# ArbiterMob/FluidSimulationCuda

Measured on AMD Instinct MI355X. Metric: Mcells/s per Jacobi iter, higher is better.
Workload: dtype f32

## Files before the change

### fluidsimulationcuda_amd/capi.py

```python
import ctypes as C
import os

import numpy as np

from ._build import LIB

OK, E_INVALID, E_NOMEM, E_HIP, E_COMM = 0, 1, 2, 3, 4
U, V, DENS, U_PREV, V_PREV, DENS_PREV, TMP0, TMP1, TMP2, TMP3, TMP4, TMP5 = range(12)
NFIELDS = 12
JACOBI_STREAM, JACOBI_LDS, JACOBI_NAIVE, JACOBI_TB = 0, 1, 2, 3
STORAGE_F32, STORAGE_F16 = 0, 1
PARAM_TB_MAX_SWEEPS, PARAM_TB_ROWS, PARAM_HALO, PARAM_TB_FAST_DIVISION, PARAM_TB_MIN_CELLS, PARAM_TB_EDGE_ROWS_PCT = 0, 1, 2, 3, 4, 5
PARAM_TB_LANE_COLUMNS = 6
PARAM_TB_T16_MIN_CELLS = 7
PARAM_TB_AUTOTUNE = 8
PARAM_FUSE_DIVERGENCE = 9
PARAM_SLAB_OVERLAP = 10
PARAM_EARLY_ADVECT = 11
PARAM_FUSE_ADD_SOURCE = 12
PARAM_XCHG_OVERLAP = 13
PARAM_F16_PRESSURE_SCALE = 14
PARAM_TB_FILL = 15
XCHG_HALO, XCHG_GATHER, XCHG_MAX, XCHG_MAX_BEGIN, XCHG_MAX_END = 0, 1, 2, 3, 4
RCCL_ID_BYTES = 128
FIELD_NAMES = ("u", "v", "dens", "u_prev", "v_prev", "dens_prev", "tmp0", "tmp1", "tmp2", "tmp3", "tmp4", "tmp5")


class FluidError(RuntimeError):
    def __init__(self, code, msg):
        super().__init__("libfluid_amd error %d: %s" % (code, msg))
        self.code = code


class Config(C.Structure):
    _fields_ = [("n", C.c_int), ("rank", C.c_int), ("nranks", C.c_int), ("halo", C.c_int),
                ("jacobi_variant", C.c_int), ("stream", C.c_void_p), ("arena", C.c_void_p),
                ("arena_bytes", C.c_size_t), ("storage", C.c_int)]


TIME_SOURCE, TIME_DIFFUSION, TIME_DIVERGENCE, TIME_PROJECTION, TIME_ADVECTION = range(5)
TIMING_CATEGORIES = ("source", "diffusion", "divergence", "projection", "advection")


class Timing(C.Structure):
    _fields_ = [("jacobi_ms", C.c_double), ("sweeps", C.c_longlong), ("solves", C.c_longlong),
                ("category_ms", C.c_double * 5), ("category_calls", C.c_longlong * 5),
                ("jacobi_launches", C.c_longlong), ("jacobi_field_launches", C.c_longlong),
                ("pressure_ms", C.c_double), ("pressure_sweeps", C.c_longlong)]


class RunPlan(C.Structure):
    _fields_ = [("iters", C.c_int), ("nsteps", C.c_int), ("use_sources", C.c_int), ("sources", C.c_void_p),
                ("every", C.c_int), ("fields", C.POINTER(C.c_int)), ("nfields", C.c_int),
                ("snapshots", C.c_void_p), ("capacity", C.c_size_t)]


EXCHANGE_FN = C.CFUNCTYPE(C.c_int, C.c_void_p, C.c_int, C.POINTER(C.c_int), C.c_int, C.c_int,
                          C.POINTER(C.c_float))

_HOSTF = np.ctypeslib.ndpointer(dtype=np.float32, flags="C_CONTIGUOUS")
_ctx = C.c_void_p
_i, _f = C.c_int, C.c_float
_MF = C.POINTER(C.c_float)

SIGNATURES = {
    "step": [_i, _f, _f, _f, _HOSTF, _HOSTF, _HOSTF],
    "step_src": [_i, _f, _f, _f, _i] + [_HOSTF] * 6,
    "fluid_release_cached": [],
    "fluid_coefficients": [_i, _f, _f, C.POINTER(_f), C.POINTER(_f)],
    "fluid_layout": [_i, C.POINTER(_i), C.POINTER(_i), C.POINTER(C.c_size_t)],
    "fluid_create": [_i, C.POINTER(_ctx)],
    "fluid_create_ex": [C.POINTER(Config), C.POINTER(_ctx)],
    "fluid_create_ensemble": [C.POINTER(Config), _i, C.POINTER(_ctx)],
    "fluid_members": [_ctx, C.POINTER(_i)],
    "fluid_upload_member": [_ctx, _i, _i, _HOSTF],
    "fluid_download_member": [_ctx, _i, _i, _HOSTF],
    "fluid_step_members": [_ctx, _MF, _MF, _MF, _i, _i, _i],
    "fluid_vel_step_members": [_ctx, _MF, _MF, _i],
    "fluid_dens_step_members": [_ctx, _MF, _MF, _i],
    "fluid_op_add_source_members": [_ctx, _i, _i, _MF],
    "fluid_op_jacobi_sweep_members": [_ctx, _i, _i, _i, _i, _MF, _MF],
    "fluid_op_diffuse_members": [_ctx, _i, _i, _i, _MF, _MF, _i],
    "fluid_op_advect_members": [_ctx, _i, _i, _i, _i, _i, _MF],
    "fluid_destroy": [_ctx],
    "fluid_synchronize": [_ctx],
    "fluid_owned_rows": [_ctx, C.POINTER(_i), C.POINTER(_i)],
    "fluid_field_ptr": [_ctx, _i, C.POINTER(C.c_void_p)],
    "fluid_scalar_ptr": [_ctx, C.POINTER(C.c_void_p)],
    "fluid_upload": [_ctx, _i, _HOSTF],
    "fluid_download": [_ctx, _i, _HOSTF],
    "fluid_upload_rows": [_ctx, _i, _HOSTF, _i, _i],
    "fluid_download_rows": [_ctx, _i, _HOSTF, _i, _i],
    "fluid_fill": [_ctx, _i, _f],
    "fluid_step": [_ctx, _f, _f, _f, _i, _i, _i],
    "fluid_vel_step": [_ctx, _f, _f, _i],
    "fluid_dens_step": [_ctx, _f, _f, _i],
    "fluid_op_set_bnd": [_ctx, _i, _i],
    "fluid_op_add_source": [_ctx, _i, _i, _f],
    "fluid_op_jacobi_sweep": [_ctx, _i, _i, _i, _i, _f, _f],
    "fluid_op_diffuse": [_ctx, _i, _i, _i, _f, _f, _i],
    "fluid_op_advect": [_ctx, _i, _i, _i, _i, _i, _f],
    "fluid_op_divergence": [_ctx, _i, _i, _i, _i],
    "fluid_op_subtract_gradient": [_ctx, _i, _i, _i],
    "fluid_residual": [_ctx, _i, _i, _f, _f, C.POINTER(_f)],
    "fluid_absmax_velocity": [_ctx, _i, _i, C.POINTER(_f)],
    "fluid_residual_members": [_ctx, _i, _i, _MF, _MF, _MF],
    "fluid_absmax_velocity_members": [_ctx, _i, _i, _MF],
    "fluid_member_moments": [_ctx, _i, C.POINTER(C.c_double), C.POINTER(C.c_double)],
    "fluid_ensemble_stats": [_ctx, _i, _MF, _MF],
    "fluid_ensemble_stats_ptr": [_ctx, C.POINTER(C.c_void_p), C.POINTER(C.c_void_p)],
    "fluid_member_gram": [_ctx, _i, _i, C.POINTER(C.c_double)],
    "fluid_pack_members": [_ctx, _i, _i, _i, C.c_void_p, C.c_size_t],
    "fluid_unpack_members": [_ctx, _i, _i, _i, C.c_void_p, C.c_size_t],
    "fluid_download_members": [_ctx, _i, _MF],
    "fluid_upload_members": [_ctx, _i, _MF],
    "fluid_run": [_ctx, _f, _f, _f, C.POINTER(RunPlan), C.POINTER(_i)],
    "fluid_run_members": [_ctx, _MF, _MF, _MF, C.POINTER(RunPlan), C.POINTER(_i)],
    "fluid_coarse_size": [_i, _i, C.POINTER(_i)],
    "fluid_pack_members_coarse": [_ctx, _i, _i, _i, _i, C.c_void_p, C.c_size_t],
    "fluid_download_members_coarse": [_ctx, _i, _i, _MF],
    "fluid_run_coarse": [_ctx, _f, _f, _f, C.POINTER(RunPlan), _i, C.POINTER(_i)],
    "fluid_run_members_coarse": [_ctx, _MF, _MF, _MF, C.POINTER(RunPlan), _i, C.POINTER(_i)],
    "fluid_transform_members": [_ctx, C.POINTER(_i), _i, _MF],
    "fluid_select_members": [_ctx, C.POINTER(_i), _i, C.POINTER(_i)],
    "fluid_set_jacobi_variant": [_ctx, _i],
    "fluid_division_mode": [_ctx, _f, _f, C.POINTER(_i)],
    "fluid_autotune_pending": [_ctx, C.POINTER(_i)],
    "fluid_plan_sweeps": [_i, _i, _i, _i, _i, _i, _i, C.POINTER(_i), _i, C.POINTER(_i)],
    "fluid_set_param": [_ctx, _i, _i],
    "fluid_timing_enable": [_ctx, _i],
    "fluid_timing_read": [_ctx, C.POINTER(Timing), _i],
    "fluid_op_diffuse_tol": [_ctx, _i, _i, _i, _f, _f, _f, _i, _i, C.POINTER(_i), C.POINTER(_f)],
    "fluid_set_exchange": [_ctx, EXCHANGE_FN, C.c_void_p],
    "fluid_exchange_now": [_ctx, _i, C.POINTER(_i), _i, _i],
    "fluid_exchange_stream": [_ctx, C.POINTER(C.c_void_p)],
    "fluid_split_launches": [_ctx, C.POINTER(C.c_longlong)],
    "fluid_rccl_available": [],
    "fluid_rccl_unique_id": [C.c_void_p, C.c_size_t],
    "fluid_exchange_rccl_attach": [_ctx, C.c_void_p, C.c_size_t],
    "fluid_exchange_rccl_attach_comm": [_ctx, C.c_void_p],
    "fluid_exchange_rccl_detach": [_ctx],
    "fluid_exchange_rccl_calls": [_ctx, C.POINTER(C.c_longlong), C.POINTER(C.c_longlong), C.POINTER(C.c_longlong)],
}
OTHER_SYMBOLS = {"fluid_last_error": (C.c_char_p, []), "fluid_arena_bytes": (C.c_size_t, [_i]),
                 "fluid_arena_bytes_ex": (C.c_size_t, [_i, _i]),
                 "fluid_arena_bytes_ensemble": (C.c_size_t, [_i, _i, _i])}
MAX_MEMBERS = 21845
COARSE_FACTORS = (1, 2, 4, 8, 16, 32, 64)
TRANSFORM_MAX_MEMBERS = 64

_lib = None


def lib():
    global _lib
    if _lib is None:
        if not os.path.exists(LIB):
            raise ImportError("%s not found: run `python -c 'import __graft_entry__ as g; g.build()'` "
                              "(hipcc --offload-arch=gfx950). There is no CPU fallback." % LIB)
        try:
            import torch
        except ImportError:
            pass
        L = C.CDLL(LIB)
        for name, args in SIGNATURES.items():
            fn = getattr(L, name)
            fn.restype, fn.argtypes = C.c_int, args
        for name, (res, args) in OTHER_SYMBOLS.items():
            fn = getattr(L, name)
            fn.restype, fn.argtypes = res, args
        _lib = L
    return _lib


def check(rc):
    if rc != OK:
        raise FluidError(rc, lib().fluid_last_error().decode(errors="replace"))
```

### fluidsimulationcuda_amd/csrc/fluid_ctx.h

```cpp
#pragma once
#include <hip/hip_runtime.h>

#include <string>
#include <utility>
#include <vector>

#include "../../include/fluid_amd.h"
#include "fluid_kernels.h"

namespace fluid_detail {
int fail(int code, const char* fmt, ...);
int materialize_zero(fluid_ctx* c, int f);
int refuse_ensemble(const fluid_ctx* c, const char* what);
struct RcclExchange;
void rccl_release(RcclExchange* x);
}

#define HIP_TRY(expr)                                                                                      \
    do {                                                                                                   \
        hipError_t e_ = (expr);                                                                            \
        if (e_ != hipSuccess)                                                                              \
            return fluid_detail::fail(e_ == hipErrorOutOfMemory ? FLUID_E_NOMEM : FLUID_E_HIP, "%s: %s",   \
                                      #expr, hipGetErrorString(e_));                                       \
    } while (0)

#define TRY(expr)                        \
    do {                                 \
        int rc_ = (expr);                \
        if (rc_ != FLUID_OK) return rc_; \
    } while (0)

class MemberVal {
    float s_;
    std::vector<float> v_;
    explicit MemberVal(std::vector<float>&& v) : s_(v[0]), v_(std::move(v)) {}

public:
    MemberVal(float v = 0.0f) : s_(v) {}
    MemberVal(const float* per_member, int members) : s_(per_member[0]), v_(per_member, per_member + members) {}
    bool uniform() const { return v_.empty(); }
    float at(int m) const { return v_.empty() ? s_ : v_[(size_t)m]; }
    const std::vector<float>& values() const { return v_; }
    bool operator==(const MemberVal& o) const { return s_ == o.s_ && v_ == o.v_; }
    template <class F>
    MemberVal map(const MemberVal& b, F f) const
    {
        if (uniform() && b.uniform()) return MemberVal(f(s_, b.s_));
        std::vector<float> r(uniform() ? b.v_.size() : v_.size());
        for (size_t m = 0; m < r.size(); ++m) r[m] = f(at((int)m), b.at((int)m));
        return MemberVal(std::move(r));
    }
    template <class F>
    MemberVal map(F f) const { return map(MemberVal(), [&](float x, float) { return f(x); }); }
};

struct FieldState {
    void* ptr = nullptr;
    int reach = 0;
    bool zero = false;
    bool pend = false;
    MemberVal pend_inc;
    int src_of = 0;
    MemberVal src_dt;
    float fscale = 1.0f;
};

struct ConstRing {
    char *dev = nullptr, *host = nullptr;
    size_t bytes = 0, head = 0;
    struct Blob { size_t off, len; unsigned long long hash; hipEvent_t copied; };
    std::vector<Blob> live;
    std::vector<hipEvent_t> free_events;
};

struct EnsembleReduce {
    unsigned int* d_max = nullptr;
    double2* d_moments = nullptr;
    double2* d_partials = nullptr;
    char* host = nullptr;
    float *d_mean = nullptr, *d_var = nullptr;
    bool have_stats = false;
    double *d_gram_partials = nullptr, *d_gram = nullptr, *gram_host = nullptr;
};

struct MemberStage {
    float* dev = nullptr;
    int members = 0;
};

struct TransformTables {
    static constexpr int kSlots = 8;
    char *dev = nullptr, *host = nullptr;
    size_t slot = 0;
    int next = 0;
    hipEvent_t copied[kSlots] = {};
    bool in_use[kSlots] = {};
};

struct fluid_ctx {
    int n = 0, w = 0, pitch = 0;
    size_t field_floats = 0;
    int members = 1;
    char* arena = nullptr;
    bool own_arena = false;
    int st = fluid::STORAGE_F32;
    size_t esz = 4;
    hipStream_t stream = nullptr;
    bool own_stream = false;
    hipStream_t stream2 = nullptr;
    hipEvent_t ev_fork = nullptr, ev_join = nullptr;
    bool slab_overlap = true;
    hipStream_t xstream = nullptr;
    hipEvent_t ev_xbegin = nullptr, ev_xdone = nullptr;
    bool xchg_overlap = true;
    unsigned xowed = 0;
    long long split_launches = 0;
    bool early_advect = true;
    float vmax_prev[2] = {-1.0f, -1.0f};
    FieldState field[FLUID_NFIELDS];
    size_t field_bytes = 0;
    unsigned int* d_scalar = nullptr;
    float* d_partials = nullptr;
    ConstRing consts;
    EnsembleReduce red;
    MemberStage stage;
    TransformTables xform;
    unsigned int* tiles = nullptr;
    unsigned int* h_scalar = nullptr;
    hipEvent_t scalar_ready = nullptr;
    int variant = fluid::JACOBI_TB;
    int tb_max_t = 16, tb_rows = 0, num_cu = 256;
    long long tb_min_cells = 0;
    long long tb_t16_min_cells = -1;
    bool fuse_divergence = true;
    bool tb_fill = true;
    bool autotune = true;
    struct Trial { unsigned long long key; int cand; hipEvent_t a, b; };
    std::vector<Trial> trials;
    std::vector<hipEvent_t> free_events;
    bool defer_zero_source = true;
    bool in_halo_exchange = false;
    int tb_nv = 2;
    int tb_edge_pct = 40;
    int fast_div = 2;
    int rank = 0, nranks = 1, own0 = 1, own1 = 1, min_slab = 0, halo = 1;
    bool fuse_add_source = true;
    float pscale = 1.0f;
    fluid_exchange_fn xchg = nullptr;
    void* xchg_user = nullptr;
    fluid_detail::RcclExchange* rccl = nullptr;
    bool timing = false;
    struct Ev { hipEvent_t a, b; int cat; bool pressure; };
    std::vector<Ev> ev_pool;
    size_t ev_used = 0;
    double cat_ms[FLUID_TIMING_CATEGORIES] = {};
    long long cat_calls[FLUID_TIMING_CATEGORIES] = {};
    long long sweeps = 0, pending_sweeps = 0, launches = 0, field_launches = 0;
    double pressure_ms = 0.0;
    long long pressure_sweeps = 0, pending_pressure_sweeps = 0;
    bool in_pressure_solve = false;

    bool valid_field(int id) const { return id >= 0 && id < FLUID_NFIELDS; }
    void* ptr(int id) const { return field[id].ptr; }
    fluid::Members mb() const { return {members, field_floats}; }
    size_t all_bytes() const { return field_bytes * (size_t)members; }
    void* row(int id, int r) const { return static_cast<char*>(ptr(id)) + (size_t)r * pitch * esz; }
    int lo_all() const { return own0 - (rank == 0 ? 1 : 0); }
    int hi_all() const { return own1 + (rank == nranks - 1 ? 1 : 0); }
};
```

### fluidsimulationcuda_amd/csrc/fluid_kernels.h

```cpp
#pragma once
#include <hip/hip_runtime.h>

namespace fluid {

constexpr int XOFF = 63;

enum JacobiVariant { JACOBI_STREAM = 0, JACOBI_LDS = 1, JACOBI_NAIVE = 2, JACOBI_TB = 3, JACOBI_VARIANTS = 4 };

enum Storage { STORAGE_F32 = 0, STORAGE_F16 = 1 };
typedef _Float16 half_t;
inline size_t storage_bytes(int st) { return st == STORAGE_F16 ? 2 : 4; }

inline int pitch_for(int n) { return ((XOFF + 1 + 4 * ((n + 3) / 4) + 1) + 63) / 64 * 64; }

struct Members {
    int count = 1;
    size_t stride = 0;
};

struct TbMemberK {
    double yd;
    float alpha, beta, hi, lo;
    float x0_inc, div_scale;
    unsigned tile_thr, pad;
};

struct TbBatch {
    const void* x[3];
    const void* x0[3];
    void* out[3];
    float alpha[3], beta[3];
    double yd[3];
    float hi[3], lo[3];
    const unsigned* tiles[3];
    unsigned tile_thr[3];
    int tile_pitch;
    void* div[3];
    float div_scale;
    int b[3];
    int x_zero[3];
    float x0_inc[3];
    int count;
    int members;
    size_t mstride;
    size_t tile_mstride;
    const TbMemberK* mk;
};

void launch_set_bnd(hipStream_t s, int st, void* f, int pitch, int n, int b, Members mb = {});
void launch_add_source(hipStream_t s, int st, void* x, const void* src, int pitch, int row_lo, int row_hi, float dt, Members mb = {},
                       const float* mdt = nullptr);
void launch_jacobi(hipStream_t s, int st, int variant, const void* x, const void* x0, void* out, int pitch, int n,
                   int row_lo, int row_hi, float alpha, float beta, int b, Members mb = {}, const float2* mab = nullptr);
enum TbForm { TB_PLAIN = 0, TB_DIVSRC = 1, TB_ADDSRC = 2 };
struct TbShape { int T, divmode, nv, form; };
inline constexpr TbShape kTbShapes[] = {
    {2, 0, 2, TB_PLAIN},   {2, 2, 2, TB_PLAIN},   {2, 3, 2, TB_PLAIN},   {2, 4, 2, TB_PLAIN},   {2, 5, 2, TB_PLAIN},
    {2, 0, 4, TB_PLAIN},   {2, 2, 4, TB_PLAIN},   {2, 3, 4, TB_PLAIN},   {2, 4, 4, TB_PLAIN},   {2, 5, 4, TB_PLAIN},
    {4, 0, 2, TB_PLAIN},   {4, 2, 2, TB_PLAIN},   {4, 3, 2, TB_PLAIN},   {4, 4, 2, TB_PLAIN},   {4, 5, 2, TB_PLAIN},
    {4, 0, 4, TB_PLAIN},   {4, 2, 4, TB_PLAIN},   {4, 3, 4, TB_PLAIN},   {4, 4, 4, TB_PLAIN},   {4, 5, 4, TB_PLAIN},
    {8, 0, 2, TB_PLAIN},   {8, 2, 2, TB_PLAIN},   {8, 3, 2, TB_PLAIN},   {8, 4, 2, TB_PLAIN},   {8, 5, 2, TB_PLAIN},
    {8, 0, 4, TB_PLAIN},   {8, 2, 4, TB_PLAIN},   {8, 3, 4, TB_PLAIN},   {8, 4, 4, TB_PLAIN},   {8, 5, 4, TB_PLAIN},
    {12, 0, 2, TB_PLAIN},  {12, 2, 2, TB_PLAIN},  {12, 3, 2, TB_PLAIN},  {12, 4, 2, TB_PLAIN},  {12, 5, 2, TB_PLAIN},
    {16, 0, 2, TB_PLAIN},  {16, 2, 2, TB_PLAIN},  {16, 3, 2, TB_PLAIN},  {16, 4, 2, TB_PLAIN},  {16, 5, 2, TB_PLAIN},
    {8, 4, 2, TB_DIVSRC},  {12, 4, 2, TB_DIVSRC}, {16, 4, 2, TB_DIVSRC}, {8, 0, 2, TB_ADDSRC},  {8, 2, 2, TB_ADDSRC},  {8, 5, 2, TB_ADDSRC},
    {12, 0, 2, TB_ADDSRC}, {12, 2, 2, TB_ADDSRC}, {12, 5, 2, TB_ADDSRC}, {16, 0, 2, TB_ADDSRC}, {16, 2, 2, TB_ADDSRC}, {16, 5, 2, TB_ADDSRC},
};
constexpr int kTbShapeCount = sizeof(kTbShapes) / sizeof(kTbShapes[0]);
constexpr int jacobi_tb_index(int T, int divmode, int nv, int form)
{
    for (int i = 0; i < kTbShapeCount; ++i) {
        const TbShape& s = kTbShapes[i];
        if ((T < 0 || s.T == T) && (divmode < 0 || s.divmode == divmode) && s.nv == nv && s.form == form) return i;
    }
    return -1;
}
constexpr bool jacobi_tb_exists(int T, int divmode, int nv, int form) { return jacobi_tb_index(T, divmode, nv, form) >= 0; }
constexpr bool tb_shapes_unique(int i = 0)
{
    return i == kTbShapeCount || (jacobi_tb_index(kTbShapes[i].T, kTbShapes[i].divmode, kTbShapes[i].nv, kTbShapes[i].form) == i && tb_shapes_unique(i + 1));
}
static_assert(kTbShapeCount == 52 && tb_shapes_unique(), "52 distinct shapes: adding or removing one is a change of this table");
inline constexpr int kTbDepths[] = {16, 12, 8, 4, 2};
constexpr bool is_tb_depth(int T) { for (int d : kTbDepths) if (d == T) return true; return false; }
bool launch_jacobi_tb(hipStream_t s, int st, int T, int divmode, int nv, int form, const TbBatch& batch, int pitch, int n, int row_lo,
                      int row_hi, int rb, int rb_edge, int hole_lo = 0, int hole_hi = 0, bool fill = true);
constexpr int kTileRows = 32, kTileCols = 64;
inline int tile_rows(int n) { return (n + kTileRows - 1) / kTileRows; }
inline int tile_pitch(int n) { return (n + kTileCols - 1) / kTileCols; }
struct TileBatch {
    const void* field[3];
    unsigned* tiles[3];
    int count;
    size_t mstride, tile_mstride;
};
void launch_tile_min_abs(hipStream_t s, int st, const TileBatch& tb, int count, int pitch, int n, int row_lo, int row_hi, int tile_pitch,
                         Members mb = {}, size_t tile_mstride = 0);
void launch_validate_div(hipStream_t s, int divmode, float beta, float kbeta, double yd, float hi, float lo, unsigned long long* bad);
void launch_advect(hipStream_t s, int st, void* d, const void* d0, const void* u, const void* v, int pitch, int n,
                   int row_lo, int row_hi, float dt0, int b, Members mb = {}, const float* mdt0 = nullptr);
void launch_advect2(hipStream_t s, int st, void* da, const void* d0a, int ba, void* db, const void* d0b, int bb, const void* u,
                    const void* v, int pitch, int n, int row_lo, int row_hi, float dt0, Members mb = {}, const float* mdt0 = nullptr);
void launch_divergence(hipStream_t s, int st, const void* u, const void* v, void* p, void* div, int pitch, int n,
                       int row_lo, int row_hi, float h, int write_p, float pscale = 1.0f, Members mb = {});
void launch_scale(hipStream_t s, int st, void* x, int pitch, int row_lo, int row_hi, float factor, Members mb = {});
constexpr int kMaxPartials = 8192;
void launch_subtract_gradient(hipStream_t s, int st, void* u, void* v, const void* p, int pitch, int n, int row_lo,
                              int row_hi, float h, float* partials = nullptr, unsigned int* max_out = nullptr, float pinv = 1.0f,
                              Members mb = {});
void launch_gradient_advect(hipStream_t s, int st, void* u, void* v, const void* p, void* d, const void* d0, int pitch, int n,
                            int row_lo, int row_hi, float h, float dt0, int b, float pinv = 1.0f, Members mb = {},
                            const float* mdt0 = nullptr);
void launch_absmax2(hipStream_t s, int st, const void* u, const void* v, int pitch, int n, int row_lo, int row_hi,
                    unsigned int* result, Members mb = {}, int rstride = 0);
void launch_residual(hipStream_t s, int st, const void* x, const void* x0, int pitch, int n, int row_lo, int row_hi,
                     float alpha, float beta, unsigned int* result, Members mb = {}, int rstride = 0, const float2* mab = nullptr);
constexpr int kMomentBlocks = 4096;
int moment_blocks(int n, int members);
void launch_member_moments(hipStream_t s, int st, const void* x, int pitch, int n, Members mb, double2* partials, double2* out);
void launch_ensemble_stats(hipStream_t s, int st, const void* x, int pitch, int n, Members mb, float* mean, float* var);
void launch_pack_members(hipStream_t s, int st, const void* x, int pitch, int n, Members mb, float inv, float* dense, size_t dstride);
void launch_unpack_members(hipStream_t s, int st, void* x, int pitch, int n, Members mb, const float* dense, size_t dstride);
void launch_pack_members_coarse(hipStream_t s, int st, const void* x, int pitch, int n, Members mb, float inv, int factor, float* coarse,
                                size_t cstride);
constexpr int kTransformMaxMembers = 64;
inline int transform_padded(int members)
{
    int mp = 1;
    while (mp < members) mp <<= 1;
    return mp;
}
void launch_transform_members(hipStream_t s, int st, void* x, int pitch, int n, Members mb, float inv, const double* table,
                              const unsigned long long* bits, unsigned long long empty, bool dense);
inline int gram_padded(int members) { return members > 8 ? transform_padded(members) : 8; }
int gram_blocks(int n, int members);
void launch_member_gram(hipStream_t s, int st, const void* x, int pitch, int n, Members mb, float inv, bool centre, double* partials,
                        double* out);

}
```

### fluidsimulationcuda_amd/csrc/fluid_kernels.hip

```cpp
#include <hip/hip_runtime.h>
#include <stdint.h>

#include <algorithm>
#include <array>
#include <cstdlib>
#include <utility>

#include "fluid_kernels.h"

namespace fluid {

__device__ __forceinline__ float flip_if(bool c, float v) { return c ? -v : v; }

__device__ __forceinline__ float keep_f32(float v) { asm("" : "+v"(v)); return v; }
__device__ __forceinline__ float ld1(const float* p) { return *p; }
__device__ __forceinline__ float ld1(const half_t* p) { return keep_f32((float)*p); }
__device__ __forceinline__ void st1(float* p, float v) { *p = v; }
__device__ __forceinline__ void st1(half_t* p, float v) { *p = (half_t)keep_f32(v); }
template <typename S>
__device__ __forceinline__ float as_stored(float v)
{
    if constexpr (sizeof(S) == 2) return keep_f32((float)(S)keep_f32(v));
    else return v;
}
// ... 222 lines not shown
    if (mab) {
        const float2 ab = mab[blockIdx.z];
        alpha = ab.x;
        beta = ab.y;
    }
    x += blockIdx.z * ms; x0 += blockIdx.z * ms; out += blockIdx.z * ms;
    const int lane = threadIdx.x & 63;
    const int vec = blockIdx.x * 256 + threadIdx.x;
    const int nvec = (n + 3) >> 2;
    const int i0 = row_lo + blockIdx.y * RB;
    const int i1 = min(i0 + RB, row_hi);
    const bool active = vec < nvec;
    const int v = active ? vec : nvec - 1;
    const int j = 1 + 4 * v;
    const size_t P = (size_t)pitch;
    const S* xc = x + XOFF + j;
    const S* rc = x0 + XOFF + j;
    S* oc = out + XOFF + j;
    const bool edge_lo = (lane == 0), edge_hi = (lane == 63) | (vec >= nvec - 1);
    const bool nx = (b == 1), ny = (b == 2);

    float4 up = ld4(xc + (size_t)(i0 - 1) * P);
    float4 me = ld4(xc + (size_t)i0 * P);
    for (int i = i0; i < i1; ++i) {
        const float4 dn = ld4(xc + (size_t)(i + 1) * P);
        const float4 r = ld4(rc + (size_t)i * P);
        float le = 0.f, re = 0.f;
        if (edge_lo) le = ld1(xc + (size_t)i * P - 1);
        if (edge_hi) re = ld1(xc + (size_t)i * P + 4);
        float L = from_lane_below(me.w, le);
        float R = from_lane_above(me.x, re);
        if (edge_lo) L = le;
        if (edge_hi) R = re;
        float4 o;
        float nb;
        nb = L + me.y;     nb = nb + up.x; nb = nb + dn.x; o.x = (r.x + alpha * nb) / beta;
        nb = me.x + me.z;  nb = nb + up.y; nb = nb + dn.y; o.y = (r.y + alpha * nb) / beta;
        nb = me.y + me.w;  nb = nb + up.z; nb = nb + dn.z; o.z = (r.z + alpha * nb) / beta;
        nb = me.z + R;     nb = nb + up.w; nb = nb + dn.w; o.w = (r.w + alpha * nb) / beta;
        if (active) {
            S* orow = oc + (size_t)i * P;
            const int last = n - j;
            if (last >= 3) {
                st4(orow, o);
            } else {
                st1(orow, o.x);
                if (last >= 1) st1(orow + 1, o.y);
                if (last >= 2) st1(orow + 2, o.z);
            }
            const float vn = last == 0 ? o.x : last == 1 ? o.y : last == 2 ? o.z : o.w;
            if (j == 1) st1(orow - 1, flip_if(nx, o.x));
            if (last <= 3) st1(orow + last + 1, flip_if(nx, vn));
            if (i == 1 || i == n) {
                float4 g4;
                g4.x = flip_if(ny, o.x); g4.y = flip_if(ny, o.y);
                g4.z = flip_if(ny, o.z); g4.w = flip_if(ny, o.w);
                const float cl = 0.5f * (g4.x + flip_if(nx, o.x));
                const float cr = 0.5f * (flip_if(ny, vn) + flip_if(nx, vn));
#pragma unroll
                for (int side = 0; side < 2; ++side) {
                    if (side == 0 ? i != 1 : i != n) continue;
                    S* g = oc + (side == 0 ? (size_t)0 : (size_t)(n + 1) * P);
                    if (last >= 3) {
                        st4(g, g4);
                    } else {
                        st1(g, g4.x);
                        if (last >= 1) st1(g + 1, g4.y);
                        if (last >= 2) st1(g + 2, g4.z);
                    }
                    if (j == 1) st1(g - 1, cl);
                    if (last <= 3) st1(g + last + 1, cr);
                }
            }
        }
        up = me;
        me = dn;
    }
}



template <int NV>
struct Vec {
    float c[NV];
};
typedef float v2f __attribute__((ext_vector_type(2)));
typedef half_t half2_t __attribute__((ext_vector_type(2)));

template <int NV>
__device__ __forceinline__ Vec<NV> buf_ldv(const float*, __amdgpu_buffer_rsrc_t r, unsigned off)
{
    Vec<NV> v;
    if constexpr (NV == 4) {
        const uint4_t u = __builtin_amdgcn_raw_buffer_load_b128(r, off, 0, 0);
        v.c[0] = __uint_as_float(u.x); v.c[1] = __uint_as_float(u.y); v.c[2] = __uint_as_float(u.z); v.c[3] = __uint_as_float(u.w);
    } else {
        const uint2_t u = __builtin_amdgcn_raw_buffer_load_b64(r, off, 0, 0);
        v.c[0] = __uint_as_float(u.x); v.c[1] = __uint_as_float(u.y);
    }
    return v;
}
template <int NV>
__device__ __forceinline__ Vec<NV> buf_ldv(const half_t*, __amdgpu_buffer_rsrc_t r, unsigned off)
{
    Vec<NV> v;
    if constexpr (NV == 4) {
        const uint2_t u = __builtin_amdgcn_raw_buffer_load_b64(r, off, 0, 0);
        half4_t h;
        __builtin_memcpy(&h, &u, 8);
        v.c[0] = keep_f32((float)h.x); v.c[1] = keep_f32((float)h.y); v.c[2] = keep_f32((float)h.z); v.c[3] = keep_f32((float)h.w);
    } else {
        const unsigned u = __builtin_amdgcn_raw_buffer_load_b32(r, off, 0, 0);
        half2_t h;
        __builtin_memcpy(&h, &u, 4);
        v.c[0] = keep_f32((float)h.x); v.c[1] = keep_f32((float)h.y);
    }
    return v;
}
template <int NV>
__device__ __forceinline__ void buf_stv(float*, __amdgpu_buffer_rsrc_t r, unsigned off, const Vec<NV>& v)
{
    if constexpr (NV == 4) {
        uint4_t u;
        u.x = __float_as_uint(v.c[0]); u.y = __float_as_uint(v.c[1]); u.z = __float_as_uint(v.c[2]); u.w = __float_as_uint(v.c[3]);
        __builtin_amdgcn_raw_buffer_store_b128(u, r, off, 0, 0);
    } else {
        uint2_t u;
        u.x = __float_as_uint(v.c[0]); u.y = __float_as_uint(v.c[1]);
        __builtin_amdgcn_raw_buffer_store_b64(u, r, off, 0, 0);
    }
}
template <int NV>
__device__ __forceinline__ void buf_stv(half_t*, __amdgpu_buffer_rsrc_t r, unsigned off, const Vec<NV>& v)
{
    if constexpr (NV == 4) {
        half4_t h;
        h.x = (half_t)keep_f32(v.c[0]); h.y = (half_t)keep_f32(v.c[1]); h.z = (half_t)keep_f32(v.c[2]); h.w = (half_t)keep_f32(v.c[3]);
        uint2_t u;
        __builtin_memcpy(&u, &h, 8);
        __builtin_amdgcn_raw_buffer_store_b64(u, r, off, 0, 0);
    } else {
        half2_t h;
        h.x = (half_t)keep_f32(v.c[0]); h.y = (half_t)keep_f32(v.c[1]);
        unsigned u;
        __builtin_memcpy(&u, &h, 4);
        __builtin_amdgcn_raw_buffer_store_b32(u, r, off, 0, 0);
    }
}

struct DivK {
    float beta;
    double yd;
    float hi, lo;
};
constexpr float kDiv5NegScale = -0x1p24f;

template <typename S, int NV>
struct TbArgs {
    const S* xc;
    const S* rc;
    S* oc;
    __amdgpu_buffer_rsrc_t bx, br, bo;
    unsigned ld_off;
    unsigned st_off;
    unsigned row_bytes;
    unsigned m_lg;
    unsigned m_r[NV];
    int n, q_lo, q_hi, cg;
    float alpha;
    DivK k;
    S* dc;
    __amdgpu_buffer_rsrc_t bd;
    float div_scale;
    int s_lo, s_hi;
    unsigned sx, sy;
    float x0_inc;
    bool st_rg_lane, is_lg;
    bool fill;
};

__device__ __forceinline__ float fxor(float v, unsigned m) { return __uint_as_float(__float_as_uint(v) ^ m); }
template <int NV>
__device__ __forceinline__ Vec<NV> fxorv(const Vec<NV>& v, unsigned m)
{
    Vec<NV> o;
#pragma unroll
    for (int c = 0; c < NV; ++c) o.c[c] = fxor(v.c[c], m);
    return o;
}

template <int DIVMODE>
__device__ __forceinline__ float tb_div(float num, const DivK& k)
{
    if (DIVMODE == 0) return num / k.beta;
    if (DIVMODE == 4) return num * k.beta;
    if (DIVMODE == 3) return __builtin_fmaf(num, k.hi, num * k.lo);
    if (DIVMODE == 5) {
        const float q0 = num * k.beta;
        const float e = __builtin_fmaf(q0, k.hi, num * kDiv5NegScale);
        return __builtin_fmaf(e, k.lo, q0);
    }
    return (float)((double)num * k.yd);
}
template <int DIVMODE>
__device__ __forceinline__ v2f tb_div2(v2f num, const DivK& k)
{
    if constexpr (DIVMODE == 4) return num * k.beta;
    else if constexpr (DIVMODE == 3) {
        const v2f p = num * k.lo;
        return __builtin_elementwise_fma(num, (v2f){k.hi, k.hi}, p);
    } else if constexpr (DIVMODE == 5) {
        const v2f ds = num * kDiv5NegScale;
        const v2f q0 = num * k.beta;
        const v2f e = __builtin_elementwise_fma(q0, (v2f){k.hi, k.hi}, ds);
        return __builtin_elementwise_fma(e, (v2f){k.lo, k.lo}, q0);
    } else return (v2f){tb_div<DIVMODE>(num.x, k), tb_div<DIVMODE>(num.y, k)};
}

template <int DIVMODE, int NV>
__device__ __forceinline__ Vec<NV> tb_stencil(const Vec<NV>& up, const Vec<NV>& me, const Vec<NV>& dn, const Vec<NV>& r,
                                              float alpha, const DivK& k)
{
    float h[NV];
    h[0] = lane_below0(me.c[NV - 1]) + me.c[1];
#pragma unroll
    for (int c = 1; c < NV - 1; ++c) h[c] = me.c[c - 1] + me.c[c + 1];
    h[NV - 1] = me.c[NV - 2] + lane_above0(me.c[0]);
    Vec<NV> G;
#pragma unroll
    for (int p = 0; p < NV; p += 2) {
        v2f s = {h[p], h[p + 1]};
        s = s + (v2f){up.c[p], up.c[p + 1]};
        s = s + (v2f){dn.c[p], dn.c[p + 1]};
        if constexpr (DIVMODE != 4) s = s * alpha;
        s = (v2f){r.c[p], r.c[p + 1]} + s;
        s = tb_div2<DIVMODE>(s, k);
        G.c[p] = s.x;
        G.c[p + 1] = s.y;
    }
    return G;
}

template <int DIVMODE>
__global__ __launch_bounds__(256) void k_validate_div(float beta, DivK k, unsigned long long* __restrict__ bad)
{
    unsigned long long n = 0;
    const unsigned long long stride = (unsigned long long)gridDim.x * 256;
    auto differs = [](float got, float ref) { return (ref != ref) ? !(got != got) : (__float_as_uint(got) != __float_as_uint(ref)); };
    DivK k2 = k;
    for (unsigned long long i = (unsigned long long)blockIdx.x * 256 + threadIdx.x; i < (1ull << 32); i += stride) {
        const float a = __uint_as_float((unsigned)i);
        const float ref = a / beta;
        if constexpr (DIVMODE == 3) {
            const bool in_range = a == 0.0f || !(__builtin_fabsf(a) < beta * 0x1p-98f);
            n += differs(tb_div<2>(a, k2), ref) || (in_range && differs(tb_div<3>(a, k), ref));
        } else if constexpr (DIVMODE == 5) {
            const float got = tb_div<5>(a, k);
            const bool finite = __builtin_fabsf(got) < __builtin_inff();
            const bool must_be_exact = __builtin_fabsf(a) < 0x1p100f;
            n += differs(got, ref) && (finite || must_be_exact);
        } else {
            n += differs(tb_div<DIVMODE>(a, k), ref);
        }
    }
    if (n) atomicAdd(bad, n);
}

__device__ __forceinline__ float bitsel(unsigned mask, float a, float b)
{
    return __uint_as_float((__float_as_uint(a) & mask) | (__float_as_uint(b) & ~mask));
}

template <typename S, int NV>
__device__ __forceinline__ void tb_fix_columns(Vec<NV>& G, const TbArgs<S, NV>& a, float& v1, float& vn, bool need_corners)
{
    float o[NV];
#pragma unroll
    for (int c = 0; c < NV; ++c) o[c] = G.c[c];
    const float from_right = lane_above0(o[0]);
    const float from_left = lane_below0(o[NV - 1]);
    G.c[0] = bitsel(a.m_r[0], fxor(from_left, a.sx), o[0]);
#pragma unroll
    for (int c = 1; c < NV - 1; ++c) G.c[c] = bitsel(a.m_r[c], fxor(o[c - 1], a.sx), o[c]);
    G.c[NV - 1] = bitsel(a.m_lg, fxor(from_right, a.sx), bitsel(a.m_r[NV - 1], fxor(o[NV - 2], a.sx), o[NV - 1]));
    if (need_corners) {
        v1 = from_right;
        unsigned bits = __float_as_uint(from_left) & a.m_r[0];
#pragma unroll
        for (int c = 1; c < NV; ++c) bits |= __float_as_uint(o[c - 1]) & a.m_r[c];
        vn = __uint_as_float(bits);
    }
}

template <bool EDGE, bool WALL, typename S, int NV>
__device__ __forceinline__ void tb_store_to(S* oc, __amdgpu_buffer_rsrc_t bo, const Vec<NV>& G, int q, bool mine, const TbArgs<S, NV>& a,
                                            float v1, float vn)
{
    auto on = [](bool c, unsigned off) { return c ? off : kBufOff; };
    buf_stv<NV>(oc, bo, on(mine, a.st_off) + (unsigned)q * a.row_bytes, G);
    if (WALL) {
        Vec<NV> g = fxorv<NV>(G, a.sy);
        if (EDGE) {
            const float cl = 0.5f * (fxor(v1, a.sy) + fxor(v1, a.sx));
            const float cr = 0.5f * (fxor(vn, a.sy) + fxor(vn, a.sx));
            if (a.is_lg) g.c[NV - 1] = cl;
#pragma unroll
            for (int c = 0; c < NV; ++c)
                if (a.st_rg_lane && a.cg == c) g.c[c] = cr;
        }
        buf_stv<NV>(oc, bo, on(mine & (q == 1), a.st_off), g);
        buf_stv<NV>(oc, bo, on(mine & (q == a.n), a.st_off) + (unsigned)(a.n + 1) * a.row_bytes, g);
    }
}
template <bool EDGE, bool WALL, typename S, int NV>
__device__ __forceinline__ void tb_store(const Vec<NV>& G, int q, bool mine, const TbArgs<S, NV>& a, float v1, float vn)
{
    tb_store_to<EDGE, WALL, S, NV>(a.oc, a.bo, G, q, mine, a, v1, vn);
}

template <int NV>
__device__ __forceinline__ Vec<NV> tb_divergence(const Vec<NV>& u, const Vec<NV>& v_up, const Vec<NV>& v_dn, float scale)
{
    float g[NV];
#pragma unroll
    for (int c = 0; c < NV; ++c) {
        const float ur = c < NV - 1 ? u.c[c + 1] : lane_above0(u.c[0]);
        const float ul = c > 0 ? u.c[c - 1] : lane_below0(u.c[NV - 1]);
        g[c] = ur - ul;
    }
    Vec<NV> d;
#pragma unroll
    for (int p = 0; p < NV; p += 2) {
        v2f s = {g[p], g[p + 1]};
        s = s + (v2f){v_dn.c[p], v_dn.c[p + 1]};
        s = s - (v2f){v_up.c[p], v_up.c[p + 1]};
        s = s * scale;
        d.c[p] = s.x;
        d.c[p + 1] = s.y;
    }
    return d;
}

template <int NV>
__device__ __forceinline__ Vec<NV> take(const Vec<NV>& v)
{
    Vec<NV> o;
#pragma unroll
    for (int p = 0; p < NV; p += 2) {
        v2f in = {v.c[p], v.c[p + 1]}, out;
        asm("v_mov_b64 %0, %1" : "=v"(out) : "v"(in));
        o.c[p] = out.x;
        o.c[p + 1] = out.y;
    }
    return o;
}

template <int K, int N, int NV>
__device__ __forceinline__ void tb_qshift(Vec<NV> (&Q)[N])
{
    if constexpr (K >= 1) {
        Q[K] = Q[K - 1];
        tb_qshift<K - 1, N, NV>(Q);
    }
}

template <int DIVMODE, int NV>
__device__ __forceinline__ void tb_sticky(const Vec<NV>& G, v2f& nf)
{
    if constexpr (DIVMODE == 5) {
#pragma unroll
        for (int p = 0; p < NV; p += 2) nf = __builtin_elementwise_fma((v2f){G.c[p], G.c[p + 1]}, (v2f){0.f, 0.f}, nf);
    }
}

template <int T, int DIVMODE, bool EDGE, bool WALL, bool GEN, int PH, typename S, int NV, bool DIVSRC = false, bool ADDSRC = false,
          bool PART = false>
__device__ __forceinline__ void tb_step(int t, Vec<NV> (&W)[T][3], Vec<NV> (&Q)[T + 1], Vec<NV> (&PX)[3], Vec<NV> (&PQ)[3],
                                        const TbArgs<S, NV>& a, Vec<NV> (&UR)[3], Vec<NV> (&VR)[3], v2f& nf, int smax = T)
{
    static_assert(!(PART && GEN), "the general body runs every stage");
    constexpr int UP = PH % 3, ME = (PH + 1) % 3, FR = (PH + 2) % 3;
    __builtin_amdgcn_sched_barrier(0);
    if constexpr (DIVSRC) {
        UR[FR] = take<NV>(PX[PH]);
        VR[FR] = take<NV>(PQ[PH]);
    } else {
        W[0][FR] = take<NV>(PX[PH]);
        Q[0] = take<NV>(PQ[PH]);
        if constexpr (ADDSRC) {
#pragma unroll
            for (int p = 0; p < NV; p += 2) {
                const v2f ds = (v2f){W[0][FR].c[p], W[0][FR].c[p + 1]} * a.div_scale;
                const v2f q = (v2f){Q[0].c[p], Q[0].c[p + 1]} + ds;
                Q[0].c[p] = as_stored<S>(q.x);
                Q[0].c[p + 1] = as_stored<S>(q.y);
            }
            buf_stv<NV>(a.dc, a.bd, (((t >= a.s_lo) & (t < a.s_hi)) ? a.st_off : kBufOff) + (unsigned)t * a.row_bytes, Q[0]);
        } else {
#pragma unroll
            for (int p = 0; p < NV; p += 2) {
                const v2f q = (v2f){Q[0].c[p], Q[0].c[p + 1]} + a.x0_inc;
                Q[0].c[p] = q.x;
                Q[0].c[p + 1] = q.y;
            }
        }
    }
    {
        const unsigned off = a.ld_off + (unsigned)(t + 3) * a.row_bytes;
        PX[PH] = buf_ldv<NV>(a.xc, a.bx, off);
        PQ[PH] = buf_ldv<NV>(a.rc, a.br, off);
    }
    __builtin_amdgcn_sched_barrier(0);
    if constexpr (DIVSRC) {
        const int q = t - 1;
        Vec<NV> D = tb_divergence<NV>(UR[ME], VR[UP], VR[FR], a.div_scale);
#pragma unroll
        for (int c = 0; c < NV; ++c) D.c[c] = as_stored<S>(D.c[c]);
        Q[1] = D;
        float v1 = 0.f, vn = 0.f;
        if (EDGE) tb_fix_columns<S, NV>(D, a, v1, vn, WALL);
        tb_store_to<EDGE, (WALL || GEN), S, NV>(a.dc, a.bd, D, q, (q >= 1) & (q <= a.n) & (q >= a.q_lo) & (q < a.q_hi), a, v1, vn);
    }
    if constexpr (!GEN) {
#pragma unroll
        for (int s = 1; s <= T; ++s) {
            const bool run = !PART || s <= smax;
            const int q = t - s;
            Vec<NV> G;
            float v1 = 0.f, vn = 0.f;
            if (run) {
                G = tb_stencil<DIVMODE, NV>(W[s - 1][UP], W[s - 1][ME], W[s - 1][FR], Q[s], a.alpha, a.k);
                if (EDGE) tb_fix_columns<S, NV>(G, a, v1, vn, WALL && s == T);
                if (s == T) tb_sticky<DIVMODE, NV>(G, nf);
            } else {
#pragma unroll
                for (int c = 0; c < NV; ++c) G.c[c] = __builtin_nondeterministic_value(W[s - 1][FR].c[c]);
            }
            if (s < T) W[s][FR] = G;
            else tb_store<EDGE, WALL, S, NV>(G, q, run & (q >= a.q_lo) & (q < a.q_hi), a, v1, vn);
        }
    } else {
#pragma unroll
        for (int s = 1; s <= T; ++s) {
            const int q = t - s;
            const bool interior = (q >= 1 && q <= a.n);
            Vec<NV> G = tb_stencil<DIVMODE, NV>(W[s - 1][UP], W[s - 1][ME], W[s - 1][FR], Q[s], a.alpha, a.k);
            float v1 = 0.f, vn = 0.f;
            if (EDGE) tb_fix_columns<S, NV>(G, a, v1, vn, s == T);
            if (s < T) {
                const Vec<NV> me = W[s][ME];
                const Vec<NV> flipped_me = fxorv<NV>(me, a.sy);
                const Vec<NV> flipped_g = fxorv<NV>(G, a.sy);
                const bool bot_ghost = (q == a.n + 1), top_ghost = (q == 1);
#pragma unroll
                for (int c = 0; c < NV; ++c) {
                    W[s][FR].c[c] = bot_ghost ? flipped_me.c[c] : G.c[c];
                    W[s][ME].c[c] = top_ghost ? flipped_g.c[c] : me.c[c];
                }
            } else {
                tb_sticky<DIVMODE, NV>(G, nf);
                tb_store<EDGE, true, S, NV>(G, q, interior & (q >= a.q_lo) & (q < a.q_hi), a, v1, vn);
            }
        }
    }
    tb_qshift<T, T + 1, NV>(Q);
}

template <int T, int DIVMODE, bool EDGE, bool WALL, typename S, int NV, bool DIVSRC = false, bool ADDSRC = false>
__device__ __forceinline__ bool tb_march(int t0, int t1, const TbArgs<S, NV>& a)
{
    Vec<NV> W[T][3], Q[T + 1], PX[3], PQ[3], UR[3], VR[3];
    v2f nf = {0.f, 0.f};
    Vec<NV> zero;
#pragma unroll
    for (int c = 0; c < NV; ++c) zero.c[c] = 0.f;
#pragma unroll
    for (int s = 0; s < T; ++s) { W[s][0] = zero; W[s][1] = zero; W[s][2] = zero; }
#pragma unroll
    for (int s = 0; s <= T; ++s) Q[s] = zero;
#pragma unroll
    for (int d = 0; d < 3; ++d) { UR[d] = zero; VR[d] = zero; }
#pragma unroll
    for (int d = 0; d < 3; ++d) {
        const unsigned off = a.ld_off + (unsigned)(t0 + d) * a.row_bytes;
        PX[d] = buf_ldv<NV>(a.xc, a.bx, off);
        PQ[d] = buf_ldv<NV>(a.rc, a.br, off);
        buf_stv<NV>(a.oc, a.bo, kBufOff, zero);
        if constexpr (DIVSRC || ADDSRC) buf_stv<NV>(a.dc, a.bd, kBufOff, zero);
        __builtin_amdgcn_sched_barrier(0);
    }
    int t = t0;
    if constexpr (WALL) {
        for (; t <= t1 && t < T + 1; t += 3) {
            tb_step<T, DIVMODE, EDGE, WALL, true, 0, S, NV, DIVSRC, ADDSRC>(t, W, Q, PX, PQ, a, UR, VR, nf);
            tb_step<T, DIVMODE, EDGE, WALL, true, 1, S, NV, DIVSRC, ADDSRC>(t + 1, W, Q, PX, PQ, a, UR, VR, nf);
            tb_step<T, DIVMODE, EDGE, WALL, true, 2, S, NV, DIVSRC, ADDSRC>(t + 2, W, Q, PX, PQ, a, UR, VR, nf);
        }
    }
    const int fill_end = (a.fill && t0 == a.q_lo - T) ? t0 + 3 * ((2 * T + 2) / 3) : t0;
    const int full_end = a.fill ? t1 - 2 : t1;
    auto stages = [&](int u) { return u > t1 ? 0 : u < fill_end ? (u - t0) >> 1 : T; };
    for (; t <= t1 && t < fill_end && (!WALL || t + 1 <= a.n); t += 3) {
        tb_step<T, DIVMODE, EDGE, WALL, false, 0, S, NV, DIVSRC, ADDSRC, true>(t, W, Q, PX, PQ, a, UR, VR, nf, stages(t));
        tb_step<T, DIVMODE, EDGE, WALL, false, 1, S, NV, DIVSRC, ADDSRC, true>(t + 1, W, Q, PX, PQ, a, UR, VR, nf, stages(t + 1));
        tb_step<T, DIVMODE, EDGE, WALL, false, 2, S, NV, DIVSRC, ADDSRC, true>(t + 2, W, Q, PX, PQ, a, UR, VR, nf, stages(t + 2));
    }
    for (; t <= full_end && (!WALL || t + 1 <= a.n); t += 3) {
        tb_step<T, DIVMODE, EDGE, WALL, false, 0, S, NV, DIVSRC, ADDSRC>(t, W, Q, PX, PQ, a, UR, VR, nf);
        tb_step<T, DIVMODE, EDGE, WALL, false, 1, S, NV, DIVSRC, ADDSRC>(t + 1, W, Q, PX, PQ, a, UR, VR, nf);
        tb_step<T, DIVMODE, EDGE, WALL, false, 2, S, NV, DIVSRC, ADDSRC>(t + 2, W, Q, PX, PQ, a, UR, VR, nf);
    }
    for (; t <= t1 && (!WALL || t + 1 <= a.n); t += 3) {
        tb_step<T, DIVMODE, EDGE, WALL, false, 0, S, NV, DIVSRC, ADDSRC, true>(t, W, Q, PX, PQ, a, UR, VR, nf, stages(t));
        tb_step<T, DIVMODE, EDGE, WALL, false, 1, S, NV, DIVSRC, ADDSRC, true>(t + 1, W, Q, PX, PQ, a, UR, VR, nf, stages(t + 1));
        tb_step<T, DIVMODE, EDGE, WALL, false, 2, S, NV, DIVSRC, ADDSRC, true>(t + 2, W, Q, PX, PQ, a, UR, VR, nf, stages(t + 2));
    }
    if constexpr (WALL) {
        for (; t <= t1; t += 3) {
            tb_step<T, DIVMODE, EDGE, WALL, true, 0, S, NV, DIVSRC, ADDSRC>(t, W, Q, PX, PQ, a, UR, VR, nf);
            tb_step<T, DIVMODE, EDGE, WALL, true, 1, S, NV, DIVSRC, ADDSRC>(t + 1, W, Q, PX, PQ, a, UR, VR, nf);
            tb_step<T, DIVMODE, EDGE, WALL, true, 2, S, NV, DIVSRC, ADDSRC>(t + 2, W, Q, PX, PQ, a, UR, VR, nf);
        }
    }
    if constexpr (DIVMODE == 5) return __builtin_amdgcn_ballot_w64((nf.x != nf.x) | (nf.y != nf.y)) != 0ull;
    else return false;
}

template <int T, int DIVMODE, typename S, int NV, bool DIVSRC = false, bool ADDSRC = false>
__device__ __forceinline__ bool tb_march_any(bool edge, bool wall, int t0, int t1, const TbArgs<S, NV>& a)
{
    if (edge) {
        if (wall) return tb_march<T, DIVMODE, true, true, S, NV, DIVSRC, ADDSRC>(t0, t1, a);
        return tb_march<T, DIVMODE, true, false, S, NV, DIVSRC, ADDSRC>(t0, t1, a);
    }
    if (wall) return tb_march<T, DIVMODE, false, true, S, NV, DIVSRC, ADDSRC>(t0, t1, a);
    return tb_march<T, DIVMODE, false, false, S, NV, DIVSRC, ADDSRC>(t0, t1, a);
}

struct TbGrid {
    int inner_wins, inner_blocks, edge_wins, edge_blocks, first_right;
    int hole_lo, hole_hi;
};

constexpr int tb_waves_per_simd(int T, int NV) { return NV == 2 ? (T <= 8 ? 4 : T <= 12 ? 3 : 2) : (T <= 4 ? 3 : 2); }

template <int T, int DIVMODE, int NV, typename S, bool DIVSRC = false, bool ADDSRC = false>
__global__ __launch_bounds__(256, tb_waves_per_simd(T, NV)) void k_jacobi_tb(TbBatch batch, int pitch, int n, int row_lo,
                                                                             int row_hi, int rb, int rb_edge, TbGrid g, int fill)
{
    static_assert(!DIVSRC || DIVMODE == 4, "the divergence-sourced launch is the first launch of a pressure solve");
    static_assert(!(DIVSRC && ADDSRC) && (!ADDSRC || DIVMODE != 3), "one second store per launch; mode 3's tiles are taken from the summed field");
    const unsigned per_xcd = gridDim.x >> 3;
    unsigned vid = (blockIdx.x & 7u) * per_xcd + (blockIdx.x >> 3);
    if (vid >= (unsigned)(g.inner_blocks + g.edge_blocks)) return;
    int win, strip_group;
    if (vid < (unsigned)g.inner_blocks) {
        win = 1 + (int)(vid % (unsigned)g.inner_wins);
        strip_group = (int)(vid / (unsigned)g.inner_wins);
    } else {
        vid -= (unsigned)g.inner_blocks;
        const int e = (int)(vid % (unsigned)g.edge_wins);
        strip_group = (int)(vid / (unsigned)g.edge_wins);
        win = e == 0 ? 0 : g.first_right + e - 1;
    }
    const unsigned member = batch.count == 3 ? blockIdx.z / 3u : batch.count == 2 ? blockIdx.z >> 1 : blockIdx.z;
    const unsigned sv = blockIdx.z - member * (unsigned)batch.count;
    const size_t mofs = (size_t)member * batch.mstride;
    const S* __restrict__ x = static_cast<const S*>(batch.x[sv]) + mofs;
    const S* __restrict__ x0 = static_cast<const S*>(batch.x0[sv]) + mofs;
    S* __restrict__ out = static_cast<S*>(batch.out[sv]) + mofs;
    float alpha = batch.alpha[sv], beta = batch.beta[sv];
    double yd = batch.yd[sv];
    float k_hi = batch.hi[sv], k_lo = batch.lo[sv], x0_inc = batch.x0_inc[sv], div_scale = batch.div_scale;
    unsigned tile_thr = batch.tile_thr[sv];
    if (batch.mk != nullptr) {
        typedef const TbMemberK __attribute__((address_space(4))) * MemberKPtr;
        const MemberKPtr mk = (MemberKPtr)(uintptr_t)batch.mk + ((size_t)sv * (unsigned)batch.members + member);
        alpha = mk->alpha;
        beta = mk->beta;
        yd = mk->yd;
        k_hi = mk->hi;
        k_lo = mk->lo;
        x0_inc = mk->x0_inc;
        if (ADDSRC) div_scale = mk->div_scale;
        if (DIVMODE == 3) tile_thr = mk->tile_thr;
    }
    const int b = batch.b[sv];
    constexpr int HL = (T + NV - 1) / NV;
    constexpr int VS = 64 - 2 * HL;
    constexpr int C0 = (XOFF + 1) / NV;
    static_assert((XOFF + 1) % NV == 0 && HL <= C0, "window overlap must fit the row's left pad");
    const int lane = threadIdx.x & 63;
    const int strip = strip_group * 4 + __builtin_amdgcn_readfirstlane(threadIdx.x >> 6);
    const int kg = n / NV;
    const bool left_edge = (win == 0);
    const bool right_edge = (kg >= win * VS - HL) && (kg < win * VS - HL + 64);
    const bool edge = left_edge || right_edge;
    const int rbw = edge ? rb_edge : rb;
    TbArgs<S, NV> a;
    a.k.yd = yd;
    a.k.lo = k_lo;
    a.k.hi = k_hi;
    a.x0_inc = x0_inc;
    int seg_hi = row_hi;
    a.q_lo = row_lo + strip * rbw;
    if (g.hole_lo < g.hole_hi) {
        const int top = (g.hole_lo - row_lo + rbw - 1) / rbw;
        if (strip < top) seg_hi = g.hole_lo;
        else a.q_lo = g.hole_hi + (strip - top) * rbw;
    }
    if (a.q_lo >= seg_hi) return;
    a.q_hi = min(a.q_lo + rbw, seg_hi);
    a.s_lo = a.q_lo == 1 ? 0 : a.q_lo;
    a.s_hi = a.q_hi == n + 1 ? n + 2 : a.q_hi;
    const int k = win * VS - HL + lane;
    const int nvec = (n + NV - 1) / NV;
    const bool ld_ok = k <= pitch / NV - C0 - 1;
    const ptrdiff_t cofs = (ptrdiff_t)(XOFF + 1) + NV * (ptrdiff_t)(ld_ok ? k : 0);
    a.xc = x + cofs;
    a.rc = x0 + cofs;
    a.oc = out + cofs;
    {
        const unsigned field_bytes = (unsigned)((size_t)(n + 2) * (size_t)pitch * sizeof(S));
        a.bx = __builtin_amdgcn_make_buffer_rsrc(const_cast<S*>(x), 0, (batch.x_zero[sv] && !DIVSRC) ? 0u : field_bytes, 0x00020000);
        a.br = __builtin_amdgcn_make_buffer_rsrc(const_cast<S*>(x0), 0, field_bytes, 0x00020000);
        a.bo = __builtin_amdgcn_make_buffer_rsrc(out, 0, field_bytes, 0x00020000);
        S* dv = (DIVSRC || ADDSRC) ? static_cast<S*>(batch.div[sv]) + mofs : out;
        a.dc = dv + cofs;
        a.bd = __builtin_amdgcn_make_buffer_rsrc(dv, 0, field_bytes, 0x00020000);
        a.div_scale = div_scale;
        a.row_bytes = (unsigned)((size_t)pitch * sizeof(S));
        const unsigned col = (unsigned)((XOFF + 1 + NV * (ptrdiff_t)k) * (ptrdiff_t)sizeof(S));
        a.ld_off = ld_ok ? col : kBufOff;
    }
    a.n = n;
    a.cg = n % NV;
    a.is_lg = (k == -1);
    const bool is_rg = (k == kg);
    const bool own = (lane >= HL) && (lane < 64 - HL);
    const bool st_int = own && k >= 0 && k < nvec;
    a.st_rg_lane = is_rg && (own || k == nvec);
    a.m_lg = a.is_lg ? 0xFFFFFFFFu : 0u;
#pragma unroll
    for (int c = 0; c < NV; ++c) a.m_r[c] = (is_rg && a.cg == c) ? 0xFFFFFFFFu : 0u;
    a.st_off = (ld_ok && (st_int || a.is_lg || a.st_rg_lane)) ? a.ld_off : kBufOff;
    a.sx = (b == 1) ? 0x80000000u : 0u;
    a.sy = (b == 2) ? 0x80000000u : 0u;
    a.alpha = alpha;
    a.k.beta = beta;
    a.fill = fill != 0;
    const int t0 = max(0, a.q_lo - T), t1 = a.q_hi - 1 + T;
    const bool wall = (a.q_lo < T) || (a.q_hi - 1 + T > n + 1);
    constexpr int DM = DIVMODE == 3 ? 2 : DIVMODE;
    bool two_term = false;
    if constexpr (DIVMODE == 3) {
        const unsigned* __restrict__ tiles = batch.tiles[sv] ? batch.tiles[sv] + (size_t)member * batch.tile_mstride : nullptr;
        const unsigned thr = tile_thr;
        const int tr0 = (max(1, a.q_lo - T + 1) - 1) / kTileRows, tr1 = (min(n, a.q_hi + T - 2) - 1) / kTileRows;
        const int c0 = max(1, 1 + NV * (win * VS - HL)), c1 = min(n, NV * (win * VS - HL + 64));
        const int tc0 = (c0 - 1) / kTileCols, tc1 = (c1 - 1) / kTileCols, ntc = tc1 - tc0 + 1;
        const int count = (tr1 - tr0 + 1) * ntc;
        bool low = false;
        if (tiles != nullptr)
            for (int i = lane; i < count; i += 64)
                low |= tiles[(size_t)(tr0 + i / ntc) * batch.tile_pitch + (tc0 + i % ntc)] < thr;
        two_term = tiles != nullptr && __builtin_amdgcn_ballot_w64(low) == 0ull;
    }
    if (two_term) {
        tb_march_any<T, DIVMODE, S, NV>(edge, wall, t0, t1, a);
    } else {
        const bool again = tb_march_any<T, DM, S, NV, DIVSRC, ADDSRC>(edge, wall, t0, t1, a);
        if constexpr (DIVMODE == 5) {
            if (again) tb_march_any<T, 2, S, NV, false, ADDSRC>(edge, wall, t0, t1, a);
        }
    }
}

template <typename S>
__global__ __launch_bounds__(256) void k_tile_min_abs(TileBatch tb, int pitch, int n, int row_lo, int row_hi, int tile_row0, int tile_pitch)
{
    const unsigned member = blockIdx.z / (unsigned)tb.count, sv = blockIdx.z - member * (unsigned)tb.count;
    const S* __restrict__ f = static_cast<const S*>(tb.field[sv]) + (size_t)member * tb.mstride;
    unsigned* __restrict__ out = tb.tiles[sv] + (size_t)member * tb.tile_mstride;
    const int lane = threadIdx.x & 63, wave = threadIdx.x >> 6;
    const int tr = tile_row0 + blockIdx.y;
    const int j = 1 + 4 * (lane + 64 * (blockIdx.x * 4 + wave));
    const int i0 = max(row_lo, 1 + tr * kTileRows), i1 = min(row_hi, 1 + (tr + 1) * kTileRows);
    const size_t P = (size_t)pitch;
    float m = __builtin_inff();
    if (j <= n)
        for (int i = i0; i < i1; ++i) {
            const float4 v = ld4(f + (size_t)i * P + XOFF + j);
            m = fminf(m, fabsf(v.x));
            if (j + 1 <= n) m = fminf(m, fabsf(v.y));
            if (j + 2 <= n) m = fminf(m, fabsf(v.z));
            if (j + 3 <= n) m = fminf(m, fabsf(v.w));
        }
#pragma unroll
    for (int off = 8; off > 0; off >>= 1) m = fminf(m, __shfl_xor(m, off, 16));
    const bool whole = row_lo <= 1 + tr * kTileRows && row_hi >= min(n + 1, 1 + (tr + 1) * kTileRows);
    if ((lane & 15) == 0 && j <= n) out[(size_t)tr * tile_pitch + (j - 1) / kTileCols] = whole ? __float_as_uint(m) : 0u;
}

template <typename S, typename IDX>
__device__ __forceinline__ const S* at(const S* base, IDX byte_off) { return reinterpret_cast<const S*>(reinterpret_cast<const char*>(base) + byte_off); }
template <typename S, typename IDX>
__device__ __forceinline__ S* at(S* base, IDX byte_off) { return reinterpret_cast<S*>(reinterpret_cast<char*>(base) + byte_off); }

template <typename IDX>
struct AdvectTap {
    IDX o;
    float s0, s1, t0, t1;
};

template <typename IDX>
__device__ __forceinline__ AdvectTap<IDX> advect_trace(int j, int i, float uu, float vv, float dt0, int n, IDX P, IDX E)
{
    float px = (float)j - dt0 * uu;
    float py = (float)i - dt0 * vv;
    const float hi = (float)n + 0.5f;
    px = __builtin_fminf(__builtin_fmaxf(px, 0.5f), hi);
    py = __builtin_fminf(__builtin_fmaxf(py, 0.5f), hi);
    const int j0 = (int)px, i0 = (int)py;
    AdvectTap<IDX> t;
    t.s1 = px - (float)j0;
    t.s0 = 1.0f - t.s1;
    t.t1 = py - (float)i0;
    t.t0 = 1.0f - t.t1;
    t.o = (IDX)i0 * P + (IDX)(XOFF + j0) * E;
    return t;
}

struct __attribute__((packed, aligned(4))) FloatPair { float a, b; };
__device__ __forceinline__ void ld_pair(const float* p, float& a, float& b)
{
    const FloatPair v = *reinterpret_cast<const FloatPair*>(p);
    a = v.a;
    b = v.b;
}
__device__ __forceinline__ void ld_pair(const half_t* p, float& a, float& b)
{
    a = ld1(p);
    b = ld1(p + 1);
}

template <typename S, typename IDX>
__device__ __forceinline__ float advect_sample(const S* __restrict__ d0, IDX P, const AdvectTap<IDX>& t)
{
    float q00, q10, q01, q11;
    ld_pair(at(d0, t.o), q00, q10);
    ld_pair(at(d0, t.o + P), q01, q11);
    const float a = t.t0 * q00 + t.t1 * q01;
    const float e = t.t0 * q10 + t.t1 * q11;
    return t.s0 * a + t.s1 * e;
}

constexpr int kAdvectRounds = 4;
__device__ __forceinline__ int advect_col0() { return 1 + (int)blockIdx.x * 1024 + (int)(threadIdx.x >> 6) * 256 + (int)(threadIdx.x & 63); }
__device__ __forceinline__ bool advect_wall_block(int i, int n) { return i == 1 || i == n || blockIdx.x == 0 || blockIdx.x == gridDim.x - 1; }

template <typename S>
__device__ __forceinline__ void wave_cells_in(const S* __restrict__ p, int cells, float* __restrict__ tile, float (&out)[4])
{
    const int lane = threadIdx.x & 63;
    const int vec = min(lane, (cells - 1) >> 2);
    *reinterpret_cast<float4*>(tile + 4 * lane) = ld4(p + 4 * vec);
    __builtin_amdgcn_wave_barrier();
#pragma unroll
    for (int k = 0; k < 4; ++k) out[k] = tile[lane + 64 * k];
    __builtin_amdgcn_wave_barrier();
}
template <typename S>
__device__ __forceinline__ void wave_cells_out(S* __restrict__ p, int cells, float* __restrict__ tile, const float (&val)[4])
{
    const int lane = threadIdx.x & 63;
#pragma unroll
    for (int k = 0; k < 4; ++k) tile[lane + 64 * k] = val[k];
    __builtin_amdgcn_wave_barrier();
    const float4 y = *reinterpret_cast<const float4*>(tile + 4 * lane);
    __builtin_amdgcn_wave_barrier();
    const int left = cells - 4 * lane;
    if (left >= 4) {
        st4(p + 4 * lane, y);
    } else if (left > 0) {
        st1(p + 4 * lane, y.x);
        if (left > 1) st1(p + 4 * lane + 1, y.y);
        if (left > 2) st1(p + 4 * lane + 2, y.z);
    }
}

template <typename S, typename IDX>
__global__ __launch_bounds__(256) void k_advect(S* __restrict__ d, const S* __restrict__ d0, const S* __restrict__ u,
                                                const S* __restrict__ v, int pitch, int n, int row_lo, int row_hi,
                                                float dt0, int b, size_t ms, const float* __restrict__ mdt0)
{
    __shared__ __attribute__((aligned(16))) float tiles[4][2][256];
    if (mdt0) dt0 = mdt0[blockIdx.z];
    d += blockIdx.z * ms; d0 += blockIdx.z * ms; u += blockIdx.z * ms; v += blockIdx.z * ms;
    const int j0 = advect_col0();
    const int i = row_lo + blockIdx.y;
    if (i >= row_hi) return;
    const IDX E = (IDX)sizeof(S), P = (IDX)pitch * E;
    const IDX r = (IDX)i * P + (IDX)XOFF * E;
    const bool wall = advect_wall_block(i, n);
    const int wave = threadIdx.x >> 6;
    const int c0 = j0 - (int)(threadIdx.x & 63);
    const int cells = min(256, n + 1 - c0);
    if (cells <= 0) return;
    float uu[kAdvectRounds], vv[kAdvectRounds], val[kAdvectRounds];
    wave_cells_in(at(u, r + (IDX)c0 * E), cells, tiles[wave][0], uu);
    wave_cells_in(at(v, r + (IDX)c0 * E), cells, tiles[wave][1], vv);
#pragma unroll
    for (int k = 0; k < kAdvectRounds; ++k) val[k] = advect_sample(d0, P, advect_trace<IDX>(min(j0 + 64 * k, n), i, uu[k], vv[k], dt0, n, P, E));
    wave_cells_out(at(d, r + (IDX)c0 * E), cells, tiles[wave][0], val);
    if (wall) {
#pragma unroll
        for (int k = 0; k < kAdvectRounds; ++k) {
            const int j = j0 + 64 * k;
            if (j <= n) emit_ghosts(d, (size_t)pitch, n, b, j, i, val[k]);
        }
    }
}

template <typename S, typename IDX>
// ... 646 lines not shown
    const int bi = (int)(t / (unsigned)groups), g = (int)(t % (unsigned)groups);
    x += blockIdx.y * ms;
    coarse += blockIdx.y * cstride;
    const bool own = (threadIdx.x & 63u) == 0 || g == 0;
    I at = (I)(bi << LR) * (I)pitch + (I)(XOFF + 1 + VW * g);
    double s[OUTS];
    coarse_rows<S, I, LR, ROWS, true>(x, at, pitch, inv, own, s);
#pragma unroll 1
    for (int i = ROWS; i < R; i += ROWS) {
        at += (I)ROWS * (I)pitch;
        coarse_rows<S, I, LR, ROWS, false>(x, at, pitch, inv, own, s);
    }
    const size_t out = (size_t)bi * (size_t)side;
    if constexpr (R >= VW) {
        if ((g & (LANES - 1)) == 0) coarse[out + (size_t)(g / LANES)] = (float)(s[0] * SCALE);
    } else {
#pragma unroll
        for (int k = 0; k < OUTS; ++k)
            if (g * OUTS + k < side) coarse[out + (size_t)(g * OUTS + k)] = (float)(s[k] * SCALE);
    }
}

constexpr int kTransformAhead = 4;

template <int MP, bool DENSE>
__device__ __forceinline__ void transform_term(double (&acc)[MP], double xd, const double* __restrict__ w, unsigned long long bits)
{
    if constexpr (DENSE) {
#pragma unroll
        for (int g = 0; g < MP; g += 32) {
#pragma unroll
            for (int m = g; m < g + 32 && m < MP; ++m) acc[m] = __builtin_fma(xd, w[m], acc[m]);
            __builtin_amdgcn_sched_barrier(0);
        }
    } else {
        if (bits == 0) return;
#pragma unroll
        for (int g = 0; g < MP; g += 8) {
            if (MP > 8 && ((bits >> g) & 0xffull) == 0) continue;
#pragma unroll
            for (int m = g; m < g + 8 && m < MP; ++m)
                if ((bits >> m) & 1ull) acc[m] = __builtin_fma(xd, w[m], acc[m]);
        }
    }
}

template <typename S, int MP, bool DENSE>
__global__ __launch_bounds__(256) void k_transform_members(S* __restrict__ x, int pitch, int n, size_t ms, int members, float inv,
                                                           const double* __restrict__ table, const unsigned long long* __restrict__ bits,
                                                           unsigned long long empty)
{
    const unsigned col = blockIdx.x * 256u + threadIdx.x;
    if (col > (unsigned)(n + 1)) return;
    x += (size_t)blockIdx.y * (size_t)pitch + (size_t)XOFF;
    double acc[MP];
#pragma unroll
    for (int m = 0; m < MP; ++m) acc[m] = -0.0;
    int k = 0;
    for (; k + kTransformAhead <= members; k += kTransformAhead) {
        float f[kTransformAhead];
#pragma unroll
        for (int r = 0; r < kTransformAhead; ++r) f[r] = ld1(x + (size_t)(k + r) * ms + col);
#pragma unroll
        for (int r = 0; r < kTransformAhead; ++r) {
            if constexpr (sizeof(S) != 4) f[r] = f[r] * inv;
            transform_term<MP, DENSE>(acc, (double)f[r], table + (size_t)(k + r) * MP, DENSE ? 0ull : bits[k + r]);
        }
    }
    for (; k < members; ++k) {
        float f = ld1(x + (size_t)k * ms + col);
        if constexpr (sizeof(S) != 4) f = f * inv;
        transform_term<MP, DENSE>(acc, (double)f, table + (size_t)k * MP, DENSE ? 0ull : bits[k]);
    }
#pragma unroll
    for (int m = 0; m < MP; ++m)
        if (m < members) st1(x + (size_t)m * ms + col, (empty >> m) & 1ull ? 0.0f : (float)acc[m]);
}

static inline unsigned cdiv(unsigned a, unsigned b) { return (a + b - 1) / b; }

static inline bool narrow_index(int st, int pitch, int n) { return (size_t)(n + 2) * (size_t)pitch * storage_bytes(st) < (1ull << 32); }

#define FLUID_BY_STORAGE(st, ...)             \
    do {                                      \
        if ((st) == STORAGE_F16) {            \
            using S = half_t;                 \
            __VA_ARGS__;                      \
        } else {                              \
            using S = float;                  \
            __VA_ARGS__;                      \
        }                                     \
    } while (0)
#define FLUID_BY_STORAGE_INDEX(st, pitch, n, ...)                                                  \
    do {                                                                                           \
        if (narrow_index(st, pitch, n)) { using I = unsigned; FLUID_BY_STORAGE(st, __VA_ARGS__); } \
        else { using I = size_t; FLUID_BY_STORAGE(st, __VA_ARGS__); }                              \
    } while (0)

static inline unsigned stride_blocks(int pitch, int row_lo, int row_hi)
{
    return (unsigned)std::clamp<size_t>(((size_t)(row_hi - row_lo) * (pitch >> 2) + 255) / 256, 1, 8192);
}

void launch_set_bnd(hipStream_t s, int st, void* f, int pitch, int n, int b, Members mb)
{
    FLUID_BY_STORAGE(st, hipLaunchKernelGGL(k_set_bnd<S>, dim3(cdiv(n, 256), mb.count), dim3(256), 0, s, (S*)f, pitch, n, b, mb.stride));
}

void launch_add_source(hipStream_t s, int st, void* x, const void* src, int pitch, int row_lo, int row_hi, float dt, Members mb,
                       const float* mdt)
{
    const dim3 grid(stride_blocks(pitch, row_lo, row_hi), mb.count);
    if (!src) {
        FLUID_BY_STORAGE(st, hipLaunchKernelGGL(k_add_zero_source<S>, grid, dim3(256), 0, s, (S*)x, pitch, row_lo, row_hi, dt, mb.stride, mdt));
        return;
    }
    FLUID_BY_STORAGE(st, hipLaunchKernelGGL(k_add_source<S>, grid, dim3(256), 0, s, (S*)x, (const S*)src, pitch, row_lo, row_hi, dt, mb.stride,
                                            mdt));
}

void launch_scale(hipStream_t s, int st, void* x, int pitch, int row_lo, int row_hi, float factor, Members mb)
{
    FLUID_BY_STORAGE(st, hipLaunchKernelGGL(k_scale<S>, dim3(stride_blocks(pitch, row_lo, row_hi), mb.count), dim3(256), 0, s, (S*)x, pitch,
                                            row_lo, row_hi, factor, mb.stride));
}

void launch_jacobi(hipStream_t s, int st, int variant, const void* x, const void* x0, void* out, int pitch, int n,
                   int row_lo, int row_hi, float alpha, float beta, int b, Members mb, const float2* mab)
{
    const int rows = row_hi - row_lo;
    if (rows <= 0) return;
    switch (variant) {
    case JACOBI_NAIVE:
        FLUID_BY_STORAGE(st, hipLaunchKernelGGL(k_jacobi_naive<S>, dim3(cdiv(n, 64), cdiv(rows, 4), mb.count), dim3(256), 0, s,
                                                (const S*)x, (const S*)x0, (S*)out, pitch, n, row_lo, row_hi, alpha,
                                                beta, b, mb.stride, mab));
        break;
    case JACOBI_LDS:
        FLUID_BY_STORAGE(st, hipLaunchKernelGGL(k_jacobi_lds<S>, dim3(cdiv(n, LT_X), cdiv(rows, LT_Y), mb.count), dim3(256), 0, s,
                                                (const S*)x, (const S*)x0, (S*)out, pitch, n, row_lo, row_hi, alpha,
                                                beta, b, mb.stride, mab));
        break;
    default: {
        constexpr int RB = 8;
        const unsigned nvec = (n + 3) / 4;
        FLUID_BY_STORAGE(st, hipLaunchKernelGGL((k_jacobi_stream<RB, S>), dim3(cdiv(nvec, 256), cdiv(rows, RB), mb.count), dim3(256),
                                                0, s, (const S*)x, (const S*)x0, (S*)out, pitch, n, row_lo, row_hi,
                                                alpha, beta, b, mb.stride, mab));
    }
    }
}

using TbKernel = void (*)(TbBatch, int, int, int, int, int, int, TbGrid, int);
template <typename S, size_t... I>
static std::array<TbKernel, kTbShapeCount> tb_kernels(std::index_sequence<I...>)
{
    return {&k_jacobi_tb<kTbShapes[I].T, kTbShapes[I].divmode, kTbShapes[I].nv, S, kTbShapes[I].form == TB_DIVSRC,
                         kTbShapes[I].form == TB_ADDSRC>...};
}

bool launch_jacobi_tb(hipStream_t s, int st, int T, int divmode, int nv, int form, const TbBatch& batch, int pitch, int n, int row_lo,
                      int row_hi, int rb, int rb_edge, int hole_lo, int hole_hi, bool fill)
{
    static const auto f32 = tb_kernels<float>(std::make_index_sequence<kTbShapeCount>());
    static const auto f16 = tb_kernels<half_t>(std::make_index_sequence<kTbShapeCount>());
    const int shape = jacobi_tb_index(T, divmode, nv, form);
    if (shape < 0) return false;
    const int rows = row_hi - row_lo;
    if (rows <= 0 || batch.count <= 0 || batch.members <= 0) return true;
    if (hole_lo < row_lo) hole_lo = row_lo;
    if (hole_hi > row_hi) hole_hi = row_hi;
    const bool hole = hole_lo < hole_hi;
    if (hole && hole_lo == row_lo && hole_hi == row_hi) return true;
    const int HL = (T + nv - 1) / nv, VS = 64 - 2 * HL;
    const unsigned nvec = (n + nv - 1) / nv;
    rb_edge = rb_edge < 1 ? rb : (rb_edge > rb ? rb : rb_edge);
    const int nwin = (int)cdiv(nvec, VS), kg = n / nv;
    int first_right = nwin - 1;
    while (first_right > 1 && kg < (first_right - 1) * VS - HL + 64) --first_right;
    if (first_right < 1) first_right = 1;
    TbGrid g;
    g.first_right = first_right;
    g.inner_wins = first_right - 1;
    g.edge_wins = 1 + (nwin - first_right);
    auto strips = [&](int r) { return hole ? cdiv(hole_lo - row_lo, r) + cdiv(row_hi - hole_hi, r) : cdiv(rows, r); };
    g.hole_lo = hole ? hole_lo : 0;
    g.hole_hi = hole ? hole_hi : 0;
    g.inner_blocks = g.inner_wins * (int)cdiv(strips(rb), 4);
    g.edge_blocks = g.edge_wins * (int)cdiv(strips(rb_edge), 4);
    const dim3 grid(8 * cdiv(g.inner_blocks + g.edge_blocks, 8), 1, batch.count * batch.members), block(256);
    const TbKernel k = (st == STORAGE_F16 ? f16 : f32)[shape];
    hipLaunchKernelGGL(k, grid, block, 0, s, batch, pitch, n, row_lo, row_hi, rb, rb_edge, g, fill ? 1 : 0);
    return true;
}

void launch_tile_min_abs(hipStream_t s, int st, const TileBatch& tiles, int count, int pitch, int n, int row_lo, int row_hi, int tile_pitch,
                         Members mb, size_t tile_mstride)
{
    if (row_lo < 1) row_lo = 1;
    if (row_hi > n + 1) row_hi = n + 1;
    if (row_hi <= row_lo || count <= 0) return;
    const int tr0 = (row_lo - 1) / kTileRows, tr1 = (row_hi - 2) / kTileRows;
    const dim3 grid(cdiv(cdiv(n, 4), 256), tr1 - tr0 + 1, count * mb.count);
    TileBatch tb = tiles;
    tb.count = count;
    tb.mstride = mb.stride;
    tb.tile_mstride = tile_mstride;
    FLUID_BY_STORAGE(st, hipLaunchKernelGGL(k_tile_min_abs<S>, grid, dim3(256), 0, s, tb, pitch, n, row_lo, row_hi, tr0, tile_pitch));
}

void launch_validate_div(hipStream_t s, int divmode, float beta, float kbeta, double yd, float hi, float lo, unsigned long long* bad)
{
    DivK k;
    k.beta = kbeta;
    k.yd = yd;
    k.hi = hi;
    k.lo = lo;
    const auto f = divmode == 4 ? k_validate_div<4> : divmode == 5 ? k_validate_div<5> : divmode == 3 ? k_validate_div<3> : k_validate_div<2>;
    hipLaunchKernelGGL(f, dim3(8192), dim3(256), 0, s, beta, k, bad);
}

void launch_advect(hipStream_t s, int st, void* d, const void* d0, const void* u, const void* v, int pitch, int n,
                   int row_lo, int row_hi, float dt0, int b, Members mb, const float* mdt0)
{
    if (row_hi <= row_lo) return;
    const dim3 grid(cdiv(n, 1024), row_hi - row_lo, mb.count);
    FLUID_BY_STORAGE_INDEX(st, pitch, n, hipLaunchKernelGGL((k_advect<S, I>), grid, dim3(256), 0, s, (S*)d, (const S*)d0, (const S*)u,
                                                            (const S*)v, pitch, n, row_lo, row_hi, dt0, b, mb.stride, mdt0));
}

void launch_advect2(hipStream_t s, int st, void* da, const void* d0a, int ba, void* db, const void* d0b, int bb, const void* u,
                    const void* v, int pitch, int n, int row_lo, int row_hi, float dt0, Members mb, const float* mdt0)
{
    if (row_hi <= row_lo) return;
    const dim3 grid(cdiv(n, 1024), row_hi - row_lo, mb.count);
    FLUID_BY_STORAGE_INDEX(st, pitch, n, hipLaunchKernelGGL((k_advect2<S, I>), grid, dim3(256), 0, s, (S*)da, (const S*)d0a, ba, (S*)db,
                                                            (const S*)d0b, bb, (const S*)u, (const S*)v, pitch, n, row_lo, row_hi, dt0, mb.stride,
                                                            mdt0));
}

void launch_divergence(hipStream_t s, int st, const void* u, const void* v, void* p, void* div, int pitch, int n,
                       int row_lo, int row_hi, float h, int write_p, float pscale, Members mb)
{
    if (row_hi <= row_lo) return;
    FLUID_BY_STORAGE(st, hipLaunchKernelGGL(k_divergence<S>, dim3(cdiv(n, 256), row_hi - row_lo, mb.count), dim3(256), 0, s,
                                            (const S*)u, (const S*)v, (S*)p, (S*)div, pitch, n, row_lo, row_hi, h,
                                            write_p, pscale, mb.stride));
}

void launch_subtract_gradient(hipStream_t s, int st, void* u, void* v, const void* p, int pitch, int n, int row_lo,
                              int row_hi, float h, float* partials, unsigned int* max_out, float pinv, Members mb)
{
    if (row_hi <= row_lo) return;
    if (max_out && mb.count == 1) {
        const unsigned per_col = cdiv(n, 256), rows = (unsigned)(row_hi - row_lo);
        const unsigned gy = std::max(1u, std::min(rows, (unsigned)kMaxPartials / per_col));
        FLUID_BY_STORAGE(st, hipLaunchKernelGGL(k_subtract_gradient_max<S>, dim3(per_col, gy), dim3(256), 0, s, (S*)u, (S*)v,
                                                (const S*)p, pitch, n, row_lo, row_hi, h, partials, pinv));
        hipLaunchKernelGGL(k_max_partials, dim3(1), dim3(256), 0, s, partials, (int)(per_col * gy), max_out);
        return;
    }
    FLUID_BY_STORAGE(st, hipLaunchKernelGGL(k_subtract_gradient<S>, dim3(cdiv(n, 256), row_hi - row_lo, mb.count), dim3(256), 0, s,
                                            (S*)u, (S*)v, (const S*)p, pitch, n, row_lo, row_hi, h, pinv, mb.stride));
}

void launch_gradient_advect(hipStream_t s, int st, void* u, void* v, const void* p, void* d, const void* d0, int pitch, int n,
                            int row_lo, int row_hi, float h, float dt0, int b, float pinv, Members mb, const float* mdt0)
{
    if (row_hi <= row_lo) return;
    const dim3 grid(cdiv(n, 1024), row_hi - row_lo, mb.count);
    FLUID_BY_STORAGE_INDEX(st, pitch, n, hipLaunchKernelGGL((k_gradient_advect<S, I>), grid, dim3(256), 0, s, (S*)u, (S*)v, (const S*)p,
                                                            (S*)d, (const S*)d0, pitch, n, row_lo, row_hi, h, dt0, b, pinv, mb.stride,
                                                            mdt0));
}

void launch_absmax2(hipStream_t s, int st, const void* u, const void* v, int pitch, int n, int row_lo, int row_hi,
                    unsigned int* result, Members mb, int rstride)
{
    if (row_hi <= row_lo) return;
    const unsigned blocks = (unsigned)(row_hi - row_lo) < 1024u ? (unsigned)(row_hi - row_lo) : 1024u;
    FLUID_BY_STORAGE(st, hipLaunchKernelGGL(k_absmax2<S>, dim3(blocks, mb.count), dim3(256), 0, s, (const S*)u, (const S*)v, pitch,
                                            n, row_lo, row_hi, result, mb.stride, rstride));
}

void launch_residual(hipStream_t s, int st, const void* x, const void* x0, int pitch, int n, int row_lo, int row_hi,
                     float alpha, float beta, unsigned int* result, Members mb, int rstride, const float2* mab)
{
    if (row_hi <= row_lo) return;
    const unsigned blocks = (unsigned)(row_hi - row_lo) < 1024u ? (unsigned)(row_hi - row_lo) : 1024u;
    FLUID_BY_STORAGE(st, hipLaunchKernelGGL(k_residual<S>, dim3(blocks, mb.count), dim3(256), 0, s, (const S*)x, (const S*)x0, pitch,
                                            n, row_lo, row_hi, alpha, beta, result, mb.stride, rstride, mab));
}

int moment_blocks(int n, int members)
{
    return std::max(1, std::min(n, kMomentBlocks / std::max(1, members)));
}

void launch_member_moments(hipStream_t s, int st, const void* x, int pitch, int n, Members mb, double2* partials, double2* out)
{
    const int blocks = moment_blocks(n, mb.count);
    FLUID_BY_STORAGE(st, hipLaunchKernelGGL(k_member_moments<S>, dim3(blocks, mb.count), dim3(256), 0, s, (const S*)x, pitch, n, mb.stride,
                                            partials));
    hipLaunchKernelGGL(k_fold_moments, dim3(mb.count), dim3(64), 0, s, partials, blocks, out);
}

static inline unsigned gram_chunks(int n, int mp)
{
    const int ch = kGramChunkValues / mp;
    return (unsigned)n * (unsigned)((n + ch - 1) / ch);
}

int gram_blocks(int n, int members)
{
    const int mp = gram_padded(members);
    return (int)std::min<unsigned>(gram_chunks(n, mp), mp == 64 ? 512u : 1024u);
}

void launch_member_gram(hipStream_t s, int st, const void* x, int pitch, int n, Members mb, float inv, bool centre, double* partials,
                        double* out)
// ... 104 lines not shown
```

### fluidsimulationcuda_amd/csrc/fluid_solver.hip

```cpp
#include <hip/hip_runtime.h>

#include <algorithm>
#include <cmath>
#include <cstdarg>
#include <cstdio>
#include <cstring>
#include <functional>
#include <mutex>
#include <new>
#include <string>
#include <unordered_map>
#include <vector>

#include "fluid_ctx.h"

namespace fluid_detail {

thread_local std::string g_err;

int fail(int code, const char* fmt, ...)
{
    char buf[512];
    va_list ap;
    va_start(ap, fmt);
// ... 104 lines not shown
        r.live.erase(r.live.begin() + (ptrdiff_t)k);
    }
    std::memcpy(r.host + lo, data, len);
    HIP_TRY(hipMemcpyAsync(r.dev + lo, r.host + lo, len, hipMemcpyHostToDevice, c->stream));
    hipEvent_t ev = r.free_events.back();
    r.free_events.pop_back();
    HIP_TRY(hipEventRecord(ev, c->stream));
    r.live.push_back({lo, len, hash, ev});
    r.head = hi;
    *dev = r.dev + lo;
    return FLUID_OK;
}

int member_pairs(fluid_ctx* c, const MemberVal& alpha, const MemberVal& beta, const float2** dev)
{
    *dev = nullptr;
    if (alpha.uniform() && beta.uniform()) return FLUID_OK;
    std::vector<float2> ab(c->members);
    for (int m = 0; m < c->members; ++m) ab[m] = make_float2(alpha.at(m), beta.at(m));
    const void* p = nullptr;
    TRY(member_consts(c, ab.data(), ab.size() * sizeof ab[0], &p));
    *dev = static_cast<const float2*>(p);
    return FLUID_OK;
}

int member_floats(fluid_ctx* c, const MemberVal& v, const float** dev)
{
    *dev = nullptr;
    if (v.uniform()) return FLUID_OK;
    const void* p = nullptr;
    TRY(member_consts(c, v.values().data(), v.values().size() * sizeof(float), &p));
    *dev = static_cast<const float*>(p);
    return FLUID_OK;
}

unsigned stream_bit(const fluid_ctx* c) { return c->stream2 && c->stream == c->stream2 ? 2u : 1u; }

int xchg_join(fluid_ctx* c)
{
    if (!(c->xowed & stream_bit(c))) return FLUID_OK;
    HIP_TRY(hipStreamWaitEvent(c->stream, c->ev_xdone, 0));
    c->xowed &= ~stream_bit(c);
    return FLUID_OK;
}

int call_exchange(fluid_ctx* c, int kind, const int* ids, int count, int depth, float* scalar, bool async = false)
{
    TRY(xchg_join(c));
    if (!async || !c->xstream || !c->xchg_overlap) return c->xchg(c->xchg_user, kind, ids, count, depth, scalar);
    HIP_TRY(hipEventRecord(c->ev_xbegin, c->stream));
    HIP_TRY(hipStreamWaitEvent(c->xstream, c->ev_xbegin, 0));
    hipStream_t compute = c->stream;
    c->stream = c->xstream;
    const int rc = c->xchg(c->xchg_user, kind, ids, count, depth, scalar);
    c->stream = compute;
    if (rc != 0) return rc;
    HIP_TRY(hipEventRecord(c->ev_xdone, c->xstream));
    c->xowed = 3u;
    return 0;
}

int exchange(fluid_ctx* c, int kind, std::initializer_list<int> fields, int depth, float* scalar = nullptr)
{
    if (c->nranks == 1 && !c->rccl) return FLUID_OK;
    if (!c->xchg) return fail(FLUID_E_COMM, "multi-GPU context without an exchange callback");
    std::vector<int> ids(fields);
    std::sort(ids.begin(), ids.end());
    ids.erase(std::unique(ids.begin(), ids.end()), ids.end());
    const int rc = call_exchange(c, kind, ids.data(), (int)ids.size(), depth, scalar);
    if (rc != 0) return fail(FLUID_E_COMM, "exchange callback failed (kind %d, rc %d)", kind, rc);
    return FLUID_OK;
}

int reduce_to_host(fluid_ctx* c, float* out)
{
    HIP_TRY(hipMemcpyAsync(c->h_scalar, c->d_scalar, sizeof(unsigned), hipMemcpyDeviceToHost, c->stream));
    HIP_TRY(hipStreamSynchronize(c->stream));
    float v;
    std::memcpy(&v, c->h_scalar, sizeof v);
    *out = v;
    return FLUID_OK;
}

int timing_begin(fluid_ctx* c, int cat, hipEvent_t* stop_out)
{
    *stop_out = nullptr;
    if (!c->timing) return FLUID_OK;
    if (c->ev_used == c->ev_pool.size()) {
        fluid_ctx::Ev e{};
        HIP_TRY(hipEventCreate(&e.a));
        HIP_TRY(hipEventCreate(&e.b));
        c->ev_pool.push_back(e);
    }
    auto& p = c->ev_pool[c->ev_used++];
    p.cat = cat;
    p.pressure = cat == FLUID_TIME_DIFFUSION && c->in_pressure_solve;
    HIP_TRY(hipEventRecord(p.a, c->stream));
    *stop_out = p.b;
    return FLUID_OK;
}

int timing_end(fluid_ctx* c, hipEvent_t stop, int sweeps)
{
    if (!stop) return FLUID_OK;
    HIP_TRY(hipEventRecord(stop, c->stream));
    c->pending_sweeps += sweeps;
    if (c->in_pressure_solve) c->pending_pressure_sweeps += sweeps;
    return FLUID_OK;
}

int timing_collect(fluid_ctx* c)
{
    if (c->ev_used == 0) return FLUID_OK;
    HIP_TRY(hipStreamSynchronize(c->stream));
    if (c->stream2) HIP_TRY(hipStreamSynchronize(c->stream2));
    for (size_t k = 0; k < c->ev_used; ++k) {
        float ms = 0.f;
        HIP_TRY(hipEventElapsedTime(&ms, c->ev_pool[k].a, c->ev_pool[k].b));
        c->cat_ms[c->ev_pool[k].cat] += ms;
        c->cat_calls[c->ev_pool[k].cat] += 1;
        if (c->ev_pool[k].pressure) c->pressure_ms += ms;
    }
    c->sweeps += c->pending_sweeps;
    c->pending_sweeps = 0;
    c->pressure_sweeps += c->pending_pressure_sweeps;
    c->pending_pressure_sweeps = 0;
    c->ev_used = 0;
    return FLUID_OK;
}

#define TIMED(c, cat, stmt)                      \
    do {                                         \
        hipEvent_t stop_;                        \
        TRY(timing_begin((c), (cat), &stop_));   \
        stmt;                                    \
        TRY(timing_end((c), stop_, 0));          \
    } while (0)

struct DivProofs {
    std::mutex mu;
    std::unordered_map<unsigned long long, int> proven;
};
DivProofs& div_proofs()
{
    static DivProofs p;
    return p;
}

struct DivPlan {
    int mode = 0;
    float arg = 0.f;
    float hi = 0.f, lo = 0.f;
    unsigned tile_thr = 0;
    double yd = 0.0;
};

float round_down_to_float(double v)
{
    float f = (float)v;
    if ((double)f > v) f = std::nextafterf(f, -INFINITY);
    return f;
}

DivPlan division_mode(fluid_ctx* c, float beta, float alpha, int force = 0)
{
    DivPlan plan;
    plan.arg = beta;
    plan.yd = 1.0 / (double)beta;
    if (c->fast_div == 0 || !(beta > 0.f) || !std::isfinite(beta)) return plan;
    int e2 = 0;
    const float rbeta = 1.0f / beta;
    const bool pow2 = std::frexp(beta, &e2) == 0.5f && std::isnormal(rbeta) && rbeta * beta == 1.0f;
    const float hi = round_down_to_float(plan.yd), lo = (float)(plan.yd - (double)hi);
    const bool two_term = c->fast_div == 1 && c->tiles && beta >= 1.0f && beta <= 0x1p24f && std::isnormal(hi) && std::isnormal(lo) && lo > 0.f;
    const bool residual = c->fast_div == 2 && beta >= 0x1p-60f && beta <= 0x1p60f;
    const float r5_hi = beta * 0x1p24f, r5_lo = -(rbeta * 0x1p-24f);
    int want = force ? force : (pow2 && alpha == 1.0f) ? 4 : two_term ? 3 : residual ? 5 : 2;
    unsigned bits;
    std::memcpy(&bits, &beta, sizeof bits);
    int dev = 0;
    (void)hipGetDevice(&dev);
    DivProofs& proofs = div_proofs();
    std::lock_guard<std::mutex> lock(proofs.mu);
    int mode = 0;
    while (want != 0) {
        const unsigned long long key = ((unsigned long long)(dev & 0xFF) << 40) | ((unsigned long long)want << 32) | bits;
        auto it = proofs.proven.find(key);
        if (it != proofs.proven.end()) {
            mode = it->second;
        } else {
            unsigned long long* bad = reinterpret_cast<unsigned long long*>(c->d_scalar) + 1;
            unsigned long long* hbad = reinterpret_cast<unsigned long long*>(c->h_scalar) + 1;
            if (hipMemsetAsync(bad, 0, sizeof *bad, c->stream) != hipSuccess) return plan;
            fluid::launch_validate_div(c->stream, want, beta, (want == 4 || want == 5) ? rbeta : beta, plan.yd, want == 5 ? r5_hi : hi,
                                       want == 5 ? r5_lo : lo, bad);
            if (hipMemcpyAsync(hbad, bad, sizeof *bad, hipMemcpyDeviceToHost, c->stream) != hipSuccess ||
                hipStreamSynchronize(c->stream) != hipSuccess)
                return plan;
            mode = *hbad == 0 ? want : 0;
            proofs.proven.emplace(key, mode);
        }
        if (mode != 0) break;
        want = want == 2 ? 0 : 2;
    }
    plan.mode = mode;
    if (mode == 4 || mode == 5) plan.arg = rbeta;
    if (mode == 5) {
        plan.hi = r5_hi;
        plan.lo = r5_lo;
    }
    if (mode == 3) {
        plan.hi = hi;
        plan.lo = lo;
        const float thr = beta * 0x1p-72f;
        std::memcpy(&plan.tile_thr, &thr, sizeof thr);
    }
    return plan;
}

constexpr int kEverywhere = 1 << 28;

int exchange_cap(const fluid_ctx* c) { return c->min_slab - 1; }

void wrote(fluid_ctx* c, int f, int reach)
{
    c->field[f].reach = c->nranks > 1 ? reach : kEverywhere;
    c->field[f].zero = false;
    c->field[f].pend = false;
    c->field[f].src_of = 0;
    c->field[f].fscale = 1.0f;
}

void trade(fluid_ctx* c, int a, int b) { std::swap(c->field[a], c->field[b]); }

int need_list(fluid_ctx* c, const std::vector<int>& fields, int reach, bool async = false)
{
    if (c->nranks == 1 || reach <= 0) return FLUID_OK;
    if (reach > exchange_cap(c)) return fail(FLUID_E_COMM, "halo of %d rows exceeds the slab height", reach);
    std::vector<int> ids;
    for (int f : fields)
        if (c->field[f].reach < reach) ids.push_back(f);
    if (ids.empty()) return FLUID_OK;
    if (!c->xchg) return fail(FLUID_E_COMM, "multi-GPU context without an exchange callback");
    std::sort(ids.begin(), ids.end());
    ids.erase(std::unique(ids.begin(), ids.end()), ids.end());
    c->in_halo_exchange = true;
    const int rc = call_exchange(c, FLUID_XCHG_HALO, ids.data(), (int)ids.size(), reach, nullptr, async);
    c->in_halo_exchange = false;
    if (rc != 0) return fail(FLUID_E_COMM, "halo exchange failed (rc %d)", rc);
    for (int f : ids) c->field[f].reach = reach;
    return FLUID_OK;
}

int need(fluid_ctx* c, std::initializer_list<int> fields, int reach, bool async = false)
{
    return need_list(c, std::vector<int>(fields), reach, async);
}

void rows(const fluid_ctx* c, int reach, int* lo, int* hi)
{
    *lo = std::max(1, c->own0 - reach);
    *hi = std::min(c->n + 1, c->own1 + reach);
}

void rows_with_walls(const fluid_ctx* c, int reach, int* lo, int* hi)
{
    rows(c, reach, lo, hi);
    if (*lo == 1) *lo = 0;
    if (*hi == c->n + 1) *hi = c->n + 2;
}

int settle_source(fluid_ctx* c, int f);

int unscale(fluid_ctx* c, int f)
{
    if (c->field[f].fscale == 1.0f) return FLUID_OK;
    const float inv = 1.0f / c->field[f].fscale;
    c->field[f].fscale = 1.0f;
    if (c->field[f].zero) return FLUID_OK;
    fluid::launch_scale(c->stream, c->st, c->ptr(f), c->pitch, 0, c->n + 2, inv, c->mb());
    return FLUID_OK;
}

int add_source_now(fluid_ctx* c, int x, const void* src, int lo, int hi, const MemberVal& amount)
{
    const float* per_member = nullptr;
    TRY(member_floats(c, amount, &per_member));
    TIMED(c, FLUID_TIME_SOURCE,
          fluid::launch_add_source(c->stream, c->st, c->ptr(x), src, c->pitch, lo, hi, amount.at(0), c->mb(), per_member));
    return FLUID_OK;
}

int settle(fluid_ctx* c, int f, bool keep_scale = false)
{
    if (!keep_scale) TRY(unscale(c, f));
    if (c->field[f].src_of) return settle_source(c, f);
    if (!c->field[f].pend) return FLUID_OK;
    const int reach = c->nranks > 1 ? std::min(c->field[f].reach, exchange_cap(c)) : 0;
    int lo, hi;
    rows_with_walls(c, reach, &lo, &hi);
    TRY(add_source_now(c, f, nullptr, lo, hi, c->field[f].pend_inc));
    c->field[f].pend = false;
    return FLUID_OK;
}

int settle_source(fluid_ctx* c, int f)
{
    if (!c->field[f].src_of) return FLUID_OK;
    const int s = c->field[f].src_of - 1;
    const int reach = c->nranks > 1 ? std::min({c->field[f].reach, c->field[s].reach, exchange_cap(c)}) : 0;
    int lo, hi;
    rows_with_walls(c, reach, &lo, &hi);
    TRY(add_source_now(c, f, c->ptr(s), lo, hi, c->field[f].src_dt));
    wrote(c, f, reach);
    return FLUID_OK;
}

int materialize(fluid_ctx* c, int f, bool keep_scale = false)
{
    TRY(materialize_zero(c, f));
    return settle(c, f, keep_scale);
}

int materialize(fluid_ctx* c, std::initializer_list<int> fs)
{
    for (int f : fs) TRY(materialize(c, f));
    return FLUID_OK;
}

void mark_zero(fluid_ctx* c, int f) { wrote(c, f, kEverywhere); c->field[f].zero = true; }

int op_add_source(fluid_ctx* c, int x, int s, const MemberVal& dt, bool defer = false)
{
    const int reach = c->nranks > 1 ? std::min({c->field[x].reach, c->field[s].reach, exchange_cap(c)}) : 0;
    int lo, hi;
    rows_with_walls(c, reach, &lo, &hi);
    TRY(materialize(c, x));
    if (c->field[s].zero) {
        volatile float z = 0.0f;
        const MemberVal inc = dt.map([&](float d) { return d * z; });
        if (c->variant == fluid::JACOBI_TB && c->defer_zero_source) {
            c->field[x].pend = true;
            c->field[x].pend_inc = inc;
            return FLUID_OK;
        }
        TRY(add_source_now(c, x, nullptr, lo, hi, inc));
    } else {
        TRY(settle(c, s));
        if (defer && c->fuse_add_source && c->variant == fluid::JACOBI_TB && fluid::jacobi_tb_exists(-1, -1, c->tb_nv, fluid::TB_ADDSRC)) {
            c->field[x].src_of = 1 + s;
            c->field[x].src_dt = dt;
            return FLUID_OK;
        }
        TRY(add_source_now(c, x, c->ptr(s), lo, hi, dt));
    }
    wrote(c, x, reach);
    return FLUID_OK;
}

struct RbTuner {
    struct Entry {
        std::vector<int> cand;
        std::vector<float> best_ms;
        std::vector<int> samples, issued;
        int fixed = 0;
        std::string what;
// ... 53 lines not shown
            }
        }
        c->free_events.push_back(tr.a);
        c->free_events.push_back(tr.b);
    }
    c->trials.resize(keep);
}

int tune_pick(fluid_ctx* c, unsigned long long key, int heuristic, int T, long long rows_n, int* trial, int solves = 0, int form = 0, int divmode = 0)
{
    *trial = -1;
    tune_harvest(c);
    RbTuner& t = rb_tuner();
    std::lock_guard<std::mutex> lock(t.mu);
    RbTuner::Entry& e = t.table[key];
    if (e.fixed) return e.fixed;
    if (e.cand.empty()) {
        char what[96];
        snprintf(what, sizeof what, "N=%d T=%d solves=%d members=%d form=%d divmode=%d rows=%lld", c->n, T, solves, c->members, form, divmode, rows_n);
        e.what = what;
        e.cand.push_back(heuristic);
        for (int r : {48, 56, 64, 80, 96, 112, 128, 160, 192}) {
            if (r < T || r >= rows_n + 2 * T) continue;
            if (std::find(e.cand.begin(), e.cand.end(), r) == e.cand.end()) e.cand.push_back(r);
        }
        if (rows_n > 2200)
            for (int r : {32, 40})
                if (r >= T && std::find(e.cand.begin(), e.cand.end(), r) == e.cand.end()) e.cand.push_back(r);
        if (rows_n <= 2200)
            for (int r : {2, 4, 8, 12, 24, 32, 40})
                if (r < rows_n && std::find(e.cand.begin(), e.cand.end(), r) == e.cand.end()) e.cand.push_back(r);
        if (e.cand.size() == 1) {
            e.fixed = heuristic;
            return heuristic;
        }
        e.best_ms.assign(e.cand.size(), 0.f);
        e.samples.assign(e.cand.size(), 0);
        e.issued.assign(e.cand.size(), 0);
    }
    const int pick = (int)(std::min_element(e.issued.begin(), e.issued.end()) - e.issued.begin());
    if (e.issued[pick] >= kTuneSamples + 2) return e.cand[0];
    e.issued[pick] += 1;
    *trial = pick;
    return e.cand[pick];
}

int tune_begin(fluid_ctx* c, unsigned long long key, int trial)
{
    fluid_ctx::Trial tr{};
    tr.key = key;
    tr.cand = trial;
    for (hipEvent_t* ev : {&tr.a, &tr.b}) {
        if (!c->free_events.empty()) {
            *ev = c->free_events.back();
            c->free_events.pop_back();
        } else {
            HIP_TRY(hipEventCreate(ev));
        }
    }
    HIP_TRY(hipEventRecord(tr.a, c->stream));
    c->trials.push_back(tr);
    return FLUID_OK;
}

int tune_end(fluid_ctx* c)
{
    HIP_TRY(hipEventRecord(c->trials.back().b, c->stream));
    return FLUID_OK;
}

struct SweepShape {
    bool canonical, small;
    long long slab_cells;
};

SweepShape sweep_shape(const fluid_ctx* c, int count)
{
    const bool canonical = c->st == fluid::STORAGE_F16;
    const long long slab_cells = (long long)(c->nranks > 1 ? c->min_slab : c->n) * c->n;
    return {canonical, (canonical ? (long long)c->n * c->n : slab_cells * count) < c->tb_min_cells, slab_cells};
}

int pick_sweeps(const fluid_ctx* c, int remaining, int room, const SweepShape& shape, bool all_mode4)
{
    const long long slab_cells = shape.slab_cells;
    if (c->variant != fluid::JACOBI_TB || shape.small || c->field_bytes >= 0x7F000000ull) return 1;
    room = std::min(room, remaining);
    const int greedy = (room >= 8 && c->tb_max_t >= 8) ? 8 : (room >= 4 && c->tb_max_t >= 4) ? 4 : room >= 2 ? 2 : 1;
    if (shape.canonical || !fluid::jacobi_tb_exists(12, -1, c->tb_nv, fluid::TB_PLAIN) || c->tb_max_t < 12 || room < 12 || (remaining & 1)) return greedy;
    const bool forced = c->tb_t16_min_cells >= 0;
    const bool big = forced ? slab_cells >= c->tb_t16_min_cells : slab_cells >= (8ll << 20);
    if (!big) return greedy;
    const long long slab_rows = slab_cells / std::max(c->n, 1);
    const bool pays16 = forced || ((all_mode4 || (unsigned long long)slab_cells * c->esz > (96ull << 20)) && slab_rows >= 3000);
    const int* depth = fluid::kTbDepths;
    constexpr int nd = (int)std::size(fluid::kTbDepths);
    static const double per_sweep[] = {1.00, 1.04, 1.30, 2.6, 5.0};
    static_assert(std::size(per_sweep) == nd, "one cost per depth");
    const double per_launch = 0.5;
    bool allowed[nd];
    for (int k = 0; k < nd; ++k)
        allowed[k] = depth[k] <= c->tb_max_t && (depth[k] != 16 || pays16) && fluid::jacobi_tb_exists(depth[k], -1, c->tb_nv, fluid::TB_PLAIN);
    std::vector<double> cost(remaining + 1, 1e300);
    cost[0] = 0.0;
    for (int r = 2; r <= remaining; r += 2)
        for (int k = 0; k < nd; ++k) {
            if (!allowed[k] || depth[k] > r) continue;
            const double v = cost[r - depth[k]] + depth[k] * per_sweep[k] + per_launch;
            if (v < cost[r] - 1e-9) cost[r] = v;
        }
    int best = 0;
    for (int r = remaining; r > 0;) {
        int pickd = 0;
        for (int k = 0; k < nd && !pickd; ++k)
            if (allowed[k] && depth[k] <= r && std::fabs(cost[r - depth[k]] + depth[k] * per_sweep[k] + per_launch - cost[r]) < 1e-9)
                pickd = depth[k];
        if (!pickd) break;
        if (pickd <= room) best = std::max(best, pickd);
        r -= pickd;
    }
    return best ? best : greedy;
}

struct Coeffs {
    MemberVal alpha, beta;
};

struct Solve {
    int b, x, x0;
    const Coeffs* k;
};

struct DivSource {
    int u, v;
    float scale;
};

struct Batch {
    const Solve* sv;
    int count, iters, final_reach;
    const DivSource* ds;
    int scratch_base;
    const int* scratch;
    const int* sum;
    int cur[3], nxt[3];
    std::vector<DivPlan> plan[3];
    bool same_mode, all_mode4, add_src;
    float out_scale[3];
    SweepShape shape;
};

size_t tile_words(const fluid_ctx* c) { return (size_t)fluid::tile_rows(c->n) * fluid::tile_pitch(c->n); }
unsigned* solve_tiles(const fluid_ctx* c, int slot) { return c->tiles + (size_t)slot * c->members * tile_words(c); }

void plan_members(fluid_ctx* c, const Coeffs& k, std::vector<DivPlan>& out)
{
    const int M = c->members;
    const MemberVal &alpha = k.alpha, &beta = k.beta;
    out.resize(M);
    bool same = true;
    for (int m = 0; m < M; ++m) {
        out[m] = (m > 0 && beta.at(m) == beta.at(m - 1) && alpha.at(m) == alpha.at(m - 1)) ? out[m - 1] : division_mode(c, beta.at(m), alpha.at(m));
        same = same && out[m].mode == out[0].mode;
    }
    if (same) return;
    bool all2 = true;
    for (int m = 0; m < M; ++m) {
        out[m] = division_mode(c, beta.at(m), alpha.at(m), 2);
        all2 = all2 && out[m].mode == 2;
    }
    if (all2) return;
    for (int m = 0; m < M; ++m) {
        out[m] = DivPlan{};
        out[m].arg = beta.at(m);
        out[m].yd = 1.0 / (double)beta.at(m);
    }
}

int batch_prepare(fluid_ctx* c, Batch& B)
{
    static const int kScratch[3] = {FLUID_TMP0, FLUID_TMP1, FLUID_TMP2};
    static const int kSum[3] = {FLUID_TMP3, FLUID_TMP4, FLUID_TMP5};
    const Solve* sv = B.sv;
    if (B.scratch_base < 0 || B.scratch_base + B.count > 3) return fail(FLUID_E_INVALID, "a batch holds 1 to 3 solves");
    B.scratch = kScratch + B.scratch_base;
    B.sum = kSum + B.scratch_base;
    TRY(check_iters(B.iters));
    if (B.count < 1 || B.count > 3) return fail(FLUID_E_INVALID, "a batch holds 1 to 3 solves");
    for (int k = 0; k < B.count; ++k) {
        if (sv[k].x == sv[k].x0 || sv[k].x >= FLUID_TMP0 || sv[k].x0 >= FLUID_TMP0)
            return fail(FLUID_E_INVALID, "diffuse: x and x0 must be distinct non-scratch fields");
        for (int j = 0; j < k; ++j)
            if (sv[j].x == sv[k].x || sv[j].x == sv[k].x0 || sv[j].x0 == sv[k].x)
                return fail(FLUID_E_INVALID, "diffuse: the solves of a batch must not share fields");
    }
    for (int k = 0; k < B.count; ++k) {
        const FieldState &x = c->field[sv[k].x], &x0 = c->field[sv[k].x0];
        if ((x.zero ? x0.fscale : x.fscale) != x0.fscale || x0.src_of) {
            if (x.fscale != 1.0f || x0.fscale != 1.0f) TRY(xchg_join(c));
            TRY(unscale(c, sv[k].x));
            TRY(unscale(c, sv[k].x0));
        }
        B.out_scale[k] = x0.fscale;
    }
    if (B.iters == 0) {
        TRY(xchg_join(c));
        for (int k = 0; k < B.count; ++k) TRY(settle_source(c, sv[k].x0));
        return FLUID_OK;
    }
    for (int k = 0; k < B.count; ++k) TRY(materialize_zero(c, sv[k].x0));
    for (int k = 0; k < B.count; ++k)
        if (c->field[sv[k].x].pend) {
            TRY(xchg_join(c));
            TRY(settle(c, sv[k].x, true));
        }
    return FLUID_OK;
}

int batch_plan(fluid_ctx* c, Batch& B)
{
    const Solve* sv = B.sv;
    B.same_mode = B.all_mode4 = true;
    for (int k = 0; k < B.count; ++k) {
        B.cur[k] = sv[k].x;
        B.nxt[k] = B.scratch[k];
        const Coeffs& co = *sv[k].k;
        if (k > 0 && sv[k].k == sv[k - 1].k) {
            B.plan[k] = B.plan[k - 1];
        } else if (c->variant != fluid::JACOBI_TB) {
            B.plan[k].assign(1, DivPlan{});
            B.plan[k][0].arg = co.beta.at(0);
        } else if (co.alpha.uniform() && co.beta.uniform()) {
            B.plan[k].assign(1, division_mode(c, co.beta.at(0), co.alpha.at(0)));
        } else {
            plan_members(c, co, B.plan[k]);
        }
        B.same_mode = B.same_mode && B.plan[k][0].mode == B.plan[0][0].mode;
        B.all_mode4 = B.all_mode4 && B.plan[k][0].mode == 4;
    }
    B.shape = sweep_shape(c, B.count);
    const FieldState& x00 = c->field[sv[0].x0];
    bool add_src = x00.src_of != 0 && B.ds == nullptr && B.same_mode;
    for (int k = 0; k < B.count; ++k) {
        const FieldState &x = c->field[sv[k].x], &x0 = c->field[sv[k].x0];
        add_src = add_src && x0.src_of == 1 + sv[k].x && x0.src_dt == x00.src_dt && !x.zero && !x.pend && !x.src_of;
    }
    B.add_src = add_src && fluid::jacobi_tb_exists(pick_sweeps(c, B.iters, B.iters, B.shape, B.all_mode4), B.plan[0][0].mode, c->tb_nv, fluid::TB_ADDSRC);
    if (!B.add_src)
        for (int k = 0; k < B.count; ++k)
            if (c->field[sv[k].x0].src_of) {
                TRY(xchg_join(c));
                TRY(settle_source(c, sv[k].x0));
            }
    fluid::TileBatch tb{};
    int m = 0, valid = kEverywhere;
    for (int k = 0; k < B.count; ++k)
        if (B.plan[k][0].mode == 3) {
            tb.field[m] = c->ptr(sv[k].x0);
            tb.tiles[m] = solve_tiles(c, B.scratch_base + k);
            valid = std::min(valid, c->nranks > 1 ? c->field[sv[k].x0].reach : kEverywhere);
            ++m;
        }
    if (m == 0) return FLUID_OK;
    TRY(xchg_join(c));
    if (c->nranks > 1)
        HIP_TRY(hipMemsetAsync(solve_tiles(c, B.scratch_base), 0, (size_t)B.count * c->members * tile_words(c) * sizeof(unsigned), c->stream));
    int lo, hi;
    rows(c, std::min(valid, c->n), &lo, &hi);
    fluid::launch_tile_min_abs(c->stream, c->st, tb, m, c->pitch, c->n, lo, hi, fluid::tile_pitch(c->n), c->mb(), tile_words(c));
    return FLUID_OK;
}

int batch_reach(const fluid_ctx* c, const Batch& B)
{
    int r = kEverywhere;
    for (int k = 0; k < B.count; ++k) r = std::min(r, std::min(c->field[B.cur[k]].reach, c->field[B.sv[k].x0].reach + 1));
    return r;
}

fluid::TbMemberK solve_constants(const Batch& B, int j, int m, const MemberVal& x0_inc, const MemberVal& div_scale)
{
    const DivPlan& p = B.plan[j][B.plan[j].size() > 1 ? (size_t)m : 0];
    return {p.yd, B.sv[j].k->alpha.at(m), p.arg, p.hi, p.lo, x0_inc.at(m), div_scale.at(m), p.tile_thr, 0};
}

int fill_batch(fluid_ctx* c, const Batch& B, int first, int last, bool divsrc, bool addsrc, fluid::TbBatch* out)
{
    static const MemberVal nothing_pending(-0.0f);
    const MemberVal own_scale(divsrc ? B.ds->scale : 0.0f);
    const MemberVal& div_scale = addsrc ? c->field[B.sv[first].x0].src_dt : own_scale;
    const MemberVal* x0_inc[3];
    fluid::TbBatch bt{};
    bool per_member = !div_scale.uniform();
    for (int j = first; j < last; ++j) {
        const int q = j - first;
        const FieldState& x0 = c->field[B.sv[j].x0];
        x0_inc[q] = x0.pend && !addsrc && !divsrc ? &x0.pend_inc : &nothing_pending;
        per_member = per_member || B.plan[j].size() > 1 || !x0_inc[q]->uniform();
        const fluid::TbMemberK k0 = solve_constants(B, j, 0, *x0_inc[q], div_scale);
        bt.x[q] = c->ptr(B.cur[j]);
        bt.x0[q] = x0.ptr;
        bt.out[q] = c->ptr(B.nxt[j]);
        bt.alpha[q] = k0.alpha;
        bt.beta[q] = k0.beta;
        bt.yd[q] = k0.yd;
        bt.hi[q] = k0.hi;
        bt.lo[q] = k0.lo;
        bt.tiles[q] = B.plan[j][0].mode == 3 ? solve_tiles(c, B.scratch_base + j) : nullptr;
        bt.tile_thr[q] = k0.tile_thr;
        bt.b[q] = B.sv[j].b;
        bt.x_zero[q] = c->field[B.cur[j]].zero ? 1 : 0;
        bt.x0_inc[q] = k0.x0_inc;
        if (addsrc) bt.div[q] = c->ptr(B.sum[j]);
    }
    bt.count = last - first;
    bt.members = c->members;
    bt.mstride = c->field_floats;
    bt.tile_mstride = tile_words(c);
    bt.tile_pitch = fluid::tile_pitch(c->n);
    bt.div_scale = div_scale.at(0);
    if (divsrc) {
        bt.x[0] = c->ptr(B.ds->u);
        bt.x0[0] = c->ptr(B.ds->v);
        bt.div[0] = c->ptr(B.sv[0].x0);
    }
    if (per_member && c->members > 1) {
        const int M = c->members;
        std::vector<fluid::TbMemberK> rec((size_t)bt.count * M);
        for (int j = first; j < last; ++j)
            for (int m = 0; m < M; ++m) rec[(size_t)(j - first) * M + m] = solve_constants(B, j, m, *x0_inc[j - first], div_scale);
        const void* dev = nullptr;
        TRY(member_consts(c, rec.data(), rec.size() * sizeof rec[0], &dev));
        bt.mk = static_cast<const fluid::TbMemberK*>(dev);
    }
    *out = bt;
    return FLUID_OK;
}

int edge_rows(const fluid_ctx* c, int T, int rb) { return std::max(2 * T, rb * (c->tb_edge_pct > 0 ? c->tb_edge_pct : 100) / 100); }

int strip_rows(const fluid_ctx* c, int T, int m, long long rows_n)
{
    const int nv = c->tb_nv;
    const int HL = (T + nv - 1) / nv, VS = 64 - 2 * HL;
    const long long windows = ((c->n + nv - 1) / nv + VS - 1) / VS;
    const long long inner = windows > 2 ? windows - 2 : 0, outer = windows - inner;
    const int resident = nv == 2 ? (T >= 16 ? 2 : 4) : (T >= 8 ? 2 : 3);
    const long long room = (long long)c->num_cu * resident * 92 / 100;
    const int cap = T >= 16 ? 192 : (T >= 8 ? 80 : 96) * (m > 1 ? 2 : 1);
    int rb = c->tb_fill ? T : 2 * T;
    auto fits = [&](int r) {
        const long long si = (rows_n + r - 1) / r, se = (rows_n + edge_rows(c, T, r) - 1) / edge_rows(c, T, r);
        return (inner * ((si + 3) / 4) + outer * ((se + 3) / 4)) * m <= room;
    };
    for (; rb < cap; rb += 2)
        if (fits(rb)) break;
    if (rows_n <= 1100) {
        const int low = std::max(2, std::min(rb, (int)(rows_n / 64) & ~1));
        if (c->members == 1 || fits(low)) rb = low;
        else rb = (int)std::min<long long>(rb, std::max<long long>(low, (rows_n + 1) & ~1ll));
    }
    return rb;
}

int launch_fused(fluid_ctx* c, const fluid::TbBatch& bt, int T, int divmode, bool divsrc, bool addsrc, int lo, int hi)
{
    const bool owed = c->nranks > 1 && (c->xowed & stream_bit(c));
    const int in_lo = owed && c->rank > 0 ? std::max(lo, c->own0 + T) : lo;
    const int in_hi = owed && c->rank < c->nranks - 1 ? std::min(hi, c->own1 - T) : hi;
    const bool split = owed && in_hi - in_lo >= 2 * T && (in_lo > lo || in_hi < hi);
    const int form = divsrc ? fluid::TB_DIVSRC : addsrc ? fluid::TB_ADDSRC : fluid::TB_PLAIN;
    for (int part = split ? 0 : 1; part < 2; ++part) {
        const int plo = part ? lo : in_lo, phi = part ? hi : in_hi;
        const int hole_lo = part && split ? in_lo : 0, hole_hi = part && split ? in_hi : 0;
        if (part) TRY(xchg_join(c));
        const long long rows_n = (phi - plo) - std::max(0, hole_hi - hole_lo);
        int rb = c->tb_rows > 0 ? c->tb_rows : strip_rows(c, T, bt.count * c->members, rows_n);
        int trial = -1;
        unsigned long long key = 0;
        if (c->tb_rows <= 0 && c->autotune) {
            key = tune_key(c, T, bt.count + (divsrc ? 8 : 0) + (addsrc ? 16 : 0) + (hole_hi > hole_lo ? 32 : 0), divmode, rows_n);
            rb = tune_pick(c, key, rb, T, rows_n, &trial, bt.count, form, divmode);
        }
        if (trial >= 0) TRY(tune_begin(c, key, trial));
        if (!fluid::launch_jacobi_tb(c->stream, c->st, T, divmode, c->tb_nv, form, bt, c->pitch, c->n, plo, phi, rb,
                                     std::min(rb, edge_rows(c, T, rb)), hole_lo, hole_hi, c->tb_fill))
            return fail(FLUID_E_INVALID, "no fused Jacobi kernel: %d sweeps, division mode %d, %d-column lanes, form %d", T, divmode, c->tb_nv, form);
        if (trial >= 0) TRY(tune_end(c));
    }
    if (split) c->split_launches += 1;
    return FLUID_OK;
}

void commit_launch(fluid_ctx* c, Batch& B, bool first, int r)
{
    if (B.ds && first && c->nranks > 1)
        c->field[B.sv[0].x0].reach = std::max(0, std::min(c->field[B.sv[0].x0].reach, r));
    if (B.add_src && first) {
        for (int j = 0; j < B.count; ++j) {
            trade(c, B.sv[j].x0, B.sum[j]);
            wrote(c, B.sum[j], 0);
            wrote(c, B.sv[j].x0, std::max(0, r));
        }
        B.add_src = false;
    }
    for (int j = 0; j < B.count; ++j) {
        c->field[B.cur[j]].zero = false;
        wrote(c, B.nxt[j], r);
        std::swap(B.cur[j], B.nxt[j]);
    }
}

int batch_sweep(fluid_ctx* c, Batch& B)
{
    const Solve* sv = B.sv;
    const bool multi = c->nranks > 1, canonical = B.shape.canonical;
    int r = multi ? batch_reach(c, B) : kEverywhere;
    for (int k = 0; k < B.iters;) {
        const int remaining = B.iters - k;
        const int wantT = canonical ? pick_sweeps(c, remaining, remaining, B.shape, B.all_mode4) : 1;
        if (r < wantT) {
            const int depth = std::max(wantT, std::min(c->halo, remaining + B.final_reach));
            std::vector<int> ids;
            for (int j = 0; j < B.count; ++j) {
                ids.push_back(B.cur[j]);
                if (c->field[sv[j].x0].reach < depth - 1) ids.push_back(sv[j].x0);
            }
            TRY(xchg_join(c));
            TRY(need_list(c, ids, depth, true));
            r = batch_reach(c, B);
        }
        const int T = canonical ? wantT : pick_sweeps(c, remaining, std::min(r, remaining), B.shape, B.all_mode4);
        if (B.add_src && k == 0 && !fluid::jacobi_tb_exists(T, B.plan[0][0].mode, c->tb_nv, fluid::TB_ADDSRC)) {
            B.add_src = false;
            TRY(xchg_join(c));
            for (int j = 0; j < B.count; ++j) TRY(settle_source(c, sv[j].x0));
        }
        int lo, hi;
        rows(c, multi ? std::min(r - T, exchange_cap(c)) : 0, &lo, &hi);
        if (T == 1) {
            const int v = c->variant == fluid::JACOBI_TB ? (B.shape.small ? fluid::JACOBI_NAIVE : fluid::JACOBI_STREAM) : c->variant;
            TRY(xchg_join(c));
            for (int j = 0; j < B.count; ++j) TRY(materialize(c, B.cur[j], true));
            for (int j = 0; j < B.count; ++j) TRY(settle(c, sv[j].x0, true));
            for (int j = 0; j < B.count; ++j) {
                const float2* mab = nullptr;
                TRY(member_pairs(c, sv[j].k->alpha, sv[j].k->beta, &mab));
                fluid::launch_jacobi(c->stream, c->st, v, c->ptr(B.cur[j]), c->ptr(sv[j].x0), c->ptr(B.nxt[j]), c->pitch, c->n, lo, hi,
                                     sv[j].k->alpha.at(0), sv[j].k->beta.at(0), sv[j].b, c->mb(), mab);
            }
            if (c->timing) {
                c->launches += B.count;
                c->field_launches += (long long)B.count * c->members;
            }
        } else {
            for (int first = 0, last; first < B.count; first = last) {
                last = B.same_mode ? B.count : first + 1;
                const bool divsrc = B.ds != nullptr && k == 0, addsrc = B.add_src && k == 0;
                fluid::TbBatch bt;
                TRY(fill_batch(c, B, first, last, divsrc, addsrc, &bt));
                TRY(launch_fused(c, bt, T, B.plan[first][0].mode, divsrc, addsrc, lo, hi));
                if (c->timing) {
                    c->launches += 1;
                    c->field_launches += (long long)(last - first) * c->members;
                }
            }
        }
        r = multi ? std::min(r - T, exchange_cap(c)) : kEverywhere;
        commit_launch(c, B, k == 0, r);
        k += T;
    }
    return FLUID_OK;
}

int op_diffuse_batch(fluid_ctx* c, const Solve* sv, int count, int iters, int final_reach = 0, const DivSource* ds = nullptr,
                     int scratch_base = 0)
{
    Batch B{sv, count, iters, final_reach, ds, scratch_base};
    TRY(batch_prepare(c, B));
    if (iters == 0) return FLUID_OK;
    hipEvent_t stop;
    TRY(timing_begin(c, FLUID_TIME_DIFFUSION, &stop));
    TRY(batch_plan(c, B));
    TRY(batch_sweep(c, B));
    HIP_TRY(hipGetLastError());
    for (int j = 0; j < count; ++j) {
        if (B.cur[j] != sv[j].x) trade(c, sv[j].x, B.scratch[j]);
        wrote(c, B.scratch[j], 0);
        c->field[sv[j].x].fscale = B.out_scale[j];
    }
    return timing_end(c, stop, iters * count * c->members);
}

int op_diffuse(fluid_ctx* c, int b, int x, int x0, const Coeffs& k, int iters, int final_reach = 0, const DivSource* ds = nullptr)
{
    const Solve one{b, x, x0, &k};
    return op_diffuse_batch(c, &one, 1, iters, final_reach, ds);
}

int vmax_begin(fluid_ctx* c, int u, int v, bool have_max = false)
{
    if (c->nranks == 1) return FLUID_OK;
    if (!have_max) {
        TRY(materialize(c, {u, v}));
        HIP_TRY(hipMemsetAsync(c->d_scalar, 0, sizeof(unsigned), c->stream));
        fluid::launch_absmax2(c->stream, c->st, c->ptr(u), c->ptr(v), c->pitch, c->n, c->own0, c->own1, c->d_scalar, c->mb());
    }
    TRY(exchange(c, FLUID_XCHG_MAX_BEGIN, {}, 0));
    HIP_TRY(hipMemcpyAsync(c->h_scalar, c->d_scalar, sizeof(unsigned), hipMemcpyDeviceToHost, c->stream));
    HIP_TRY(hipEventRecord(c->scalar_ready, c->stream));
    return FLUID_OK;
}

int advect_rows(fluid_ctx* c, std::initializer_list<int> sources, float dt0, int have, float* vmax, bool* fetched)
{
    HIP_TRY(hipEventSynchronize(c->scalar_ready));
    std::memcpy(vmax, c->h_scalar, sizeof *vmax);
    TRY(exchange(c, FLUID_XCHG_MAX_END, {}, 0, vmax));
    const double reach = std::ceil((double)std::fabs(dt0) * (double)*vmax) + 2.0;
    *fetched = !(have > 0 && reach <= (double)have);
    if (!*fetched) return FLUID_OK;
    if (reach <= (double)exchange_cap(c)) return need(c, sources, (int)reach);
    TRY(exchange(c, FLUID_XCHG_GATHER, sources, 0));
    for (int f : sources) c->field[f].reach = kEverywhere;
    return FLUID_OK;
}

int advect_bounded(fluid_ctx* c, int slot, std::initializer_list<int> sources, float dt0, const std::function<int()>& run)
{
    if (c->nranks == 1) return run();
    int guess = 0;
    const float prev = c->vmax_prev[slot];
    if (c->early_advect && prev >= 0.0f) {
        const double g = std::ceil((double)std::fabs(dt0) * (double)prev * 1.25) + 2.0;
        if (g <= (double)exchange_cap(c)) {
            guess = (int)g;
            TRY(need(c, sources, guess));
            TRY(run());
        }
    }
    float vmax = 0.f;
    bool fetched = false;
    TRY(advect_rows(c, sources, dt0, guess, &vmax, &fetched));
    c->vmax_prev[slot] = std::isfinite(vmax) ? vmax : -1.0f;
    return fetched ? run() : FLUID_OK;
}

int member_dt0(fluid_ctx* c, const MemberVal& dt, const float** dev)
{
    return member_floats(c, dt.map([&](float d) { return d * (float)c->n; }), dev);
}

int op_advect(fluid_ctx* c, int b, int d, int d0, int u, int v, const MemberVal& dt)
{
    if (d == d0 || d == u || d == v) return fail(FLUID_E_INVALID, "advect: output must not alias an input");
    const float dt0 = dt.at(0) * (float)c->n;
    TRY(materialize(c, {d0, u, v}));
    const float* mdt0 = nullptr;
    TRY(member_dt0(c, dt, &mdt0));
    TIMED(c, FLUID_TIME_ADVECTION,
          fluid::launch_advect(c->stream, c->st, c->ptr(d), c->ptr(d0), c->ptr(u), c->ptr(v), c->pitch, c->n, c->own0, c->own1, dt0, b, c->mb(),
                               mdt0));
    wrote(c, d, 0);
    return FLUID_OK;
}

int op_advect2(fluid_ctx* c, int ba, int da, int d0a, int bb, int db, int d0b, int u, int v, const MemberVal& dt)
{
    for (int d : {da, db})
        if (d == d0a || d == d0b || d == u || d == v) return fail(FLUID_E_INVALID, "advect: output must not alias an input");
    if (da == db) return fail(FLUID_E_INVALID, "advect: outputs must be distinct");
    const float dt0 = dt.at(0) * (float)c->n;
    TRY(materialize(c, {d0a, d0b, u, v}));
    const float* mdt0 = nullptr;
    TRY(member_dt0(c, dt, &mdt0));
    TIMED(c, FLUID_TIME_ADVECTION,
          fluid::launch_advect2(c->stream, c->st, c->ptr(da), c->ptr(d0a), ba, c->ptr(db), c->ptr(d0b), bb, c->ptr(u), c->ptr(v), c->pitch,
                                c->n, c->own0, c->own1, dt0, c->mb(), mdt0));
    wrote(c, da, 0);
    wrote(c, db, 0);
    return FLUID_OK;
}

int op_divergence(fluid_ctx* c, int u, int v, int p, int div, int want = 0, float pscale = 1.0f)
{
    if (p == u || p == v || div == u || div == v || p == div)
        return fail(FLUID_E_INVALID, "divergence: outputs must not alias inputs");
    const float h = 1.0f / (float)c->n;
    int reach = 0;
    TRY(materialize(c, {u, v}));
    if (c->nranks > 1) {
        reach = std::max(0, std::min(want, exchange_cap(c) - 1));
        TRY(need(c, {u, v}, reach + 1));
    }
    int lo, hi;
    rows(c, reach, &lo, &hi);
    TIMED(c, FLUID_TIME_DIVERGENCE,
          fluid::launch_divergence(c->stream, c->st, c->ptr(u), c->ptr(v), c->ptr(p), c->ptr(div), c->pitch, c->n, lo, hi, h,
                                   0, pscale, c->mb()));
    wrote(c, div, reach);
    c->field[div].fscale = pscale;
    mark_zero(c, p);
    return FLUID_OK;
}

int op_subtract_gradient(fluid_ctx* c, int u, int v, int p, bool with_max = false)
{
    if (p == u || p == v || u == v) return fail(FLUID_E_INVALID, "subtract_gradient: fields must be distinct");
    const float h = 1.0f / (float)c->n;
    TRY(materialize(c, {u, v}));
    TRY(materialize(c, p, true));
    TRY(need(c, {p}, 1));
    with_max = with_max && c->nranks > 1 && c->d_partials;
    TIMED(c, FLUID_TIME_PROJECTION,
// ... 214 lines not shown
    }
    std::vector<fluid::half_t> stage(rows * w);
    const size_t hp = w * sizeof(fluid::half_t);
    if (to_device) {
        const float* src = chost + (size_t)row_lo * w;
        for (size_t k = 0; k < rows * w; ++k) stage[k] = (fluid::half_t)src[k];
        HIP_TRY(hipMemcpy2DAsync(dev, dp, stage.data(), hp, hp, rows, hipMemcpyHostToDevice, c->stream));
        HIP_TRY(hipStreamSynchronize(c->stream));
    } else {
        HIP_TRY(hipMemcpy2DAsync(stage.data(), hp, dev, dp, hp, rows, hipMemcpyDeviceToHost, c->stream));
        HIP_TRY(hipStreamSynchronize(c->stream));
        float* dst = host + (size_t)row_lo * w;
        for (size_t k = 0; k < rows * w; ++k) dst[k] = (float)stage[k] * host_scale;
    }
    return FLUID_OK;
}

struct CachedCtx {
    fluid_ctx* c = nullptr;
    ~CachedCtx();
};
thread_local CachedCtx g_cached_holder;
#define g_cached (g_cached_holder.c)

}

extern "C" {

const char* fluid_last_error(void) { return g_err.c_str(); }

int fluid_coefficients(int N, float dt, float coef, float* alpha, float* beta)
{
    if (N < 1 || !alpha || !beta) return fail(FLUID_E_INVALID, "fluid_coefficients: bad argument");
    coefficients(N, dt, coef, alpha, beta);
    return FLUID_OK;
}

int fluid_layout(int N, int* pitch, int* xoff, size_t* field_floats)
{
    if (N < 1 || N > kMaxN) return fail(FLUID_E_INVALID, "N must be in [1, %d] (got %d)", kMaxN, N);
    const int p = fluid::pitch_for(N);
    if (pitch) *pitch = p;
    if (xoff) *xoff = XOFF;
    if (field_floats) *field_floats = (size_t)(N + 2) * p;
    return FLUID_OK;
}

size_t fluid_arena_bytes_ensemble(int N, int storage, int members)
{
    size_t ff = 0;
    if (fluid_layout(N, nullptr, nullptr, &ff) != FLUID_OK) return 0;
    if (storage != FLUID_STORAGE_F32 && storage != FLUID_STORAGE_F16) return 0;
    if (members < 1 || members > kMaxMembers) return 0;
    return ff * FLUID_NFIELDS * fluid::storage_bytes(storage) * (size_t)members + kControlBytes;
}

size_t fluid_arena_bytes_ex(int N, int storage) { return fluid_arena_bytes_ensemble(N, storage, 1); }

size_t fluid_arena_bytes(int N) { return fluid_arena_bytes_ex(N, FLUID_STORAGE_F32); }

int fluid_create_ex(const fluid_config* cfg, fluid_ctx** out) { return fluid_create_ensemble(cfg, 1, out); }

int fluid_create_ensemble(const fluid_config* cfg, int members, fluid_ctx** out)
{
    if (!cfg || !out) return fail(FLUID_E_INVALID, "fluid_create_ex / fluid_create_ensemble: null argument");
    *out = nullptr;
    if (members < 1 || members > kMaxMembers) return fail(FLUID_E_INVALID, "members must be in [1, %d] (got %d)", kMaxMembers, members);
    if (members > 1 && cfg->nranks > 1) return fail(FLUID_E_INVALID, "an ensemble runs on one GPU: nranks must be 1 (got %d)", cfg->nranks);
    const int n = cfg->n;
    if (n < 1 || n > kMaxN) return fail(FLUID_E_INVALID, "N must be in [1, %d] (got %d)", kMaxN, n);
    const int P = cfg->nranks < 1 ? 1 : cfg->nranks;
    if (cfg->rank < 0 || cfg->rank >= P) return fail(FLUID_E_INVALID, "rank %d outside [0,%d)", cfg->rank, P);
    if (cfg->jacobi_variant < 0 || cfg->jacobi_variant >= fluid::JACOBI_VARIANTS)
        return fail(FLUID_E_INVALID, "unknown Jacobi variant %d", cfg->jacobi_variant);
    if (cfg->storage != FLUID_STORAGE_F32 && cfg->storage != FLUID_STORAGE_F16)
        return fail(FLUID_E_INVALID, "unknown storage type %d", cfg->storage);
    if (P > 1 && n / P < 2) return fail(FLUID_E_INVALID, "N=%d is too small for %d row slabs (need >= 2 rows each)", n, P);
    fluid_ctx* c = new (std::nothrow) fluid_ctx;
    if (!c) return fail(FLUID_E_NOMEM, "out of host memory");
    c->n = n;
    c->w = n + 2;
    c->pitch = fluid::pitch_for(n);
    c->field_floats = (size_t)c->w * c->pitch;
    c->members = members;
    c->st = cfg->storage;
    c->esz = fluid::storage_bytes(c->st);
    c->field_bytes = c->field_floats * c->esz;
    c->variant = cfg->jacobi_variant;
    if (c->st == fluid::STORAGE_F16 && n >= 16) {
        int e = 0;
        (void)std::frexp((float)n, &e);
        c->pscale = std::ldexp(1.0f, e - 3);
    }
    c->rank = cfg->rank;
    c->nranks = P;
    const int base = n / P, rem = n % P;
    c->own0 = 1 + cfg->rank * base + std::min(cfg->rank, rem);
    c->own1 = c->own0 + base + (cfg->rank < rem ? 1 : 0);
    c->min_slab = base;
    const int want = cfg->halo > 0 ? cfg->halo : std::max(4, std::min(42, base / 8));
    c->halo = P > 1 ? std::max(1, std::min(want, base - 1)) : 1;
    if (P > 1 && cfg->storage == FLUID_STORAGE_F16) {
        if (base - 1 < 8) {
            delete c;
            return fail(FLUID_E_INVALID, "fp16 storage needs row slabs of at least 9 rows (N=%d over %d slabs gives %d)", n, P, base);
        }
        c->halo = std::max(c->halo, 8);
    }
    const size_t bytes = c->all_bytes() * FLUID_NFIELDS + kControlBytes;
    int rc = FLUID_OK;
    auto bail = [&](int code) { fluid_destroy(c); return code; };
    if (cfg->arena) {
        if (cfg->arena_bytes < bytes) return bail(fail(FLUID_E_INVALID, "arena too small: %zu < %zu", cfg->arena_bytes, bytes));
        if (((uintptr_t)cfg->arena & 255u) != 0) return bail(fail(FLUID_E_INVALID, "arena must be 256-byte aligned"));
        c->arena = (char*)cfg->arena;
    } else {
        hipError_t e = hipMalloc((void**)&c->arena, bytes);
        if (e != hipSuccess) return bail(fail(e == hipErrorOutOfMemory ? FLUID_E_NOMEM : FLUID_E_HIP, "hipMalloc(%zu): %s", bytes, hipGetErrorString(e)));
        c->own_arena = true;
    }
    if (cfg->stream) {
        c->stream = (hipStream_t)cfg->stream;
    } else {
        hipError_t e = hipStreamCreateWithFlags(&c->stream, hipStreamNonBlocking);
        if (e != hipSuccess) return bail(fail(FLUID_E_HIP, "hipStreamCreate: %s", hipGetErrorString(e)));
        c->own_stream = true;
    }
    for (int k = 0; k < FLUID_NFIELDS; ++k) c->field[k].ptr = c->arena + (size_t)k * c->all_bytes();
    auto hip_ok = [&](hipError_t e, const char* what) {
        if (e == hipSuccess) return true;
        rc = fail(e == hipErrorOutOfMemory ? FLUID_E_NOMEM : FLUID_E_HIP, "%s: %s", what, hipGetErrorString(e));
        return false;
    };
    {
        int dev = 0, cus = 0;
        if (hipGetDevice(&dev) == hipSuccess &&
            hipDeviceGetAttribute(&cus, hipDeviceAttributeMultiprocessorCount, dev) == hipSuccess && cus > 0)
            c->num_cu = cus;
    }
    if (P > 1) {
        if (!hip_ok(hipStreamCreateWithFlags(&c->stream2, hipStreamNonBlocking), "hipStreamCreate(second stream)")) return bail(rc);
        if (!hip_ok(hipEventCreateWithFlags(&c->ev_fork, hipEventDisableTiming), "hipEventCreate")) return bail(rc);
        if (!hip_ok(hipEventCreateWithFlags(&c->ev_join, hipEventDisableTiming), "hipEventCreate")) return bail(rc);
        if (!hip_ok(hipStreamCreateWithFlags(&c->xstream, hipStreamNonBlocking), "hipStreamCreate(exchange stream)")) return bail(rc);
        if (!hip_ok(hipEventCreateWithFlags(&c->ev_xbegin, hipEventDisableTiming), "hipEventCreate")) return bail(rc);
        if (!hip_ok(hipEventCreateWithFlags(&c->ev_xdone, hipEventDisableTiming), "hipEventCreate")) return bail(rc);
    }
    if (!hip_ok(hipMemsetAsync(c->arena, 0, bytes, c->stream), "hipMemsetAsync(arena)")) return bail(rc);
    c->d_scalar = reinterpret_cast<unsigned int*>(c->arena + c->all_bytes() * FLUID_NFIELDS);
    {
        const size_t words = 3 * (size_t)members * tile_words(c);
        if (!hip_ok(hipMalloc((void**)&c->tiles, words * sizeof(unsigned)), "hipMalloc(tiles)")) return bail(rc);
        if (!hip_ok(hipMemsetAsync(c->tiles, 0, words * sizeof(unsigned), c->stream), "hipMemsetAsync(tiles)")) return bail(rc);
    }
    if (P > 1 && !hip_ok(hipMalloc((void**)&c->d_partials, fluid::kMaxPartials * sizeof(float)), "hipMalloc(partials)")) return bail(rc);
    if (!hip_ok(hipHostMalloc((void**)&c->h_scalar, 256, hipHostMallocDefault), "hipHostMalloc")) return bail(rc);
    if (!hip_ok(hipEventCreateWithFlags(&c->scalar_ready, hipEventDisableTiming), "hipEventCreate")) return bail(rc);
    if (!hip_ok(hipStreamSynchronize(c->stream), "hipStreamSynchronize")) return bail(rc);
    *out = c;
    return FLUID_OK;
}

int fluid_create(int N, fluid_ctx** out)
{
    fluid_config cfg;
    std::memset(&cfg, 0, sizeof cfg);
    cfg.n = N;
    cfg.nranks = 1;
    cfg.jacobi_variant = FLUID_JACOBI_TB;
    return fluid_create_ex(&cfg, out);
}

int fluid_destroy(fluid_ctx* c)
{
    if (!c) return FLUID_OK;
    if (c->stream) (void)hipStreamSynchronize(c->stream);
    if (c->stream2) (void)hipStreamSynchronize(c->stream2);
    if (c->xstream) (void)hipStreamSynchronize(c->xstream);
    for (auto& p : c->ev_pool) {
        (void)hipEventDestroy(p.a);
        (void)hipEventDestroy(p.b);
    }
    if (!c->trials.empty()) {
        RbTuner& t = rb_tuner();
        std::lock_guard<std::mutex> lock(t.mu);
        for (auto& tr : c->trials) {
            auto it = t.table.find(tr.key);
            if (it != t.table.end() && !it->second.fixed && it->second.issued[tr.cand] > 0) it->second.issued[tr.cand] -= 1;
            (void)hipEventDestroy(tr.a);
            (void)hipEventDestroy(tr.b);
        }
    }
    for (hipEvent_t ev : c->free_events) (void)hipEventDestroy(ev);
    fluid_detail::rccl_release(c->rccl);
    c->rccl = nullptr;
    if (c->h_scalar) (void)hipHostFree(c->h_scalar);
    if (c->tiles) (void)hipFree(c->tiles);
    for (auto& b : c->consts.live) (void)hipEventDestroy(b.copied);
    for (hipEvent_t ev : c->consts.free_events) (void)hipEventDestroy(ev);
    if (c->consts.dev) (void)hipFree(c->consts.dev);
    if (c->consts.host) (void)hipHostFree(c->consts.host);
    if (c->red.d_max) (void)hipFree(c->red.d_max);
    if (c->red.d_moments) (void)hipFree(c->red.d_moments);
    if (c->red.d_partials) (void)hipFree(c->red.d_partials);
    if (c->red.host) (void)hipHostFree(c->red.host);
    if (c->red.d_mean) (void)hipFree(c->red.d_mean);
    if (c->red.d_var) (void)hipFree(c->red.d_var);
    if (c->red.d_gram_partials) (void)hipFree(c->red.d_gram_partials);
    if (c->red.d_gram) (void)hipFree(c->red.d_gram);
    if (c->red.gram_host) (void)hipHostFree(c->red.gram_host);
    if (c->stage.dev) (void)hipFree(c->stage.dev);
    for (hipEvent_t ev : c->xform.copied)
        if (ev) (void)hipEventDestroy(ev);
    if (c->xform.dev) (void)hipFree(c->xform.dev);
    if (c->xform.host) (void)hipHostFree(c->xform.host);
    if (c->d_partials) (void)hipFree(c->d_partials);
    if (c->scalar_ready) (void)hipEventDestroy(c->scalar_ready);
    if (c->own_arena && c->arena) (void)hipFree(c->arena);
    if (c->stream2) (void)hipStreamDestroy(c->stream2);
    if (c->xstream) (void)hipStreamDestroy(c->xstream);
    if (c->ev_xbegin) (void)hipEventDestroy(c->ev_xbegin);
    if (c->ev_xdone) (void)hipEventDestroy(c->ev_xdone);
    if (c->ev_fork) (void)hipEventDestroy(c->ev_fork);
    if (c->ev_join) (void)hipEventDestroy(c->ev_join);
    if (c->own_stream && c->stream) (void)hipStreamDestroy(c->stream);
    if (g_cached == c) g_cached = nullptr;
    delete c;
    return FLUID_OK;
}

int fluid_synchronize(fluid_ctx* c)
{
    TRY(check_ctx(c));
    HIP_TRY(hipStreamSynchronize(c->stream));
    return FLUID_OK;
}

int fluid_exchange_stream(fluid_ctx* c, void** stream)
{
    TRY(check_ctx(c));
    if (!stream) return fail(FLUID_E_INVALID, "null pointer");
    *stream = c->stream;
    return FLUID_OK;
}

int fluid_split_launches(fluid_ctx* c, long long* count)
{
    TRY(check_ctx(c));
    if (!count) return fail(FLUID_E_INVALID, "null pointer");
    *count = c->split_launches;
    return FLUID_OK;
}

int fluid_owned_rows(fluid_ctx* c, int* row_lo, int* row_hi)
{
    TRY(check_ctx(c));
    if (row_lo) *row_lo = c->own0;
    if (row_hi) *row_hi = c->own1;
    return FLUID_OK;
}

int fluid_field_ptr(fluid_ctx* c, int field, void** dev_ptr)
{
    TRY(check_ctx(c));
    TRY(check_fields(c, {field}));
    if (!dev_ptr) return fail(FLUID_E_INVALID, "null pointer");
    if (c->in_halo_exchange) TRY(materialize_zero(c, field));
    else TRY(materialize(c, field));
    *dev_ptr = c->ptr(field);
    return FLUID_OK;
}

int fluid_scalar_ptr(fluid_ctx* c, void** dev_ptr)
{
    TRY(check_ctx(c));
    if (!dev_ptr) return fail(FLUID_E_INVALID, "null pointer");
    *dev_ptr = c->d_scalar;
    return FLUID_OK;
}

int fluid_members(fluid_ctx* c, int* members)
{
    TRY(check_ctx(c));
    if (!members) return fail(FLUID_E_INVALID, "null pointer");
    *members = c->members;
    return FLUID_OK;
}

static int refuse_plain_copy(const fluid_ctx* c, const char* what)
{
    if (c->members > 1)
        return fail(FLUID_E_INVALID, "%s: this context has %d members -- use fluid_upload_member / fluid_download_member", what, c->members);
    return FLUID_OK;
}

static int check_member(const fluid_ctx* c, int member)
{
    if (member < 0 || member >= c->members) return fail(FLUID_E_INVALID, "member %d outside [0, %d)", member, c->members);
    return FLUID_OK;
}

int fluid_upload_member(fluid_ctx* c, int member, int field, const float* host)
{
    TRY(check_ctx(c));
    TRY(check_fields(c, {field}));
    TRY(check_member(c, member));
    if (!host) return fail(FLUID_E_INVALID, "null host pointer");
    return copy_rows(c, field, nullptr, host, 0, c->w, true, true, member);
}

int fluid_download_member(fluid_ctx* c, int member, int field, float* host)
{
    TRY(check_ctx(c));
    TRY(check_fields(c, {field}));
    TRY(check_member(c, member));
    if (!host) return fail(FLUID_E_INVALID, "null host pointer");
    return copy_rows(c, field, host, nullptr, 0, c->w, false, true, member);
}

int fluid_upload_rows(fluid_ctx* c, int field, const float* host, int row_lo, int row_hi)
{
    TRY(check_ctx(c));
    TRY(refuse_plain_copy(c, "fluid_upload_rows"));
    TRY(check_fields(c, {field}));
    if (!host) return fail(FLUID_E_INVALID, "null host pointer");
    return copy_rows(c, field, nullptr, host, row_lo, row_hi, true);
}

int fluid_download_rows(fluid_ctx* c, int field, float* host, int row_lo, int row_hi)
{
    TRY(check_ctx(c));
    TRY(refuse_plain_copy(c, "fluid_download_rows"));
    TRY(check_fields(c, {field}));
    if (!host) return fail(FLUID_E_INVALID, "null host pointer");
    return copy_rows(c, field, host, nullptr, row_lo, row_hi, false);
}

int fluid_upload(fluid_ctx* c, int field, const float* host)
{
    TRY(check_ctx(c));
    TRY(refuse_plain_copy(c, "fluid_upload"));
    return fluid_upload_rows(c, field, host, 0, c->w);
}

int fluid_download(fluid_ctx* c, int field, float* host)
{
    TRY(check_ctx(c));
    TRY(refuse_plain_copy(c, "fluid_download"));
    return fluid_download_rows(c, field, host, 0, c->w);
}

int fluid_fill(fluid_ctx* c, int field, float value)
{
    TRY(check_ctx(c));
    TRY(check_fields(c, {field}));
    if (value == 0.0f && !std::signbit(value)) {
        HIP_TRY(hipMemsetAsync(c->ptr(field), 0, c->all_bytes(), c->stream));
        wrote(c, field, kEverywhere);
        return FLUID_OK;
    }
    std::vector<float> row((size_t)c->w * c->w, value);
    for (int m = 0; m < c->members; ++m) TRY(fluid_upload_member(c, m, field, row.data()));
    wrote(c, field, kEverywhere);
    return FLUID_OK;
}

int fluid_set_jacobi_variant(fluid_ctx* c, int variant)
{
    TRY(check_ctx(c));
    if (variant < 0 || variant >= fluid::JACOBI_VARIANTS) return fail(FLUID_E_INVALID, "unknown Jacobi variant %d", variant);
    c->variant = variant;
    return FLUID_OK;
}

int fluid_set_param(fluid_ctx* c, int key, int value)
{
    TRY(check_ctx(c));
    switch (key) {
    case FLUID_PARAM_TB_MAX_SWEEPS:
        if (!fluid::is_tb_depth(value)) return fail(FLUID_E_INVALID, "TB_MAX_SWEEPS must be 16, 12, 8, 4 or 2");
        c->tb_max_t = value;
        return FLUID_OK;
    case FLUID_PARAM_TB_ROWS:
        if (value < 0) return fail(FLUID_E_INVALID, "TB_ROWS must be >= 0");
        c->tb_rows = value;
        return FLUID_OK;
    case FLUID_PARAM_TB_EDGE_ROWS_PCT:
        if (value < 0 || value > 100) return fail(FLUID_E_INVALID, "TB_EDGE_ROWS_PCT must be in [0,100]");
        c->tb_edge_pct = value;
        return FLUID_OK;
    case FLUID_PARAM_TB_MIN_CELLS:
        if (value < 0) return fail(FLUID_E_INVALID, "TB_MIN_CELLS must be >= 0");
        c->tb_min_cells = value;
        return FLUID_OK;
    case FLUID_PARAM_TB_FAST_DIVISION:
        if (value < 0 || value > 3) return fail(FLUID_E_INVALID, "TB_FAST_DIVISION must be 0, 1, 2 or 3");
        c->fast_div = value;
        return FLUID_OK;
    case FLUID_PARAM_TB_AUTOTUNE:
        c->autotune = value != 0;
        return FLUID_OK;
    case FLUID_PARAM_TB_FILL:
        c->tb_fill = value != 0;
        return FLUID_OK;
    case FLUID_PARAM_SLAB_OVERLAP:
        c->slab_overlap = value != 0;
        return FLUID_OK;
    case FLUID_PARAM_FUSE_DIVERGENCE:
        c->fuse_divergence = value != 0;
        return FLUID_OK;
    case FLUID_PARAM_EARLY_ADVECT:
        c->early_advect = value != 0;
        return FLUID_OK;
    case FLUID_PARAM_FUSE_ADD_SOURCE:
        c->fuse_add_source = value != 0;
        return FLUID_OK;
    case FLUID_PARAM_F16_PRESSURE_SCALE: {
        for (int f = 0; f < FLUID_NFIELDS; ++f) TRY(unscale(c, f));
        int e = 0;
        (void)std::frexp((float)c->n, &e);
        c->pscale = (value != 0 && c->st == fluid::STORAGE_F16 && c->n >= 16) ? std::ldexp(1.0f, e - 3) : 1.0f;
        return FLUID_OK;
    }
    case FLUID_PARAM_XCHG_OVERLAP:
        TRY(xchg_join(c));
        c->xchg_overlap = value != 0;
        return FLUID_OK;
    case FLUID_PARAM_TB_T16_MIN_CELLS:
        if (value < -1) return fail(FLUID_E_INVALID, "TB_T16_MIN_CELLS must be >= 0, or -1 for the default rule");
        c->tb_t16_min_cells = value;
        return FLUID_OK;
    case FLUID_PARAM_TB_LANE_COLUMNS:
        if (value != 2 && value != 4) return fail(FLUID_E_INVALID, "TB_LANE_COLUMNS must be 2 or 4");
        c->tb_nv = value;
        return FLUID_OK;
    case FLUID_PARAM_HALO:
        if (value < 1) return fail(FLUID_E_INVALID, "HALO must be >= 1");
        c->halo = c->nranks > 1 ? std::max(c->st == fluid::STORAGE_F16 ? 8 : 1, std::min(value, c->min_slab - 1)) : 1;
        return FLUID_OK;
    default:
        return fail(FLUID_E_INVALID, "unknown parameter %d", key);
    }
}

int fluid_plan_sweeps(int N, int rows, int storage, int pressure_form, int iters, int max_sweeps, int t16_min_cells, int* depths,
                      int capacity, int* count)
{
    if (N < 1 || N > kMaxN || rows < 1 || rows > N || iters < 0 || (iters & 1) || !depths || !count || capacity < 0)
        return fail(FLUID_E_INVALID, "fluid_plan_sweeps: bad argument");
    if (storage != FLUID_STORAGE_F32 && storage != FLUID_STORAGE_F16) return fail(FLUID_E_INVALID, "unknown storage type %d", storage);
    if (!fluid::is_tb_depth(max_sweeps)) return fail(FLUID_E_INVALID, "max_sweeps must be 16, 12, 8, 4 or 2");
    fluid_ctx c;
    c.n = N;
    c.st = storage;
    c.esz = fluid::storage_bytes(storage);
    c.field_bytes = (size_t)(N + 2) * fluid::pitch_for(N) * c.esz;
    c.tb_max_t = max_sweeps;
    c.tb_t16_min_cells = t16_min_cells;
    const SweepShape shape{storage == FLUID_STORAGE_F16, false, (long long)rows * N};
    int k = 0;
    for (int left = iters; left > 0;) {
        const int t = pick_sweeps(&c, left, left, shape, pressure_form != 0);
        if (k < capacity) depths[k] = t;
        ++k;
        left -= t;
    }
    *count = k;
    return FLUID_OK;
}

int fluid_autotune_pending(fluid_ctx* c, int* shapes_open)
{
    TRY(check_ctx(c));
    if (!shapes_open) return fail(FLUID_E_INVALID, "null pointer");
    tune_harvest(c);
    RbTuner& t = rb_tuner();
    std::lock_guard<std::mutex> lock(t.mu);
    int open = 0;
    for (auto& kv : t.table) open += kv.second.fixed ? 0 : 1;
    *shapes_open = open;
    return FLUID_OK;
}

int fluid_division_mode(fluid_ctx* c, float alpha, float beta, int* mode)
{
    TRY(check_ctx(c));
    if (!mode) return fail(FLUID_E_INVALID, "null pointer");
    *mode = c->variant == fluid::JACOBI_TB ? division_mode(c, beta, alpha).mode : 0;
    return FLUID_OK;
}

int fluid_set_exchange(fluid_ctx* c, fluid_exchange_fn fn, void* user)
{
    TRY(check_ctx(c));
    TRY(fluid_detail::refuse_ensemble(c, "fluid_set_exchange"));
    c->xchg = fn;
    c->xchg_user = user;
    return FLUID_OK;
}

int fluid_exchange_now(fluid_ctx* c, int kind, const int* fields, int nfields, int depth)
{
    TRY(check_ctx(c));
    TRY(fluid_detail::refuse_ensemble(c, "fluid_exchange_now"));
    if (!c->xchg) return fail(FLUID_E_COMM, "no exchange installed");
    if (kind != FLUID_XCHG_HALO && kind != FLUID_XCHG_GATHER) return fail(FLUID_E_INVALID, "fluid_exchange_now moves rows: HALO or GATHER");
    if (nfields < 0 || (nfields > 0 && !fields)) return fail(FLUID_E_INVALID, "bad field list");
    if (kind == FLUID_XCHG_HALO && c->nranks > 1 && (depth < 1 || depth > c->min_slab))
        return fail(FLUID_E_INVALID, "halo depth %d outside [1, %d] (the shortest slab)", depth, c->min_slab);
    for (int k = 0; k < nfields; ++k) {
        TRY(check_fields(c, {fields[k]}));
        TRY(settle(c, fields[k], true));
    }
    c->in_halo_exchange = true;
    const int rc = call_exchange(c, kind, fields, nfields, depth, nullptr);
    c->in_halo_exchange = false;
    if (rc != 0) return fail(FLUID_E_COMM, "exchange failed (kind %d, rc %d)", kind, rc);
    for (int k = 0; k < nfields; ++k)
        c->field[fields[k]].reach = kind == FLUID_XCHG_GATHER ? kEverywhere : std::max(c->field[fields[k]].reach, depth);
    return FLUID_OK;
}

struct MemberArg {
    const char* name;
    const float* v;
};

static int check_member_args(const fluid_ctx* c, const char* call, std::initializer_list<MemberArg> args)
{
    for (const MemberArg& a : args)
        if (!a.v) return fail(FLUID_E_INVALID, "%s: null array `%s`", call, a.name);
    if (!c) return fail(FLUID_E_INVALID, "%s: null context", call);
    for (const MemberArg& a : args)
        for (int m = 0; m < c->members; ++m)
            if (!std::isfinite(a.v[m])) return fail(FLUID_E_INVALID, "%s: member %d: %s is not finite (%g)", call, m, a.name, (double)a.v[m]);
    return FLUID_OK;
}

static int vel_step_body(fluid_ctx* c, const MemberVal& dt, const MemberVal& visc, int iters)
{
    TRY(check_ctx(c));
    TRY(check_iters(iters));
    TRY(vel_step(c, dt, visc, iters));
    HIP_TRY(hipGetLastError());
    return FLUID_OK;
}

int fluid_vel_step(fluid_ctx* c, float dt, float visc, int iters) { return vel_step_body(c, dt, visc, iters); }

int fluid_vel_step_members(fluid_ctx* c, const float* dt, const float* visc, int iters)
{
    TRY(check_member_args(c, "fluid_vel_step_members", {{"dt", dt}, {"visc", visc}}));
    if (c->members == 1) return fluid_vel_step(c, dt[0], visc[0], iters);
    TRY(ensure_consts(c));
    return vel_step_body(c, {dt, c->members}, {visc, c->members}, iters);
}

static int dens_step_body(fluid_ctx* c, const MemberVal& dt, const MemberVal& diff, int iters)
{
    TRY(check_ctx(c));
    TRY(check_iters(iters));
    TRY(dens_step(c, dt, diff, iters));
    HIP_TRY(hipGetLastError());
    return FLUID_OK;
}

int fluid_dens_step(fluid_ctx* c, float dt, float diff, int iters) { return dens_step_body(c, dt, diff, iters); }

int fluid_dens_step_members(fluid_ctx* c, const float* dt, const float* diff, int iters)
{
    TRY(check_member_args(c, "fluid_dens_step_members", {{"dt", dt}, {"diff", diff}}));
    if (c->members == 1) return fluid_dens_step(c, dt[0], diff[0], iters);
    TRY(ensure_consts(c));
    return dens_step_body(c, {dt, c->members}, {diff, c->members}, iters);
}

static int step_body(fluid_ctx* c, const MemberVal& dt, const MemberVal& diff, const MemberVal& visc, int iters, int nsteps, int use_sources)
{
    TRY(check_ctx(c));
    TRY(check_iters(iters));
    if (nsteps < 0) return fail(FLUID_E_INVALID, "nsteps < 0");
    for (int z = 0; z < nsteps; ++z) {
        if (!(use_sources && z == 0)) TRY(zero_sources(c));
        TRY(full_step(c, dt, diff, visc, iters));
    }
    HIP_TRY(hipGetLastError());
    return FLUID_OK;
}

int fluid_step(fluid_ctx* c, float dt, float diff, float visc, int iters, int nsteps, int use_sources) { return step_body(c, dt, diff, visc, iters, nsteps, use_sources); }

int fluid_step_members(fluid_ctx* c, const float* dt, const float* diff, const float* visc, int iters, int nsteps, int use_sources)
{
    TRY(check_member_args(c, "fluid_step_members", {{"dt", dt}, {"diff", diff}, {"visc", visc}}));
    if (c->members == 1) return fluid_step(c, dt[0], diff[0], visc[0], iters, nsteps, use_sources);
    TRY(ensure_consts(c));
    return step_body(c, {dt, c->members}, {diff, c->members}, {visc, c->members}, iters, nsteps, use_sources);
}

static int add_source_body(fluid_ctx* c, int x, int s, const MemberVal& dt)
{
    TRY(check_ctx(c));
    TRY(check_fields(c, {x, s}));
    if (x == s) return fail(FLUID_E_INVALID, "add_source: x and s must differ");
    TRY(op_add_source(c, x, s, dt));
    HIP_TRY(hipGetLastError());
    return FLUID_OK;
}

int fluid_op_add_source(fluid_ctx* c, int x, int s, float dt) { return add_source_body(c, x, s, dt); }

int fluid_op_add_source_members(fluid_ctx* c, int x, int s, const float* dt)
{
    TRY(check_member_args(c, "fluid_op_add_source_members", {{"dt", dt}}));
    if (c->members == 1) return fluid_op_add_source(c, x, s, dt[0]);
    TRY(ensure_consts(c));
    return add_source_body(c, x, s, {dt, c->members});
}

static int jacobi_sweep_body(fluid_ctx* c, int b, int x, int x0, int out, const MemberVal& alpha, const MemberVal& beta)
{
    TRY(check_ctx(c));
    TRY(check_fields(c, {x, x0, out}));
    TRY(check_b(b));
    if (out == x || out == x0) return fail(FLUID_E_INVALID, "jacobi_sweep: out must not alias an input");
    TRY(materialize(c, {x, x0}));
    TRY(need(c, {x}, 1));
    const float2* mab = nullptr;
    TRY(member_pairs(c, alpha, beta, &mab));
    const int v1 = c->variant == fluid::JACOBI_TB ? fluid::JACOBI_STREAM : c->variant;
    fluid::launch_jacobi(c->stream, c->st, v1, c->ptr(x), c->ptr(x0), c->ptr(out), c->pitch, c->n, c->own0, c->own1, alpha.at(0), beta.at(0),
                         b, c->mb(), mab);
    wrote(c, out, 0);
    HIP_TRY(hipGetLastError());
    return FLUID_OK;
}

int fluid_op_jacobi_sweep(fluid_ctx* c, int b, int x, int x0, int out, float alpha, float beta) { return jacobi_sweep_body(c, b, x, x0, out, alpha, beta); }

int fluid_op_jacobi_sweep_members(fluid_ctx* c, int b, int x, int x0, int out, const float* alpha, const float* beta)
{
    TRY(check_member_args(c, "fluid_op_jacobi_sweep_members", {{"alpha", alpha}, {"beta", beta}}));
    if (c->members == 1) return fluid_op_jacobi_sweep(c, b, x, x0, out, alpha[0], beta[0]);
    TRY(ensure_consts(c));
// ... 817 lines not shown
```

### fluidsimulationcuda_amd/solver.py

```python
import ctypes as C
import sys

import numpy as np

from . import capi

DT, VIS, DIFF, ITERS = 0.016, 0.0025, 0.1, 40

_ID = {name: k for k, name in enumerate(capi.FIELD_NAMES)}


def _fid(f):
    if isinstance(f, str):
        return _ID[f]
    return int(f)


def _host(a, n):
    a = np.ascontiguousarray(a, dtype=np.float32)
    if a.shape != (n + 2, n + 2):
        raise ValueError("field must have shape (%d, %d), got %s" % (n + 2, n + 2, a.shape))
    return a


# ... 150 lines not shown
        ids = [_fid(f) for f in fields]
        every, nsteps = int(every), int(nsteps)
        count = nsteps // every if every > 0 and nsteps > 0 else 0
        capacity = 0
        if every > 0:
            if out is None:
                import torch
                out = torch.empty((count, len(ids), self.members, w, w), dtype=torch.float32, device="cuda")
            capacity = device_floats(out, count * len(ids) * self.members * w * w)
        plan = capi.RunPlan(iters=int(iters), nsteps=nsteps, use_sources=1 if use_sources else 0,
                            sources=device_address(sources) if sources is not None else None, every=every,
                            fields=(C.c_int * len(ids))(*ids) if ids else None, nfields=len(ids),
                            snapshots=device_address(out) if every > 0 else None, capacity=capacity)
        written = C.c_int()
        mv = member_values(self.members, dt=dt, diff=diff, visc=visc)
        self._handover(wait)
        tail = (C.byref(plan), C.byref(written)) if coarse is None else (C.byref(plan), int(coarse), C.byref(written))
        name = "fluid_run" if mv is None else "fluid_run_members"
        fn = getattr(capi.lib(), name if coarse is None else name + "_coarse")
        capi.check(fn(self._h, *((dt, diff, visc) if mv is None else [_mf(a) for a in mv.values()]), *tail))
        if wait:
            self.synchronize()
        return (out if every > 0 else None), written.value

    def member_count(self):
        m = C.c_int()
        capi.check(capi.lib().fluid_members(self._h, C.byref(m)))
        return m.value

    def upload_rows(self, field, arr, row_lo, row_hi):
        capi.check(capi.lib().fluid_upload_rows(self._h, _fid(field), _host(arr, self.n), row_lo, row_hi))

    def download(self, field, out=None, member=None):
        if out is None:
            out = np.empty((self.n + 2, self.n + 2), dtype=np.float32)
        if member is None:
            capi.check(capi.lib().fluid_download(self._h, _fid(field), _host(out, self.n)))
        else:
            capi.check(capi.lib().fluid_download_member(self._h, int(member), _fid(field), _host(out, self.n)))
        return out

    def download_rows(self, field, out, row_lo, row_hi):
        capi.check(capi.lib().fluid_download_rows(self._h, _fid(field), out, row_lo, row_hi))
        return out

    def fill(self, field, value=0.0):
        capi.check(capi.lib().fluid_fill(self._h, _fid(field), value))

    def synchronize(self):
        capi.check(capi.lib().fluid_synchronize(self._h))

    def field_ptr(self, field):
        p = C.c_void_p()
        capi.check(capi.lib().fluid_field_ptr(self._h, _fid(field), C.byref(p)))
        return p.value

    def scalar_ptr(self):
        p = C.c_void_p()
        capi.check(capi.lib().fluid_scalar_ptr(self._h, C.byref(p)))
        return p.value

    def set_bnd(self, b, x):
        capi.check(capi.lib().fluid_op_set_bnd(self._h, b, _fid(x)))

    def _call(self, name, before, params, after=()):
        mv = member_values(self.members, **params)
        if mv is None:
            fn, values = getattr(capi.lib(), "fluid_" + name), params.values()
        else:
            fn, values = getattr(capi.lib(), "fluid_" + name + "_members"), [_mf(a) for a in mv.values()]
        capi.check(fn(self._h, *before, *values, *after))

    def add_source(self, x, s, dt=DT):
        self._call("op_add_source", (_fid(x), _fid(s)), dict(dt=dt))

    def jacobi_sweep(self, b, x, x0, out, alpha, beta):
        self._call("op_jacobi_sweep", (b, _fid(x), _fid(x0), _fid(out)), dict(alpha=alpha, beta=beta))

    def diffuse(self, b, x, x0, alpha, beta, iters=ITERS):
        self._call("op_diffuse", (b, _fid(x), _fid(x0)), dict(alpha=alpha, beta=beta), (iters,))

    def advect(self, b, d, d0, u, v, dt=DT):
        self._call("op_advect", (b, _fid(d), _fid(d0), _fid(u), _fid(v)), dict(dt=dt))

    def computeDivergenceAndPressure(self, u, v, p, div):
        capi.check(capi.lib().fluid_op_divergence(self._h, _fid(u), _fid(v), _fid(p), _fid(div)))

    def lastProject(self, u, v, p, div=None):
        capi.check(capi.lib().fluid_op_subtract_gradient(self._h, _fid(u), _fid(v), _fid(p)))

    def vel_step(self, visc=VIS, dt=DT, iters=ITERS):
        self._call("vel_step", (), dict(dt=dt, visc=visc), (iters,))

    def dens_step(self, diff=DIFF, dt=DT, iters=ITERS):
        self._call("dens_step", (), dict(dt=dt, diff=diff), (iters,))

    def step(self, nsteps=1, use_sources=False, dt=DT, diff=DIFF, visc=VIS, iters=ITERS):
        self._call("step", (), dict(dt=dt, diff=diff, visc=visc), (iters, nsteps, 1 if use_sources else 0))

    def residual(self, x, x0, alpha, beta):
        out = C.c_float()
        capi.check(capi.lib().fluid_residual(self._h, _fid(x), _fid(x0), alpha, beta, C.byref(out)))
        return out.value

    def absmax_velocity(self, u="u", v="v"):
        out = C.c_float()
        capi.check(capi.lib().fluid_absmax_velocity(self._h, _fid(u), _fid(v), C.byref(out)))
        return out.value

    def residual_members(self, x, x0, alpha, beta):
        mv = member_values(self.members, alpha=alpha, beta=beta)
        if mv is None:
            mv = {"alpha": np.full(self.members, alpha, np.float32), "beta": np.full(self.members, beta, np.float32)}
        out = np.empty(self.members, np.float32)
        capi.check(capi.lib().fluid_residual_members(self._h, _fid(x), _fid(x0), _mf(mv["alpha"]), _mf(mv["beta"]), _mf(out)))
        return out

    def absmax_velocity_members(self, u="u", v="v"):
        out = np.empty(self.members, np.float32)
        capi.check(capi.lib().fluid_absmax_velocity_members(self._h, _fid(u), _fid(v), _mf(out)))
        return out

    def member_moments(self, field):
        s, q = np.empty(self.members, np.float64), np.empty(self.members, np.float64)
        dp = C.POINTER(C.c_double)
        capi.check(capi.lib().fluid_member_moments(self._h, _fid(field), s.ctypes.data_as(dp), q.ctypes.data_as(dp)))
        return s, q

    def member_gram(self, field, centre=False):
        g = np.empty((self.members, self.members), np.float64)
        capi.check(capi.lib().fluid_member_gram(self._h, _fid(field), 1 if centre else 0, g.ctypes.data_as(C.POINTER(C.c_double))))
        return g

    def ensemble_stats(self, field, mean=True, variance=True):
        w = self.n + 2
        mu = np.empty((w, w), np.float32) if mean else None
        var = np.empty((w, w), np.float32) if variance else None
        capi.check(capi.lib().fluid_ensemble_stats(self._h, _fid(field), _mf(mu) if mean else None, _mf(var) if variance else None))
        return mu, var

    def ensemble_stats_ptr(self):
        mu, var = C.c_void_p(), C.c_void_p()
        capi.check(capi.lib().fluid_ensemble_stats_ptr(self._h, C.byref(mu), C.byref(var)))
        return mu.value, var.value

    def set_jacobi_variant(self, variant):
        capi.check(capi.lib().fluid_set_jacobi_variant(self._h, variant))

    def division_mode(self, alpha, beta):
        m = C.c_int()
        capi.check(capi.lib().fluid_division_mode(self._h, alpha, beta, C.byref(m)))
        return m.value

    def autotune_pending(self):
        m = C.c_int()
        capi.check(capi.lib().fluid_autotune_pending(self._h, C.byref(m)))
        return m.value

    def set_param(self, key, value):
        capi.check(capi.lib().fluid_set_param(self._h, key, value))

    def timing_enable(self, on=True):
        capi.check(capi.lib().fluid_timing_enable(self._h, 1 if on else 0))

    def timing_read(self, reset=True):
        t = capi.Timing()
        capi.check(capi.lib().fluid_timing_read(self._h, C.byref(t), 1 if reset else 0))
        out = {"jacobi_ms": t.jacobi_ms, "sweeps": t.sweeps, "solves": t.solves,
               "jacobi_launches": t.jacobi_launches, "jacobi_field_launches": t.jacobi_field_launches,
               "pressure_ms": t.pressure_ms, "pressure_sweeps": t.pressure_sweeps}
        for k, name in enumerate(capi.TIMING_CATEGORIES):
            out[name + "_ms"] = t.category_ms[k]
            out[name + "_calls"] = t.category_calls[k]
        return out

    def diffuse_tol(self, b, x, x0, alpha, beta, tol, max_iters=10000, check_every=8):
        it, res = C.c_int(), C.c_float()
        capi.check(capi.lib().fluid_op_diffuse_tol(self._h, b, _fid(x), _fid(x0), alpha, beta, tol, max_iters,
                                                   check_every, C.byref(it), C.byref(res)))
        return it.value, res.value

    def split_launches(self):
        m = C.c_longlong()
        capi.check(capi.lib().fluid_split_launches(self._h, C.byref(m)))
        return m.value

    def exchange_stream(self):
        p = C.c_void_p()
        capi.check(capi.lib().fluid_exchange_stream(self._h, C.byref(p)))
        return p.value or 0

    def set_exchange(self, fn):
        if fn is None:
            self._cb = None
            capi.check(capi.lib().fluid_set_exchange(self._h, C.cast(None, capi.EXCHANGE_FN), None))
            return

        def tramp(_user, kind, fields, nfields, depth, scalar):
            try:
                ids = [fields[k] for k in range(nfields)]
                if kind in (capi.XCHG_MAX, capi.XCHG_MAX_END):
                    scalar[0] = float(fn(kind, ids, depth, float(scalar[0])))
                else:
                    fn(kind, ids, depth, None)
                return 0
            except Exception:
                import traceback
                traceback.print_exc()
                return 1

        self._cb = capi.EXCHANGE_FN(tramp)
        capi.check(capi.lib().fluid_set_exchange(self._h, self._cb, None))


def coarse_size(n, factor):
    side = C.c_int()
    capi.check(capi.lib().fluid_coarse_size(int(n), int(factor), C.byref(side)))
    return side.value


def coefficients(n, dt, coef):
    a, b = C.c_float(), C.c_float()
    capi.check(capi.lib().fluid_coefficients(n, dt, coef, C.byref(a), C.byref(b)))
    return a.value, b.value


def step(N, dt, diff, visc, u, v, dens):
    for a in (u, v, dens):
        if a.dtype != np.float32 or not a.flags.c_contiguous or a.shape != (N + 2, N + 2):
            raise ValueError("fields must be C-contiguous float32 of shape (N+2, N+2)")
    capi.check(capi.lib().step(N, dt, diff, visc, u, v, dens))


def step_src(N, dt, diff, visc, iters, u, v, dens, u_prev, v_prev, dens_prev):
    for a in (u, v, dens, u_prev, v_prev, dens_prev):
        if a.dtype != np.float32 or not a.flags.c_contiguous or a.shape != (N + 2, N + 2):
            raise ValueError("fields must be C-contiguous float32 of shape (N+2, N+2)")
    capi.check(capi.lib().step_src(N, dt, diff, visc, iters, u, v, dens, u_prev, v_prev, dens_prev))
```

### include/fluid_amd.h

```cpp
#ifndef FLUID_AMD_H
#define FLUID_AMD_H

#include <stddef.h>

#ifdef __cplusplus
extern "C" {
#endif

#define FLUID_OK        0
#define FLUID_E_INVALID 1
#define FLUID_E_NOMEM   2
#define FLUID_E_HIP     3
#define FLUID_E_COMM    4

enum {
    FLUID_U = 0, FLUID_V = 1, FLUID_DENS = 2,
    FLUID_U_PREV = 3, FLUID_V_PREV = 4, FLUID_DENS_PREV = 5,
    FLUID_TMP0 = 6, FLUID_TMP1 = 7, FLUID_TMP2 = 8,
    FLUID_TMP3 = 9, FLUID_TMP4 = 10, FLUID_TMP5 = 11,
    FLUID_NFIELDS = 12
};

enum { FLUID_JACOBI_STREAM = 0, FLUID_JACOBI_LDS = 1, FLUID_JACOBI_NAIVE = 2, FLUID_JACOBI_TB = 3 };

enum {
    FLUID_PARAM_TB_MAX_SWEEPS = 0,
    FLUID_PARAM_TB_ROWS = 1,
    FLUID_PARAM_HALO = 2,
    FLUID_PARAM_TB_FAST_DIVISION = 3
    ,FLUID_PARAM_TB_EDGE_ROWS_PCT = 5
    ,FLUID_PARAM_TB_LANE_COLUMNS = 6
    ,FLUID_PARAM_TB_T16_MIN_CELLS = 7
    ,FLUID_PARAM_TB_AUTOTUNE = 8
    ,FLUID_PARAM_SLAB_OVERLAP = 10
    ,FLUID_PARAM_EARLY_ADVECT = 11
    ,FLUID_PARAM_FUSE_DIVERGENCE = 9
    ,FLUID_PARAM_FUSE_ADD_SOURCE = 12
    ,FLUID_PARAM_XCHG_OVERLAP = 13
    ,FLUID_PARAM_F16_PRESSURE_SCALE = 14
    ,FLUID_PARAM_TB_FILL = 15
    ,FLUID_PARAM_TB_MIN_CELLS = 4
};

typedef struct fluid_ctx fluid_ctx;

const char *fluid_last_error(void);

int step(int N, float dt, float diff, float visc, float *u, float *v, float *dens);
int step_src(int N, float dt, float diff, float visc, int iters,
             float *u, float *v, float *dens,
             float *u_prev, float *v_prev, float *dens_prev);
int fluid_release_cached(void);

int fluid_coefficients(int N, float dt, float coef, float *alpha, float *beta);

typedef struct fluid_config {
    int n;
    int rank, nranks;
    int halo;
    int jacobi_variant;
    void *stream;
    void *arena;
    size_t arena_bytes;
    int storage;
} fluid_config;

enum { FLUID_STORAGE_F32 = 0, FLUID_STORAGE_F16 = 1 };

size_t fluid_arena_bytes(int N);
size_t fluid_arena_bytes_ex(int N, int storage);
int fluid_layout(int N, int *pitch, int *xoff, size_t *field_floats);

int fluid_create(int N, fluid_ctx **out);
int fluid_create_ex(const fluid_config *cfg, fluid_ctx **out);
int fluid_destroy(fluid_ctx *ctx);
int fluid_synchronize(fluid_ctx *ctx);

int fluid_create_ensemble(const fluid_config *cfg, int members, fluid_ctx **out);
size_t fluid_arena_bytes_ensemble(int N, int storage, int members);
int fluid_members(fluid_ctx *ctx, int *members);
int fluid_upload_member(fluid_ctx *ctx, int member, int field, const float *host);
int fluid_download_member(fluid_ctx *ctx, int member, int field, float *host);
int fluid_step_members(fluid_ctx *ctx, const float *dt, const float *diff, const float *visc, int iters,
                       int nsteps, int use_sources);
int fluid_vel_step_members(fluid_ctx *ctx, const float *dt, const float *visc, int iters);
int fluid_dens_step_members(fluid_ctx *ctx, const float *dt, const float *diff, int iters);
int fluid_op_add_source_members(fluid_ctx *ctx, int x, int s, const float *dt);
int fluid_op_jacobi_sweep_members(fluid_ctx *ctx, int b, int x, int x0, int out,
                                  const float *alpha, const float *beta);
int fluid_op_diffuse_members(fluid_ctx *ctx, int b, int x, int x0, const float *alpha, const float *beta,
                             int iters);
int fluid_op_advect_members(fluid_ctx *ctx, int b, int d, int d0, int u, int v, const float *dt);

int fluid_owned_rows(fluid_ctx *ctx, int *row_lo, int *row_hi);
int fluid_field_ptr(fluid_ctx *ctx, int field, void **dev_ptr);
int fluid_scalar_ptr(fluid_ctx *ctx, void **dev_ptr);

int fluid_upload(fluid_ctx *ctx, int field, const float *host);
int fluid_download(fluid_ctx *ctx, int field, float *host);
int fluid_upload_rows(fluid_ctx *ctx, int field, const float *host, int row_lo, int row_hi);
int fluid_download_rows(fluid_ctx *ctx, int field, float *host, int row_lo, int row_hi);
int fluid_fill(fluid_ctx *ctx, int field, float value);

int fluid_step(fluid_ctx *ctx, float dt, float diff, float visc, int iters,
               int nsteps, int use_sources);
int fluid_vel_step(fluid_ctx *ctx, float dt, float visc, int iters);
int fluid_dens_step(fluid_ctx *ctx, float dt, float diff, int iters);

int fluid_op_set_bnd(fluid_ctx *ctx, int b, int x);
int fluid_op_add_source(fluid_ctx *ctx, int x, int s, float dt);
int fluid_op_jacobi_sweep(fluid_ctx *ctx, int b, int x, int x0, int out,
                          float alpha, float beta);
int fluid_op_diffuse(fluid_ctx *ctx, int b, int x, int x0, float alpha, float beta,
                     int iters);
int fluid_op_advect(fluid_ctx *ctx, int b, int d, int d0, int u, int v, float dt);
int fluid_op_divergence(fluid_ctx *ctx, int u, int v, int p, int div);
int fluid_op_subtract_gradient(fluid_ctx *ctx, int u, int v, int p);

int fluid_residual(fluid_ctx *ctx, int x, int x0, float alpha, float beta, float *out);
int fluid_absmax_velocity(fluid_ctx *ctx, int u, int v, float *out);

int fluid_residual_members(fluid_ctx *ctx, int x, int x0, const float *alpha, const float *beta, float *out);
int fluid_absmax_velocity_members(fluid_ctx *ctx, int u, int v, float *out);
int fluid_member_moments(fluid_ctx *ctx, int field, double *sum, double *sumsq);
int fluid_ensemble_stats(fluid_ctx *ctx, int field, float *mean, float *variance);
int fluid_ensemble_stats_ptr(fluid_ctx *ctx, void **mean_dev, void **variance_dev);
int fluid_member_gram(fluid_ctx *ctx, int field, int centre, double *gram);

int fluid_pack_members(fluid_ctx *ctx, int field, int first, int count, void *dst_dev, size_t member_stride);
int fluid_unpack_members(fluid_ctx *ctx, int field, int first, int count, const void *src_dev, size_t member_stride);
int fluid_download_members(fluid_ctx *ctx, int field, float *host);
int fluid_upload_members(fluid_ctx *ctx, int field, const float *host);
typedef struct fluid_run_plan {
    int iters, nsteps, use_sources;
    const void *sources;
    int every;
    const int *fields;
    int nfields;
    void *snapshots;
    size_t capacity;
} fluid_run_plan;
int fluid_run(fluid_ctx *ctx, float dt, float diff, float visc, const fluid_run_plan *plan, int *snapshots_written);
int fluid_run_members(fluid_ctx *ctx, const float *dt, const float *diff, const float *visc, const fluid_run_plan *plan,
                      int *snapshots_written);

int fluid_coarse_size(int N, int factor, int *side);
int fluid_pack_members_coarse(fluid_ctx *ctx, int field, int first, int count, int factor, void *dst_dev, size_t member_stride);
int fluid_download_members_coarse(fluid_ctx *ctx, int field, int factor, float *host);
int fluid_run_coarse(fluid_ctx *ctx, float dt, float diff, float visc, const fluid_run_plan *plan, int factor,
                     int *snapshots_written);
int fluid_run_members_coarse(fluid_ctx *ctx, const float *dt, const float *diff, const float *visc,
                             const fluid_run_plan *plan, int factor, int *snapshots_written);

#define FLUID_TRANSFORM_MAX_MEMBERS 64
int fluid_transform_members(fluid_ctx *ctx, const int *fields, int nfields, const float *weights);
int fluid_select_members(fluid_ctx *ctx, const int *fields, int nfields, const int *source);

int fluid_set_jacobi_variant(fluid_ctx *ctx, int variant);
int fluid_division_mode(fluid_ctx *ctx, float alpha, float beta, int *mode);
int fluid_plan_sweeps(int N, int rows, int storage, int pressure_form, int iters, int max_sweeps, int t16_min_cells,
                      int *depths, int capacity, int *count);
int fluid_autotune_pending(fluid_ctx *ctx, int *shapes_open);
int fluid_set_param(fluid_ctx *ctx, int key, int value);

enum {
    FLUID_TIME_SOURCE = 0, FLUID_TIME_DIFFUSION = 1, FLUID_TIME_DIVERGENCE = 2,
    FLUID_TIME_PROJECTION = 3, FLUID_TIME_ADVECTION = 4, FLUID_TIMING_CATEGORIES = 5
};
typedef struct fluid_timing {
    double jacobi_ms;
    long long sweeps;
    long long solves;
    double category_ms[FLUID_TIMING_CATEGORIES];
    long long category_calls[FLUID_TIMING_CATEGORIES];
    long long jacobi_launches;
    long long jacobi_field_launches;
    double pressure_ms;
    long long pressure_sweeps;
} fluid_timing;
int fluid_timing_enable(fluid_ctx *ctx, int on);
int fluid_timing_read(fluid_ctx *ctx, fluid_timing *out, int reset);

int fluid_op_diffuse_tol(fluid_ctx *ctx, int b, int x, int x0, float alpha, float beta,
                         float tol, int max_iters, int check_every,
                         int *iters_done, float *residual);

enum { FLUID_XCHG_HALO = 0, FLUID_XCHG_GATHER = 1, FLUID_XCHG_MAX = 2, FLUID_XCHG_MAX_BEGIN = 3,
       FLUID_XCHG_MAX_END = 4 };
typedef int (*fluid_exchange_fn)(void *user, int kind, const int *fields, int nfields,
                                 int depth, float *scalar);
int fluid_set_exchange(fluid_ctx *ctx, fluid_exchange_fn fn, void *user);
int fluid_exchange_stream(fluid_ctx *ctx, void **stream);
int fluid_split_launches(fluid_ctx *ctx, long long *count);
int fluid_exchange_now(fluid_ctx *ctx, int kind, const int *fields, int nfields, int depth);

#define FLUID_RCCL_ID_BYTES 128
int fluid_rccl_available(void);
int fluid_rccl_unique_id(void *id, size_t bytes);
int fluid_exchange_rccl_attach(fluid_ctx *ctx, const void *id, size_t bytes);
int fluid_exchange_rccl_attach_comm(fluid_ctx *ctx, void *nccl_comm);
int fluid_exchange_rccl_detach(fluid_ctx *ctx);
int fluid_exchange_rccl_calls(fluid_ctx *ctx, long long *halo, long long *gather, long long *max);

#ifdef __cplusplus
}
#endif
#endif
```

Baseline: 4.297 million.

## Add self-guarded two-term division mode with adaptive probing for fp32 Jacobi

Adds a new division mode 6 for the temporal-blocked Jacobi kernel. It uses a hi/lo two-term reciprocal multiply and guards itself by tracking the minimum magnitude of results, falling back to the residual-corrected mode 5 when values drop below a threshold. A per-member device ring of counters records how often the guard fails. Once failures are rare, later launches skip the guard and run mode 5 directly, probing only a hashed subset of strips. It is reachable only when fast_div is set to 4, and it adds atomics, extra kernel instantiations and a possible recompute pass.

New measurement: 4.359 million, median of 6. +1.4%, better.

```diff
diff --git a/fluidsimulationcuda_amd/capi.py b/fluidsimulationcuda_amd/capi.py
--- a/fluidsimulationcuda_amd/capi.py
+++ b/fluidsimulationcuda_amd/capi.py
@@ -21,6 +21,7 @@
 PARAM_XCHG_OVERLAP = 13
 PARAM_F16_PRESSURE_SCALE = 14
 PARAM_TB_FILL = 15
+PARAM_TB_GUARD_PROBE = 16
 XCHG_HALO, XCHG_GATHER, XCHG_MAX, XCHG_MAX_BEGIN, XCHG_MAX_END = 0, 1, 2, 3, 4
 RCCL_ID_BYTES = 128
 FIELD_NAMES = ("u", "v", "dens", "u_prev", "v_prev", "dens_prev", "tmp0", "tmp1", "tmp2", "tmp3", "tmp4", "tmp5")
@@ -125,6 +126,7 @@
     "fluid_select_members": [_ctx, C.POINTER(_i), _i, C.POINTER(_i)],
     "fluid_set_jacobi_variant": [_ctx, _i],
     "fluid_division_mode": [_ctx, _f, _f, C.POINTER(_i)],
+    "fluid_guard_counts": [_ctx, _i, _i, C.POINTER(C.c_ulonglong), C.POINTER(C.c_ulonglong)],
     "fluid_autotune_pending": [_ctx, C.POINTER(_i)],
     "fluid_plan_sweeps": [_i, _i, _i, _i, _i, _i, _i, C.POINTER(_i), _i, C.POINTER(_i)],
     "fluid_set_param": [_ctx, _i, _i],
diff --git a/fluidsimulationcuda_amd/csrc/fluid_ctx.h b/fluidsimulationcuda_amd/csrc/fluid_ctx.h
--- a/fluidsimulationcuda_amd/csrc/fluid_ctx.h
+++ b/fluidsimulationcuda_amd/csrc/fluid_ctx.h
@@ -126,6 +126,10 @@
     MemberStage stage;
     TransformTables xform;
     unsigned int* tiles = nullptr;
+    unsigned long long* guard = nullptr;
+    int guard_ring[3] = {0, 0, 0};
+    unsigned guard_seq = 0;
+    int guard_probe = 16;
     unsigned int* h_scalar = nullptr;
     hipEvent_t scalar_ready = nullptr;
     int variant = fluid::JACOBI_TB;
diff --git a/fluidsimulationcuda_amd/csrc/fluid_kernels.h b/fluidsimulationcuda_amd/csrc/fluid_kernels.h
--- a/fluidsimulationcuda_amd/csrc/fluid_kernels.h
+++ b/fluidsimulationcuda_amd/csrc/fluid_kernels.h
@@ -22,7 +22,9 @@
     double yd;
     float alpha, beta, hi, lo;
     float x0_inc, div_scale;
-    unsigned tile_thr, pad;
+    unsigned tile_thr;
+    float hi3, lo3;
+    unsigned pad;
 };
 
 struct TbBatch {
@@ -34,6 +36,11 @@
     float hi[3], lo[3];
     const unsigned* tiles[3];
     unsigned tile_thr[3];
+    float hi3[3], lo3[3];
+    unsigned long long* guard[3];
+    int guard_ring[3];
+    unsigned guard_seq;
+    unsigned guard_probe;
     int tile_pitch;
     void* div[3];
     float div_scale;
@@ -65,7 +72,11 @@
     {16, 0, 2, TB_PLAIN},  {16, 2, 2, TB_PLAIN},  {16, 3, 2, TB_PLAIN},  {16, 4, 2, TB_PLAIN},  {16, 5, 2, TB_PLAIN},
     {8, 4, 2, TB_DIVSRC},  {12, 4, 2, TB_DIVSRC}, {16, 4, 2, TB_DIVSRC}, {8, 0, 2, TB_ADDSRC},  {8, 2, 2, TB_ADDSRC},  {8, 5, 2, TB_ADDSRC},
     {12, 0, 2, TB_ADDSRC}, {12, 2, 2, TB_ADDSRC}, {12, 5, 2, TB_ADDSRC}, {16, 0, 2, TB_ADDSRC}, {16, 2, 2, TB_ADDSRC}, {16, 5, 2, TB_ADDSRC},
+    {8, 6, 2, TB_PLAIN},   {12, 6, 2, TB_PLAIN},  {16, 6, 2, TB_PLAIN},  {8, 6, 2, TB_ADDSRC},  {12, 6, 2, TB_ADDSRC}, {16, 6, 2, TB_ADDSRC},
 };
+constexpr int kGuardWords = 4;
+constexpr unsigned kGuardDirect = 0x80000000u;
+constexpr unsigned kGuardShare = 8;
 constexpr int kTbShapeCount = sizeof(kTbShapes) / sizeof(kTbShapes[0]);
 constexpr int jacobi_tb_index(int T, int divmode, int nv, int form)
 {
@@ -80,7 +91,7 @@
 {
     return i == kTbShapeCount || (jacobi_tb_index(kTbShapes[i].T, kTbShapes[i].divmode, kTbShapes[i].nv, kTbShapes[i].form) == i && tb_shapes_unique(i + 1));
 }
-static_assert(kTbShapeCount == 52 && tb_shapes_unique(), "52 distinct shapes: adding or removing one is a change of this table");
+static_assert(kTbShapeCount == 58 && tb_shapes_unique(), "58 distinct shapes: adding or removing one is a change of this table");
 inline constexpr int kTbDepths[] = {16, 12, 8, 4, 2};
 constexpr bool is_tb_depth(int T) { for (int d : kTbDepths) if (d == T) return true; return false; }
 bool launch_jacobi_tb(hipStream_t s, int st, int T, int divmode, int nv, int form, const TbBatch& batch, int pitch, int n, int row_lo,
diff --git a/fluidsimulationcuda_amd/csrc/fluid_kernels.hip b/fluidsimulationcuda_amd/csrc/fluid_kernels.hip
--- a/fluidsimulationcuda_amd/csrc/fluid_kernels.hip
+++ b/fluidsimulationcuda_amd/csrc/fluid_kernels.hip
@@ -398,7 +398,9 @@
     float beta;
     double yd;
     float hi, lo;
+    float hi3, lo3;
 };
+constexpr int tb_divides_as(int divmode) { return divmode == 7 ? 5 : divmode; }
 constexpr float kDiv5NegScale = -0x1p24f;
 
 template <typename S, int NV>
@@ -423,6 +425,8 @@
     float x0_inc;
     bool st_rg_lane, is_lg;
     bool fill;
+    float guard_thr;
+    int t_last;
 };
 
 __device__ __forceinline__ float fxor(float v, unsigned m) { return __uint_as_float(__float_as_uint(v) ^ m); }
@@ -441,6 +445,7 @@
     if (DIVMODE == 0) return num / k.beta;
     if (DIVMODE == 4) return num * k.beta;
     if (DIVMODE == 3) return __builtin_fmaf(num, k.hi, num * k.lo);
+    if (DIVMODE == 6) return __builtin_fmaf(num, k.hi3, num * k.lo3);
     if (DIVMODE == 5) {
         const float q0 = num * k.beta;
         const float e = __builtin_fmaf(q0, k.hi, num * kDiv5NegScale);
@@ -455,6 +460,9 @@
     else if constexpr (DIVMODE == 3) {
         const v2f p = num * k.lo;
         return __builtin_elementwise_fma(num, (v2f){k.hi, k.hi}, p);
+    } else if constexpr (DIVMODE == 6) {
+        const v2f p = num * k.lo3;
+        return __builtin_elementwise_fma(num, (v2f){k.hi3, k.hi3}, p);
     } else if constexpr (DIVMODE == 5) {
         const v2f ds = num * kDiv5NegScale;
         const v2f q0 = num * k.beta;
@@ -480,7 +488,7 @@
         s = s + (v2f){dn.c[p], dn.c[p + 1]};
         if constexpr (DIVMODE != 4) s = s * alpha;
         s = (v2f){r.c[p], r.c[p + 1]} + s;
-        s = tb_div2<DIVMODE>(s, k);
+        s = tb_div2<tb_divides_as(DIVMODE)>(s, k);
         G.c[p] = s.x;
         G.c[p + 1] = s.y;
     }
@@ -617,6 +625,21 @@
 #pragma unroll
         for (int p = 0; p < NV; p += 2) nf = __builtin_elementwise_fma((v2f){G.c[p], G.c[p + 1]}, (v2f){0.f, 0.f}, nf);
     }
+    if constexpr (DIVMODE == 7) {
+#pragma unroll
+        for (int c = 0; c < NV; ++c) nf.x = __builtin_fmaf(G.c[c], 0.f, nf.x);
+    }
+}
+
+template <int DIVMODE, bool COUNTED, typename S, int NV>
+__device__ __forceinline__ void tb_guard(const Vec<NV>& q, int t, const TbArgs<S, NV>& a, v2f& nf)
+{
+    if constexpr (DIVMODE == 6 || DIVMODE == 7) {
+        float m = nf.y;
+#pragma unroll
+        for (int p = 0; p < NV; p += 2) m = __builtin_fminf(__builtin_fminf(m, __builtin_fabsf(q.c[p])), __builtin_fabsf(q.c[p + 1]));
+        if (!COUNTED || t <= a.t_last) nf.y = m;
+    }
 }
 
 template <int T, int DIVMODE, bool EDGE, bool WALL, bool GEN, int PH, typename S, int NV, bool DIVSRC = false, bool ADDSRC = false,
@@ -650,6 +673,7 @@
                 Q[0].c[p + 1] = q.y;
             }
         }
+        tb_guard<DIVMODE, PART || GEN, S, NV>(Q[0], t, a, nf);
     }
     {
         const unsigned off = a.ld_off + (unsigned)(t + 3) * a.row_bytes;
@@ -712,11 +736,12 @@
     tb_qshift<T, T + 1, NV>(Q);
 }
 
+constexpr int kMarchAgain = 1, kMarchLow = 2;
 template <int T, int DIVMODE, bool EDGE, bool WALL, typename S, int NV, bool DIVSRC = false, bool ADDSRC = false>
-__device__ __forceinline__ bool tb_march(int t0, int t1, const TbArgs<S, NV>& a)
+__device__ __forceinline__ int tb_march(int t0, int t1, const TbArgs<S, NV>& a)
 {
     Vec<NV> W[T][3], Q[T + 1], PX[3], PQ[3], UR[3], VR[3];
-    v2f nf = {0.f, 0.f};
+    v2f nf = {0.f, (DIVMODE == 6 || DIVMODE == 7) ? __builtin_inff() : 0.f};
     Vec<NV> zero;
 #pragma unroll
     for (int c = 0; c < NV; ++c) zero.c[c] = 0.f;
@@ -744,7 +769,7 @@
         }
     }
     const int fill_end = (a.fill && t0 == a.q_lo - T) ? t0 + 3 * ((2 * T + 2) / 3) : t0;
-    const int full_end = a.fill ? t1 - 2 : t1;
+    const int full_end = (a.fill || DIVMODE == 6 || DIVMODE == 7) ? t1 - 2 : t1;
     auto stages = [&](int u) { return u > t1 ? 0 : u < fill_end ? (u - t0) >> 1 : T; };
     for (; t <= t1 && t < fill_end && (!WALL || t + 1 <= a.n); t += 3) {
         tb_step<T, DIVMODE, EDGE, WALL, false, 0, S, NV, DIVSRC, ADDSRC, true>(t, W, Q, PX, PQ, a, UR, VR, nf, stages(t));
@@ -768,12 +793,15 @@
             tb_step<T, DIVMODE, EDGE, WALL, true, 2, S, NV, DIVSRC, ADDSRC>(t + 2, W, Q, PX, PQ, a, UR, VR, nf);
         }
     }
-    if constexpr (DIVMODE == 5) return __builtin_amdgcn_ballot_w64((nf.x != nf.x) | (nf.y != nf.y)) != 0ull;
-    else return false;
+    if constexpr (DIVMODE == 5) return __builtin_amdgcn_ballot_w64((nf.x != nf.x) | (nf.y != nf.y)) != 0ull ? kMarchAgain : 0;
+    else if constexpr (DIVMODE == 6) return __builtin_amdgcn_ballot_w64(nf.y < a.guard_thr) != 0ull ? (kMarchAgain | kMarchLow) : 0;
+    else if constexpr (DIVMODE == 7)
+        return (__builtin_amdgcn_ballot_w64(nf.x != nf.x) != 0ull ? kMarchAgain : 0) | (__builtin_amdgcn_ballot_w64(nf.y < a.guard_thr) != 0ull ? kMarchLow : 0);
+    else return 0;
 }
 
 template <int T, int DIVMODE, typename S, int NV, bool DIVSRC = false, bool ADDSRC = false>
-__device__ __forceinline__ bool tb_march_any(bool edge, bool wall, int t0, int t1, const TbArgs<S, NV>& a)
+__device__ __forceinline__ int tb_march_any(bool edge, bool wall, int t0, int t1, const TbArgs<S, NV>& a)
 {
     if (edge) {
         if (wall) return tb_march<T, DIVMODE, true, true, S, NV, DIVSRC, ADDSRC>(t0, t1, a);
@@ -796,6 +824,8 @@
 {
     static_assert(!DIVSRC || DIVMODE == 4, "the divergence-sourced launch is the first launch of a pressure solve");
     static_assert(!(DIVSRC && ADDSRC) && (!ADDSRC || DIVMODE != 3), "one second store per launch; mode 3's tiles are taken from the summed field");
+    static_assert(DIVMODE != 6 || (NV == 2 && sizeof(S) == 4 && !DIVSRC), "the self-guarded mode: fp32 storage, 2-column lanes");
+    static_assert(DIVMODE != 7, "mode 7 is a march of mode 6's kernel, not a kernel");
     const unsigned per_xcd = gridDim.x >> 3;
     unsigned vid = (blockIdx.x & 7u) * per_xcd + (blockIdx.x >> 3);
     if (vid >= (unsigned)(g.inner_blocks + g.edge_blocks)) return;
@@ -819,6 +849,7 @@
     double yd = batch.yd[sv];
     float k_hi = batch.hi[sv], k_lo = batch.lo[sv], x0_inc = batch.x0_inc[sv], div_scale = batch.div_scale;
     unsigned tile_thr = batch.tile_thr[sv];
+    float k_hi3 = batch.hi3[sv], k_lo3 = batch.lo3[sv];
     if (batch.mk != nullptr) {
         typedef const TbMemberK __attribute__((address_space(4))) * MemberKPtr;
         const MemberKPtr mk = (MemberKPtr)(uintptr_t)batch.mk + ((size_t)sv * (unsigned)batch.members + member);
@@ -829,7 +860,8 @@
         k_lo = mk->lo;
         x0_inc = mk->x0_inc;
         if (ADDSRC) div_scale = mk->div_scale;
-        if (DIVMODE == 3) tile_thr = mk->tile_thr;
+        if (DIVMODE == 3 || DIVMODE == 6) tile_thr = mk->tile_thr;
+        if (DIVMODE == 6) { k_hi3 = mk->hi3; k_lo3 = mk->lo3; }
     }
     const int b = batch.b[sv];
     constexpr int HL = (T + NV - 1) / NV;
@@ -847,6 +879,9 @@
     a.k.yd = yd;
     a.k.lo = k_lo;
     a.k.hi = k_hi;
+    a.k.hi3 = k_hi3;
+    a.k.lo3 = k_lo3;
+    a.guard_thr = __uint_as_float(tile_thr);
     a.x0_inc = x0_inc;
     int seg_hi = row_hi;
     a.q_lo = row_lo + strip * rbw;
@@ -896,8 +931,9 @@
     a.k.beta = beta;
     a.fill = fill != 0;
     const int t0 = max(0, a.q_lo - T), t1 = a.q_hi - 1 + T;
+    a.t_last = t1;
     const bool wall = (a.q_lo < T) || (a.q_hi - 1 + T > n + 1);
-    constexpr int DM = DIVMODE == 3 ? 2 : DIVMODE;
+    constexpr int DM = DIVMODE == 3 ? 2 : DIVMODE == 6 ? 5 : DIVMODE;
     bool two_term = false;
     if constexpr (DIVMODE == 3) {
         const unsigned* __restrict__ tiles = batch.tiles[sv] ? batch.tiles[sv] + (size_t)member * batch.tile_mstride : nullptr;
@@ -912,10 +948,45 @@
                 low |= tiles[(size_t)(tr0 + i / ntc) * batch.tile_pitch + (tc0 + i % ntc)] < thr;
         two_term = tiles != nullptr && __builtin_amdgcn_ballot_w64(low) == 0ull;
     }
-    if (two_term) {
+    if constexpr (DIVMODE == 6) {
+        unsigned long long* ring = batch.guard[sv] ? batch.guard[sv] + (size_t)member * kGuardWords : nullptr;
+        const bool guarded = ring != nullptr && !edge && !wall;
+        const unsigned r = (unsigned)batch.guard_ring[sv];
+        bool direct = false;
+        if (ring != nullptr) {
+            typedef const unsigned long long __attribute__((address_space(4))) * RingPtr;
+            const unsigned long long prev = ((RingPtr)(uintptr_t)ring)[r == 0 ? 2 : r - 1];
+            const unsigned seen = (unsigned)prev & ~kGuardDirect, failed = (unsigned)(prev >> 32);
+            direct = (prev & kGuardDirect) ? !(seen != 0 && failed == 0) : (unsigned long long)failed * kGuardShare > seen;
+            if (vid == 0 && threadIdx.x == 0) {
+                ring[r == 2 ? 0 : r + 1] = 0ull;
+                if (direct) atomicAdd(ring + r, (unsigned long long)kGuardDirect);
+            }
+        }
+        int res = kMarchAgain;
+        if (guarded) {
+            bool count = true;
+            if (!direct) {
+                res = tb_march<T, 6, false, false, S, NV, false, ADDSRC>(t0, t1, a);
+                if (res & kMarchAgain) res = tb_march<T, 5, false, false, S, NV, false, ADDSRC>(t0, t1, a) | kMarchLow;
+            } else {
+                unsigned h = (unsigned)strip * 0x9E3779B1u ^ (unsigned)win * 0x85EBCA6Bu ^ batch.guard_seq * 0xC2B2AE35u;
+                h ^= h >> 15;
+                h *= 0x2C1B3C6Du;
+                h ^= h >> 12;
+                count = batch.guard_probe != 0 && h % batch.guard_probe == 0;
+                if (count) res = tb_march<T, 7, false, false, S, NV, false, ADDSRC>(t0, t1, a);
+                else res = tb_march<T, 5, false, false, S, NV, false, ADDSRC>(t0, t1, a);
+            }
+            if (count && lane == 0) atomicAdd(ring + r, 1ull | ((res & kMarchLow) ? 1ull << 32 : 0ull));
+        } else {
+            res = tb_march_any<T, 5, S, NV, false, ADDSRC>(edge, wall, t0, t1, a);
+        }
+        if (res & kMarchAgain) tb_march_any<T, 2, S, NV, false, ADDSRC>(edge, wall, t0, t1, a);
+    } else if (two_term) {
         tb_march_any<T, DIVMODE, S, NV>(edge, wall, t0, t1, a);
     } else {
-        const bool again = tb_march_any<T, DM, S, NV, DIVSRC, ADDSRC>(edge, wall, t0, t1, a);
+        const bool again = tb_march_any<T, DM, S, NV, DIVSRC, ADDSRC>(edge, wall, t0, t1, a) & kMarchAgain;
         if constexpr (DIVMODE == 5) {
             if (again) tb_march_any<T, 2, S, NV, false, ADDSRC>(edge, wall, t0, t1, a);
         }
@@ -1868,11 +1939,17 @@
 }
 
 using TbKernel = void (*)(TbBatch, int, int, int, int, int, int, TbGrid, int);
+template <typename S, size_t I>
+static TbKernel tb_kernel()
+{
+    if constexpr (kTbShapes[I].divmode == 6 && sizeof(S) != 4) return nullptr;
+    else return &k_jacobi_tb<kTbShapes[I].T, kTbShapes[I].divmode, kTbShapes[I].nv, S, kTbShapes[I].form == TB_DIVSRC,
+                             kTbShapes[I].form == TB_ADDSRC>;
+}
 template <typename S, size_t... I>
 static std::array<TbKernel, kTbShapeCount> tb_kernels(std::index_sequence<I...>)
 {
-    return {&k_jacobi_tb<kTbShapes[I].T, kTbShapes[I].divmode, kTbShapes[I].nv, S, kTbShapes[I].form == TB_DIVSRC,
-                         kTbShapes[I].form == TB_ADDSRC>...};
+    return {tb_kernel<S, I>()...};
 }
 
 bool launch_jacobi_tb(hipStream_t s, int st, int T, int divmode, int nv, int form, const TbBatch& batch, int pitch, int n, int row_lo,
@@ -1881,7 +1958,7 @@
     static const auto f32 = tb_kernels<float>(std::make_index_sequence<kTbShapeCount>());
     static const auto f16 = tb_kernels<half_t>(std::make_index_sequence<kTbShapeCount>());
     const int shape = jacobi_tb_index(T, divmode, nv, form);
-    if (shape < 0) return false;
+    if (shape < 0 || (st == STORAGE_F16 ? f16 : f32)[shape] == nullptr) return false;
     const int rows = row_hi - row_lo;
     if (rows <= 0 || batch.count <= 0 || batch.members <= 0) return true;
     if (hole_lo < row_lo) hole_lo = row_lo;
diff --git a/fluidsimulationcuda_amd/csrc/fluid_solver.hip b/fluidsimulationcuda_amd/csrc/fluid_solver.hip
--- a/fluidsimulationcuda_amd/csrc/fluid_solver.hip
+++ b/fluidsimulationcuda_amd/csrc/fluid_solver.hip
@@ -280,6 +280,7 @@
     float arg = 0.f;
     float hi = 0.f, lo = 0.f;
     unsigned tile_thr = 0;
+    float hi3 = 0.f, lo3 = 0.f;
     double yd = 0.0;
 };
 
@@ -300,46 +301,62 @@
     const float rbeta = 1.0f / beta;
     const bool pow2 = std::frexp(beta, &e2) == 0.5f && std::isnormal(rbeta) && rbeta * beta == 1.0f;
     const float hi = round_down_to_float(plan.yd), lo = (float)(plan.yd - (double)hi);
-    const bool two_term = c->fast_div == 1 && c->tiles && beta >= 1.0f && beta <= 0x1p24f && std::isnormal(hi) && std::isnormal(lo) && lo > 0.f;
-    const bool residual = c->fast_div == 2 && beta >= 0x1p-60f && beta <= 0x1p60f;
+    const bool splits = beta >= 1.0f && beta <= 0x1p24f && std::isnormal(hi) && std::isnormal(lo) && lo > 0.f;
+    const bool two_term = c->fast_div == 1 && c->tiles && splits;
+    const bool residual = (c->fast_div == 2 || c->fast_div == 4) && beta >= 0x1p-60f && beta <= 0x1p60f;
+    const bool guarded = c->fast_div == 4 && c->guard && splits && residual && c->st == fluid::STORAGE_F32 && c->tb_nv == 2 && c->nranks == 1;
     const float r5_hi = beta * 0x1p24f, r5_lo = -(rbeta * 0x1p-24f);
-    int want = force ? force : (pow2 && alpha == 1.0f) ? 4 : two_term ? 3 : residual ? 5 : 2;
+    int want = force ? force : (pow2 && alpha == 1.0f) ? 4 : two_term ? 3 : guarded ? 6 : residual ? 5 : 2;
     unsigned bits;
     std::memcpy(&bits, &beta, sizeof bits);
     int dev = 0;
     (void)hipGetDevice(&dev);
     DivProofs& proofs = div_proofs();
     std::lock_guard<std::mutex> lock(proofs.mu);
+    auto prove = [&](int w) -> int {
+        const unsigned long long key = ((unsigned long long)(dev & 0xFF) << 40) | ((unsigned long long)w << 32) | bits;
+        auto it = proofs.proven.find(key);
+        if (it != proofs.proven.end()) return it->second;
+        unsigned long long* bad = reinterpret_cast<unsigned long long*>(c->d_scalar) + 1;
+        unsigned long long* hbad = reinterpret_cast<unsigned long long*>(c->h_scalar) + 1;
+        if (hipMemsetAsync(bad, 0, sizeof *bad, c->stream) != hipSuccess) return -1;
+        fluid::launch_validate_div(c->stream, w, beta, (w == 4 || w == 5) ? rbeta : beta, plan.yd, w == 5 ? r5_hi : hi, w == 5 ? r5_lo : lo, bad);
+        if (hipMemcpyAsync(hbad, bad, sizeof *bad, hipMemcpyDeviceToHost, c->stream) != hipSuccess ||
+            hipStreamSynchronize(c->stream) != hipSuccess)
+            return -1;
+        const int m = *hbad == 0 ? w : 0;
+        proofs.proven.emplace(key, m);
+        return m;
+    };
     int mode = 0;
     while (want != 0) {
-        const unsigned long long key = ((unsigned long long)(dev & 0xFF) << 40) | ((unsigned long long)want << 32) | bits;
-        auto it = proofs.proven.find(key);
-        if (it != proofs.proven.end()) {
-            mode = it->second;
+        if (want == 6) {
+            const int p3 = prove(3), p5 = p3 < 0 ? -1 : prove(5);
+            if (p5 < 0) return plan;
+            mode = (p3 == 3 && p5 == 5) ? 6 : 0;
+            if (mode == 0) { want = 5; continue; }
         } else {
-            unsigned long long* bad = reinterpret_cast<unsigned long long*>(c->d_scalar) + 1;
-            unsigned long long* hbad = reinterpret_cast<unsigned long long*>(c->h_scalar) + 1;
-            if (hipMemsetAsync(bad, 0, sizeof *bad, c->stream) != hipSuccess) return plan;
-            fluid::launch_validate_div(c->stream, want, beta, (want == 4 || want == 5) ? rbeta : beta, plan.yd, want == 5 ? r5_hi : hi,
-                                       want == 5 ? r5_lo : lo, bad);
-            if (hipMemcpyAsync(hbad, bad, sizeof *bad, hipMemcpyDeviceToHost, c->stream) != hipSuccess ||
-                hipStreamSynchronize(c->stream) != hipSuccess)
-                return plan;
-            mode = *hbad == 0 ? want : 0;
-            proofs.proven.emplace(key, mode);
+            mode = prove(want);
+            if (mode < 0) return plan;
         }
         if (mode != 0) break;
         want = want == 2 ? 0 : 2;
     }
     plan.mode = mode;
-    if (mode == 4 || mode == 5) plan.arg = rbeta;
-    if (mode == 5) {
+    if (mode == 4 || mode == 5 || mode == 6) plan.arg = rbeta;
+    if (mode == 5 || mode == 6) {
         plan.hi = r5_hi;
         plan.lo = r5_lo;
     }
     if (mode == 3) {
         plan.hi = hi;
         plan.lo = lo;
+    }
+    if (mode == 6) {
+        plan.hi3 = hi;
+        plan.lo3 = lo;
+    }
+    if (mode == 3 || mode == 6) {
         const float thr = beta * 0x1p-72f;
         std::memcpy(&plan.tile_thr, &thr, sizeof thr);
     }
@@ -699,6 +716,7 @@
 
 size_t tile_words(const fluid_ctx* c) { return (size_t)fluid::tile_rows(c->n) * fluid::tile_pitch(c->n); }
 unsigned* solve_tiles(const fluid_ctx* c, int slot) { return c->tiles + (size_t)slot * c->members * tile_words(c); }
+unsigned long long* solve_guard(const fluid_ctx* c, int slot) { return c->guard + (size_t)slot * c->members * fluid::kGuardWords; }
 
 void plan_members(fluid_ctx* c, const Coeffs& k, std::vector<DivPlan>& out)
 {
@@ -828,7 +846,7 @@
 fluid::TbMemberK solve_constants(const Batch& B, int j, int m, const MemberVal& x0_inc, const MemberVal& div_scale)
 {
     const DivPlan& p = B.plan[j][B.plan[j].size() > 1 ? (size_t)m : 0];
-    return {p.yd, B.sv[j].k->alpha.at(m), p.arg, p.hi, p.lo, x0_inc.at(m), div_scale.at(m), p.tile_thr, 0};
+    return {p.yd, B.sv[j].k->alpha.at(m), p.arg, p.hi, p.lo, x0_inc.at(m), div_scale.at(m), p.tile_thr, p.hi3, p.lo3, 0};
 }
 
 int fill_batch(fluid_ctx* c, const Batch& B, int first, int last, bool divsrc, bool addsrc, fluid::TbBatch* out)
@@ -855,6 +873,12 @@
         bt.lo[q] = k0.lo;
         bt.tiles[q] = B.plan[j][0].mode == 3 ? solve_tiles(c, B.scratch_base + j) : nullptr;
         bt.tile_thr[q] = k0.tile_thr;
+        bt.hi3[q] = k0.hi3;
+        bt.lo3[q] = k0.lo3;
+        if (B.plan[j][0].mode == 6) {
+            bt.guard[q] = solve_guard(c, B.scratch_base + j);
+            bt.guard_ring[q] = c->guard_ring[B.scratch_base + j];
+        }
         bt.b[q] = B.sv[j].b;
         bt.x_zero[q] = c->field[B.cur[j]].zero ? 1 : 0;
         bt.x0_inc[q] = k0.x0_inc;
@@ -865,6 +889,8 @@
     bt.mstride = c->field_floats;
     bt.tile_mstride = tile_words(c);
     bt.tile_pitch = fluid::tile_pitch(c->n);
+    bt.guard_seq = c->guard_seq;
+    bt.guard_probe = (unsigned)c->guard_probe;
     bt.div_scale = div_scale.at(0);
     if (divsrc) {
         bt.x[0] = c->ptr(B.ds->u);
@@ -1006,7 +1032,13 @@
                 const bool divsrc = B.ds != nullptr && k == 0, addsrc = B.add_src && k == 0;
                 fluid::TbBatch bt;
                 TRY(fill_batch(c, B, first, last, divsrc, addsrc, &bt));
-                TRY(launch_fused(c, bt, T, B.plan[first][0].mode, divsrc, addsrc, lo, hi));
+                int mode = B.plan[first][0].mode;
+                if (mode == 6 && !fluid::jacobi_tb_exists(T, 6, c->tb_nv, addsrc ? fluid::TB_ADDSRC : fluid::TB_PLAIN)) mode = 5;
+                TRY(launch_fused(c, bt, T, mode, divsrc, addsrc, lo, hi));
+                if (mode == 6) {
+                    for (int j = first; j < last; ++j) c->guard_ring[B.scratch_base + j] = (c->guard_ring[B.scratch_base + j] + 1) % 3;
+                    c->guard_seq += 1;
+                }
                 if (c->timing) {
                     c->launches += 1;
                     c->field_launches += (long long)(last - first) * c->members;
@@ -1527,6 +1559,9 @@
         const size_t words = 3 * (size_t)members * tile_words(c);
         if (!hip_ok(hipMalloc((void**)&c->tiles, words * sizeof(unsigned)), "hipMalloc(tiles)")) return bail(rc);
         if (!hip_ok(hipMemsetAsync(c->tiles, 0, words * sizeof(unsigned), c->stream), "hipMemsetAsync(tiles)")) return bail(rc);
+        const size_t gbytes = 3 * (size_t)members * fluid::kGuardWords * sizeof(unsigned long long);
+        if (!hip_ok(hipMalloc((void**)&c->guard, gbytes), "hipMalloc(guard)")) return bail(rc);
+        if (!hip_ok(hipMemsetAsync(c->guard, 0, gbytes, c->stream), "hipMemsetAsync(guard)")) return bail(rc);
     }
     if (P > 1 && !hip_ok(hipMalloc((void**)&c->d_partials, fluid::kMaxPartials * sizeof(float)), "hipMalloc(partials)")) return bail(rc);
     if (!hip_ok(hipHostMalloc((void**)&c->h_scalar, 256, hipHostMallocDefault), "hipHostMalloc")) return bail(rc);
@@ -1571,6 +1606,7 @@
     c->rccl = nullptr;
     if (c->h_scalar) (void)hipHostFree(c->h_scalar);
     if (c->tiles) (void)hipFree(c->tiles);
+    if (c->guard) (void)hipFree(c->guard);
     for (auto& b : c->consts.live) (void)hipEventDestroy(b.copied);
     for (hipEvent_t ev : c->consts.free_events) (void)hipEventDestroy(ev);
     if (c->consts.dev) (void)hipFree(c->consts.dev);
@@ -1769,8 +1805,12 @@
         c->tb_min_cells = value;
         return FLUID_OK;
     case FLUID_PARAM_TB_FAST_DIVISION:
-        if (value < 0 || value > 3) return fail(FLUID_E_INVALID, "TB_FAST_DIVISION must be 0, 1, 2 or 3");
+        if (value < 0 || value > 4) return fail(FLUID_E_INVALID, "TB_FAST_DIVISION must be 0, 1, 2, 3 or 4");
         c->fast_div = value;
+        return FLUID_OK;
+    case FLUID_PARAM_TB_GUARD_PROBE:
+        if (value < 0) return fail(FLUID_E_INVALID, "TB_GUARD_PROBE must be >= 0");
+        c->guard_probe = value;
         return FLUID_OK;
     case FLUID_PARAM_TB_AUTOTUNE:
         c->autotune = value != 0;
@@ -1865,6 +1905,20 @@
     return FLUID_OK;
 }
 
+int fluid_guard_counts(fluid_ctx* c, int slot, int member, unsigned long long* evaluated, unsigned long long* failed)
+{
+    TRY(check_ctx(c));
+    if (!evaluated || !failed) return fail(FLUID_E_INVALID, "null pointer");
+    if (slot < 0 || slot > 2 || member < 0 || member >= c->members) return fail(FLUID_E_INVALID, "fluid_guard_counts: slot in [0,3), member in [0,members)");
+    unsigned long long word = 0;
+    const unsigned long long* src = solve_guard(c, slot) + (size_t)member * fluid::kGuardWords + (c->guard_ring[slot] + 2) % 3;
+    HIP_TRY(hipMemcpyAsync(&word, src, sizeof word, hipMemcpyDeviceToHost, c->stream));
+    HIP_TRY(hipStreamSynchronize(c->stream));
+    *evaluated = word & 0xFFFFFFFFull & ~(unsigned long long)fluid::kGuardDirect;
+    *failed = word >> 32;
+    return FLUID_OK;
+}
+
 int fluid_set_exchange(fluid_ctx* c, fluid_exchange_fn fn, void* user)
 {
     TRY(check_ctx(c));
diff --git a/fluidsimulationcuda_amd/solver.py b/fluidsimulationcuda_amd/solver.py
--- a/fluidsimulationcuda_amd/solver.py
+++ b/fluidsimulationcuda_amd/solver.py
@@ -326,6 +326,11 @@
         capi.check(capi.lib().fluid_division_mode(self._h, alpha, beta, C.byref(m)))
         return m.value
 
+    def guard_counts(self, slot, member=0):
+        a, b = C.c_ulonglong(), C.c_ulonglong()
+        capi.check(capi.lib().fluid_guard_counts(self._h, slot, member, C.byref(a), C.byref(b)))
+        return a.value, b.value
+
     def autotune_pending(self):
         m = C.c_int()
         capi.check(capi.lib().fluid_autotune_pending(self._h, C.byref(m)))
diff --git a/include/fluid_amd.h b/include/fluid_amd.h
--- a/include/fluid_amd.h
+++ b/include/fluid_amd.h
@@ -39,6 +39,7 @@
     ,FLUID_PARAM_XCHG_OVERLAP = 13
     ,FLUID_PARAM_F16_PRESSURE_SCALE = 14
     ,FLUID_PARAM_TB_FILL = 15
+    ,FLUID_PARAM_TB_GUARD_PROBE = 16
     ,FLUID_PARAM_TB_MIN_CELLS = 4
 };
 
@@ -158,6 +159,7 @@
 
 int fluid_set_jacobi_variant(fluid_ctx *ctx, int variant);
 int fluid_division_mode(fluid_ctx *ctx, float alpha, float beta, int *mode);
+int fluid_guard_counts(fluid_ctx *ctx, int slot, int member, unsigned long long *evaluated, unsigned long long *failed);
 int fluid_plan_sweeps(int N, int rows, int storage, int pressure_form, int iters, int max_sweeps, int t16_min_cells,
                       int *depths, int capacity, int *count);
 int fluid_autotune_pending(fluid_ctx *ctx, int *shapes_open);
```
